# DCDmllm/AnyEdit

Hardware: AMD Instinct MI355X
Metric: edited-images/sec @512x512, 50 DDIM steps (higher is better)
Workload: dtype bf16; 1 GPU; configs[1]: AnySD (SD-1.5 UNet in=8 + task embedding/expert adapters) 512x512 bf16, 50 DDIM steps, batch=4/GPU, 3-branch CFG (UNet batch 12); images_per_gpu=4, ddim_steps=50, cfg_branches=3, hip_graph=True, parallelism=dp1 (image-sharded, no data-path collective)

## Files before the change

### anyedit_amd/_lib.py

```python
import ctypes
import os

import torch

_HERE = os.path.dirname(os.path.abspath(__file__))
LIB_PATH = os.environ.get("AE_LIB_PATH") or os.path.join(_HERE, "libanyedit_hip.so")

c_void_p, c_int, c_long, c_float = ctypes.c_void_p, ctypes.c_int, ctypes.c_long, ctypes.c_float

SIGNATURES = {
    "ae_version": [],
    "ae_last_error": [],
    "ae_device_arch": [ctypes.c_char_p, c_int],
    "ae_device_info": [ctypes.POINTER(c_int), ctypes.POINTER(c_long), ctypes.POINTER(c_int)],
    "ae_gemm_bf16": [c_void_p, c_long, c_void_p, c_long, c_int, c_void_p, c_long, c_void_p, c_long, c_int, c_int, c_int,
                     c_void_p, c_void_p, c_long, c_void_p, c_long, c_int, c_int, c_int, c_void_p, c_void_p],
    "ae_conv3x3_workspace_floats": [c_int, c_int, c_int, c_int, c_int, c_int, c_int],
    "ae_conv3x3_bf16": [c_void_p, c_void_p, c_void_p, c_void_p, c_long, c_void_p, c_void_p, c_int, c_int, c_int, c_int, c_int,
                        c_int, c_int, c_int, c_void_p, c_void_p, c_int, c_void_p],
    "ae_conv3x3_up2_bf16": [c_void_p, c_void_p, c_void_p, c_void_p, c_int, c_int, c_int, c_int, c_int, c_void_p, c_void_p],
    "ae_gemm_plan": [c_int] * 8 + [ctypes.POINTER(c_int)],
    "ae_conv3x3_plan": [c_int] * 11 + [ctypes.POINTER(c_int)],
    "ae_conv3x3_up2_plan": [c_int] * 6 + [ctypes.POINTER(c_int)],
    "ae_groupnorm_rows_per_chunk": [c_int, c_int],
    "ae_groupnorm_workspace_floats": [c_int, c_int, c_int, c_int],
    "ae_groupnorm_nhwc_bf16": [c_void_p, c_void_p, c_int, c_void_p, c_void_p, c_void_p, c_int, c_int, c_int, c_int, c_float,
                               c_int, c_void_p, c_void_p, c_void_p, c_void_p, c_void_p, c_void_p],
    "ae_layernorm_bf16": [c_void_p, c_void_p, c_void_p, c_void_p, c_int, c_int, c_float, c_void_p],
    "ae_attn_fwd_bf16": [c_void_p, c_void_p, c_void_p, c_void_p, c_int, c_int, c_int, c_int, c_int,
                         c_long, c_long, c_long, c_long, c_long, c_long, c_long, c_long, c_long, c_long, c_long, c_long,
                         c_float, c_void_p, c_void_p, c_int, c_int, c_void_p, c_void_p, c_int,
                         c_void_p, c_void_p, c_int, c_long, c_long, c_long, c_long, c_long, c_long, c_void_p, c_void_p, c_void_p,
                         c_void_p],
    "ae_attn_bwd_bf16": [c_void_p] * 10 + [c_int] * 5 + [c_long] * 21 + [c_float, c_void_p, c_int, c_void_p, c_void_p],
    "ae_attn_bwd_workspace_floats": [c_int] * 5,
    "ae_groupnorm_bwd_workspace_floats": [c_int, c_int, c_int, c_int],
    "ae_groupnorm_bwd_nhwc_bf16": [c_void_p, c_void_p, c_int, c_void_p, c_void_p, c_void_p, c_void_p, c_void_p, c_int, c_int, c_int,
                                   c_int, c_float, c_int, c_void_p, c_void_p, c_void_p, c_int, c_void_p],
    "ae_layernorm_bwd_bf16": [c_void_p, c_void_p, c_void_p, c_void_p, c_void_p, c_int, c_int, c_float, c_int, c_void_p],
    "ae_layernorm_param_grad_f32": [c_void_p, c_void_p, c_void_p, c_void_p, c_void_p, c_int, c_int, c_void_p],
    "ae_add_bf16": [c_void_p, c_void_p, c_void_p, c_long, c_void_p],
    "ae_axpy_bf16": [c_void_p, c_void_p, c_float, c_void_p, c_long, c_void_p],
    "ae_geglu_fwd_bf16": [c_void_p, c_void_p, c_long, c_int, c_void_p],
    "ae_geglu_bwd_bf16": [c_void_p, c_void_p, c_void_p, c_long, c_int, c_void_p],
    "ae_sumpool2x2_bf16": [c_void_p, c_void_p, c_int, c_int, c_int, c_int, c_void_p],
    "ae_colsum_bf16_f32": [c_void_p, c_void_p, c_int, c_int, c_long, c_void_p],
    "ae_mse_grad_f32": [c_void_p, c_void_p, c_void_p, c_long, c_float, c_void_p],
    "ae_adamw_f32": [c_void_p, c_void_p, c_void_p, c_void_p, c_long, c_float, c_float, c_float, c_float, c_float, c_int, c_float,
                     c_void_p],
    "ae_rowsum_f32": [c_void_p, c_void_p, c_int, c_long, c_void_p],
    "ae_scatter_add_rows_f32": [c_void_p, c_void_p, c_void_p, c_int, c_int, c_int, c_void_p],
    "ae_attn_fp8_workspace_bytes": [c_int, c_int, c_int, c_int, c_int],
    "ae_attn_fwd_fp8": [c_void_p, c_void_p, c_void_p, c_void_p, c_int, c_int, c_int, c_int, c_int] + [c_long] * 12 +
                       [c_float, c_void_p, c_void_p, c_int, c_int, c_void_p, c_long, c_void_p],
    "ae_ln_gemm_supported": [c_int, c_int, c_int, c_int],
    "ae_ln_gemm_bf16": [c_void_p, c_long, c_void_p, c_long, c_void_p, c_long, c_int, c_int, c_int, c_void_p, c_void_p, c_long, c_void_p, c_void_p,
                        c_float, c_int, c_void_p, c_void_p],
    "ae_gemm_ln_plan": [c_int, c_int, c_int, c_int, c_int],
    "ae_ff_fused_supported": [c_int, c_int, c_int],
    "ae_ff_fused_bf16": [c_void_p, c_long, c_void_p, c_void_p, c_float, c_void_p, c_long, c_void_p, c_void_p, c_void_p, c_void_p, c_long,
                         c_void_p, c_long, c_void_p, c_void_p, c_long, c_void_p, c_void_p, c_long, c_int, c_int, c_int, c_void_p],
    "ae_gemm_ln_bf16": [c_void_p, c_long, c_void_p, c_long, c_void_p, c_long, c_int, c_int, c_int, c_void_p, c_void_p, c_long, c_int, c_void_p,
                        c_void_p, c_int, c_void_p, c_float, c_void_p],
    "ae_task_gate_bwd": [c_void_p, c_void_p, c_void_p, c_void_p, c_int, c_int, c_int, c_void_p, c_void_p],
    "ae_task_gate_wgrad": [c_void_p, c_void_p, c_void_p, c_void_p, c_void_p, c_int, c_int, c_int, c_int, c_void_p, c_void_p, c_void_p],
    "ae_expert_kv_fwd": [c_void_p, c_void_p, c_void_p, c_void_p, c_int, c_int, c_int, c_int, c_int, c_void_p],
    "ae_expert_kv_dgrad_slices": [c_int],
    "ae_expert_kv_dgrad": [c_void_p, c_void_p, c_void_p, c_void_p, c_int, c_int, c_int, c_int, c_int, c_void_p, c_void_p],
    "ae_expert_kv_wgrad": [c_void_p, c_void_p, c_void_p, c_void_p, c_int, c_int, c_int, c_int, c_int, c_void_p],
    "ae_transpose_last2": [c_void_p, c_void_p, c_int, c_int, c_int, c_int, c_int, c_int, c_void_p],
    "ae_concat_channels_bf16": [c_void_p, c_int, c_void_p, c_int, c_void_p, c_long, c_void_p],
    "ae_im2col3x3_c8_bf16": [c_void_p, c_void_p, c_int, c_int, c_int, c_void_p],
    "ae_split_channels_bf16": [c_void_p, c_int, c_int, c_void_p, c_void_p, c_long, c_int, c_int, c_void_p],
    "ae_timestep_embedding": [c_void_p, c_void_p, c_void_p, c_void_p, c_int, c_int, c_float, c_void_p],
    "ae_ddim_step_f32": [c_void_p, c_void_p, c_void_p, c_void_p, c_void_p, c_void_p, c_long, c_int, c_float, c_float, c_float,
                         c_float, c_float, c_float, c_float, c_float, c_void_p],
    "ae_ddim_encode_step_f32": [c_void_p, c_void_p, c_void_p, c_long, c_int, c_float, c_float, c_float, c_void_p],
    "ae_plms_combine_f32": [c_void_p, c_void_p, c_void_p, c_void_p, c_void_p, c_long, c_int, c_void_p],
    "ae_mask_blend_f32": [c_void_p, c_void_p, c_void_p, c_void_p, c_void_p, c_int, c_int, c_int, c_float, c_float, c_int, c_void_p],
    "ae_q_sample_f32": [c_void_p, c_void_p, c_void_p, c_void_p, c_void_p, c_int, c_long, c_void_p],
    "ae_silu_to_bf16": [c_void_p, c_int, c_void_p, c_long, c_void_p],
    "ae_add_bcast_bf16": [c_void_p, c_void_p, c_void_p, c_long, c_long, c_void_p],
    "ae_resample2x_rows_bf16": [c_void_p, c_void_p, c_int, c_int, c_int, c_int, c_int, c_void_p],
    "ae_scale_shift_rows_bf16": [c_void_p, c_void_p, c_long, c_void_p, c_int, c_long, c_int, c_int, c_void_p],
    "ae_window_partition_bf16": [c_void_p, c_void_p, c_int, c_int, c_int, c_int, c_int, c_int, c_void_p],
    "ae_layernorm_window_supported": [c_int],
    "ae_layernorm_window_bf16": [c_void_p, c_void_p, c_void_p, c_void_p, c_void_p, c_void_p, c_int, c_int, c_int, c_int, c_int, c_int, c_float,
                                 c_void_p],
    "ae_sam_relpos_terms": [c_void_p, c_long, c_long, c_long, c_void_p, c_void_p, c_void_p, c_void_p, c_int, c_int, c_int, c_int,
                            c_int, c_int, c_int, c_void_p],
    "ae_softmax_rows_f32_bf16": [c_void_p, c_long, c_void_p, c_long, c_int, c_int, c_float, c_void_p],
    "ae_gaussian_moments_f32": [c_void_p, c_void_p, c_void_p, c_void_p, c_void_p, c_void_p, c_int, c_long, c_void_p],
    "ae_ms_deform_attn_fwd_f32": [c_void_p] * 6 + [c_int] * 7 + [c_void_p],
    "ae_ms_deform_attn_bwd_f32": [c_void_p] * 9 + [c_int] * 7 + [c_void_p],
    "ae_linear_f32": [c_void_p, c_long, c_void_p, c_long, c_void_p, c_void_p, c_long, c_int, c_int, c_int, c_void_p],
    "ae_dpm_multistep_f32": [c_void_p] * 5 + [c_long, c_int, c_float, c_int, c_int, c_float, c_float, c_int, c_float, c_float, c_float,
                             c_float, c_void_p],
    "ae_layernorm_act_bf16": [c_void_p, c_void_p, c_void_p, c_void_p, c_long, c_int, c_float, c_int, c_void_p],
    "ae_sam_pe_encode_f32": [c_void_p, c_void_p, c_void_p, c_void_p, c_void_p, c_int, c_int, c_float, c_float, c_float, c_void_p],
    "ae_sam_mask_downscale_bf16": [c_void_p] * 10 + [c_int, c_int, c_int, c_float, c_void_p],
    "ae_sam_mask_product_f32": [c_void_p, c_void_p, c_void_p, c_int, c_int, c_int, c_int, c_int, c_void_p],
    "ae_sam_postprocess_masks": [c_void_p, c_void_p, c_void_p] + [c_int] * 8 + [c_float, c_int, c_void_p],
    "ae_nms_sorted_f32": [c_void_p, c_void_p, c_int, c_float, c_void_p],
    "ae_sam_preprocess_f32": [c_void_p, c_int, c_void_p, c_int, c_int, c_int, c_int, c_int, c_void_p, c_void_p, c_void_p],
    "ae_patchify_f32_bf16": [c_void_p, c_void_p, c_int, c_int, c_int, c_int, c_int, c_void_p],
    "ae_mse_f32": [c_void_p, c_void_p, c_void_p, c_void_p, c_long, c_void_p],
    "ae_lincomb4_f32": [c_void_p, c_void_p, c_float, c_void_p, c_float, c_void_p, c_float, c_void_p, c_float, c_long, c_void_p],
    "ae_dpm_adaptive_err_f32": [c_void_p, c_void_p, c_void_p, c_float, c_float, c_int, c_long, c_void_p, c_void_p],
    "ae_task_gate": [c_void_p, c_void_p, c_void_p, c_void_p, c_int, c_int, c_int, c_int, c_void_p, c_void_p, c_void_p, c_void_p],
    "ae_attn_causal_short_bf16": [c_void_p, c_void_p, c_void_p, c_void_p, c_int, c_int, c_int, c_int] + [c_long] * 12 + [c_float, c_void_p],
    "ae_clip_embed_bf16": [c_void_p, c_int, c_void_p, c_void_p, c_void_p, c_int, c_int, c_int, c_int, c_int, c_void_p],
    "ae_bias_act_f32_bf16": [c_void_p, c_long, c_void_p, c_void_p, c_long, c_long, c_int, c_int, c_void_p],
    "ae_clip_pool_eos_bf16": [c_void_p, c_int, c_void_p, c_void_p, c_int, c_int, c_int, c_long, c_void_p],
    "ae_clip_patch_rows_bf16": [c_void_p, c_int, c_void_p, c_int, c_int, c_int, c_int, c_int, c_int, c_float, c_void_p, c_void_p, c_void_p],
    "ae_clip_vision_embed_ln_bf16": [c_void_p, c_long, c_void_p, c_void_p, c_void_p, c_void_p, c_void_p, c_int, c_int, c_int, c_float, c_void_p],
    "ae_clip_vision_pool_ln_bf16": [c_void_p, c_long, c_void_p, c_void_p, c_void_p, c_int, c_int, c_float, c_void_p],
    "ae_dino_embed_bf16": [c_void_p, c_long, c_void_p, c_void_p, c_void_p, c_void_p, c_int, c_int, c_int, c_void_p],
    "ae_swiglu_f32_bf16": [c_void_p, c_long, c_void_p, c_void_p, c_long, c_long, c_int, c_void_p],
    "ae_swin_window_attn_bf16": [c_void_p, c_long, c_void_p, c_void_p, c_void_p, c_long, c_int, c_int, c_int, c_int, c_int, c_int, c_int, c_float, c_void_p],
    "ae_swin_merge_ln_bf16": [c_void_p, c_void_p, c_void_p, c_void_p, c_int, c_int, c_int, c_int, c_float, c_void_p],
    "ae_scale_residual_f32_bf16": [c_void_p, c_long, c_void_p, c_void_p, c_void_p, c_long, c_void_p, c_long, c_long, c_int, c_void_p],
    "ae_biattn_split_rows": [c_int],
    "ae_biattn_workspace_bytes": [c_int, c_int, c_int, c_int, c_int],
    "ae_biattn_bf16": [c_void_p, c_long] * 4 + [c_void_p, c_void_p] + [c_void_p, c_long] * 2 + [c_int] * 5 + [c_float, c_void_p, c_long, c_void_p],
    "ae_attn_masked_short_bf16": [c_void_p] * 5 + [c_int] * 4 + [c_long] * 12 + [c_float, c_void_p],
    "ae_contrastive_bf16": [c_void_p, c_long, c_void_p, c_void_p, c_void_p, c_long, c_void_p] + [c_int] * 5 + [c_void_p],
    "ae_topk_rows_max_n": [],
    "ae_topk_rows_f32": [c_void_p, c_long, c_void_p, c_int, c_int, c_int, c_void_p],
    "ae_gdino_proposals_f32": [c_void_p, ctypes.POINTER(c_int), ctypes.POINTER(c_int), c_int, c_void_p, c_void_p, c_int, c_int, c_void_p],
    "ae_gdino_query_sine": [c_void_p, c_void_p, c_void_p, c_void_p, c_long, c_int, c_int, c_int, c_void_p],
    "ae_gdino_box_refine_f32": [c_void_p, c_long, c_void_p, c_void_p, c_void_p, c_void_p, c_void_p, c_long, c_int, c_void_p],
    "ae_gdino_text_spans": [c_void_p, c_int, c_int, c_int, c_int] + [c_long] * 8 + [c_void_p, c_void_p, c_void_p, c_void_p],
    "ae_bert_embed_ln_bf16": [c_void_p, c_void_p, c_void_p] + [c_void_p] * 6 + [c_int] * 6 + [c_float, c_void_p],
    "ae_attn_span_short_bf16": [c_void_p] * 5 + [c_int] * 4 + [c_long] * 12 + [c_float, c_void_p],
    "ae_gdino_level_geometry": [c_void_p, c_int, c_int, c_int, ctypes.POINTER(c_int), ctypes.POINTER(c_int), c_int, c_float, c_float, c_void_p, c_void_p, c_void_p,
                                c_void_p, c_int, c_void_p],
    "ae_gdino_neck_groupnorm_workspace_floats": [c_int, c_int],
    "ae_gdino_neck_groupnorm": [c_void_p, c_long, c_void_p, c_void_p, c_float, c_void_p, c_long, c_long, c_int, c_int, c_void_p, c_void_p],
    "ae_gdino_ground": [c_void_p, c_void_p, c_float, c_float, c_void_p, c_void_p, c_void_p, c_void_p, c_void_p, c_int, c_int, c_int, c_void_p],
    "ae_hed_stem_bf16": [c_void_p, c_int, c_long, c_long, c_long, c_long, c_void_p, c_void_p, c_void_p, c_void_p, c_int, c_int, c_int, c_int, c_void_p],
    "ae_relu_bf16": [c_void_p, c_long, c_void_p],
    "ae_hed_tail_bf16": [c_void_p, c_void_p, c_void_p, c_void_p, c_void_p, c_int, c_int, c_int, c_int, c_void_p],
    "ae_hed_fuse": [c_void_p] * 7 + [c_int] * 4 + [c_void_p],
}
_RESTYPES = {"ae_last_error": ctypes.c_char_p, "ae_groupnorm_workspace_floats": c_long, "ae_conv3x3_workspace_floats": c_long,
             "ae_groupnorm_bwd_workspace_floats": c_long, "ae_attn_fp8_workspace_bytes": c_long, "ae_attn_bwd_workspace_floats": c_long,
             "ae_biattn_workspace_bytes": c_long, "ae_gdino_neck_groupnorm_workspace_floats": c_long}


class AnyEditHipError(RuntimeError):
    pass


def _load():
    if not os.path.exists(LIB_PATH):
        raise ImportError(
            f"{LIB_PATH} is missing: the HIP extension is REQUIRED (no CPU/eager fallback exists). "
            "Build it with `python -c 'import __graft_entry__ as g; g.build()'` or `python anyedit_amd/build.py`.")
    lib = ctypes.CDLL(LIB_PATH)
    for name, argtypes in SIGNATURES.items():
        fn = getattr(lib, name)
        fn.argtypes = argtypes
        fn.restype = _RESTYPES.get(name, c_int)
    return lib


lib = _load()


def check(rc, what=""):
    if rc != 0:
        msg = lib.ae_last_error()
        raise AnyEditHipError(f"{what} failed (rc={rc}): {msg.decode() if msg else ''}")


def device_arch():
    buf = ctypes.create_string_buffer(128)
    check(lib.ae_device_arch(buf, 128), "ae_device_arch")
    return buf.value.decode()
```

### anyedit_amd/anysd/model.py

```python
import torch
import torch.nn as nn

from anyedit_amd import ops
from anyedit_amd.cldm.model import trusted_torch_load
from anyedit_amd.ldm.modules.attention import BasicTransformerBlock

BF16 = torch.bfloat16

EDIT_TYPES = ["add", "remove", "replace", "color_alter", "appearance_alter", "material_alter", "action_change",
              "textual_change", "background_change", "tone_transfer", "style_change", "movement", "outpaint", "rotation_change",
              "resize", "implicit_change", "relation_change", "counting", "visual_reference", "visual_bbox", "visual_depth",
              "visual_scribble", "visual_segment", "visual_sketch", "visual_material_transfer"]


class ImageProjModel(nn.Module):

    def __init__(self, clip_dim=1280, cross_dim=768, tokens=4):
        super().__init__()
        self.tokens, self.cross_dim = tokens, cross_dim
        self.proj = nn.Linear(clip_dim, tokens * cross_dim)
        self.norm = nn.LayerNorm(cross_dim)

    def rows(self, ref_embeds):
        B = ref_embeds.shape[0]
        cls = ref_embeds[:, 0].to(BF16).contiguous()
        y = ops.gemm(cls, ops.pack_linear(self.proj.weight), self.proj.bias.detach().float().contiguous())
        y = y.reshape(B * self.tokens, self.cross_dim)
        return ops.layernorm(y, self.norm.weight.detach().float().contiguous(), self.norm.bias.detach().float().contiguous(),
                             self.norm.eps)


class MoE(nn.Module):

    def __init__(self, unet, image_encoder=None, expert_num=11, ckpt_path=None, n_tasks=len(EDIT_TYPES), context_dim=768,
                 clip_dim=1280, ip_tokens=4):
        super().__init__()
        self.unet = unet
        enc_dim = getattr(image_encoder, "hidden_size", None)
        if enc_dim is not None and enc_dim != clip_dim:
            raise ValueError(f"MoE: the image encoder's hidden_size {enc_dim} does not match clip_dim {clip_dim} (image_proj_model reads hidden states of that width)")
        self.image_encoder = image_encoder
        self.expert_num = expert_num
        self.context_dim = context_dim
        self.image_proj_model = ImageProjModel(clip_dim, context_dim, ip_tokens)
        self.task_embs = nn.Parameter(torch.randn(n_tasks, context_dim) * 0.02)
        self.gate = nn.Linear(context_dim, expert_num)
        self._blocks = [m for m in unet.modules() if isinstance(m, BasicTransformerBlock)]
        self.adapter_modules = nn.ParameterList(
            [nn.Parameter(torch.randn(expert_num, 2 * b.attn2.heads * b.attn2.dim_head, context_dim) * context_dim ** -0.5)
             for b in self._blocks])
        if ckpt_path is not None:
            self.load_state_dict(trusted_torch_load(ckpt_path, "cpu"), strict=False)

    def save_pretrained(self, path):
        sd = {k: v for k, v in self.state_dict().items() if not k.startswith(("unet.", "image_encoder."))}
        torch.save(sd, path)

    @torch.no_grad()
    def route(self, edit_code):
        return ops.task_gate(self.task_embs.detach(), edit_code, self.gate.weight.detach(), self.gate.bias.detach())

    @torch.no_grad()
    def reference_embeds(self, pixel_values):
        if self.image_encoder is None:
            raise ValueError("MoE.reference_embeds: this MoE was built without an image_encoder (MoE(unet, image_encoder=CLIPVisionModelWithProjection(...)))")
        return self.image_encoder.encode_pixels(pixel_values, -2).clone()

    @torch.no_grad()
    def prepare_conditioning(self, encoder_hidden_states, ref_embeds, edit_code, ip_scale=None):
        if ref_embeds.dim() == 4:
            ref_embeds = self.reference_embeds(ref_embeds)
        B, L, Dc = encoder_hidden_states.shape
        dev = encoder_hidden_states.device
        te = self.task_embs.detach()[edit_code.long()]
        ctx = torch.cat([encoder_hidden_states.float(), te[:, None, :].float()], dim=1)
        context_rows = ctx.reshape(B * (L + 1), Dc).to(BF16).contiguous()
        probs, top1, top1p = self.route(edit_code)
        gate = top1p if ip_scale is None else top1p * ip_scale
        ip_rows = self.image_proj_model.rows(ref_embeds)
        T_ip = self.image_proj_model.tokens
        kv_cache = {}
        for blk, W in zip(self._blocks, self.adapter_modules):
            attn = blk.attn2
            kv_cache[id(attn)] = attn.project_kv(context_rows)
            Wm = W.detach()
            if Wm.dtype != torch.float32 or not Wm.is_contiguous():
                Wm = Wm.float().contiguous()
            kv_ip = ops.expert_kv(ip_rows, Wm, top1, T_ip)
            kv_cache[("adapter", id(attn))] = (kv_ip, gate.float().contiguous())
        return context_rows, kv_cache

    @torch.no_grad()
    def denoise(self, x, timesteps, context_rows, kv_cache, emb_pack=None):
        return self.unet.forward_rows(x, timesteps, context_rows, kv_cache=kv_cache, emb_pack=emb_pack)

    def forward(self, noisy_latents, timesteps, encoder_hidden_states, image_embeds, edit_code):
        context_rows, kv_cache = self.prepare_conditioning(encoder_hidden_states, image_embeds, edit_code)
        return self.denoise(noisy_latents, timesteps, context_rows, kv_cache)
```

### anyedit_amd/anysd/pipeline.py

```python
import numpy as np
import torch

from anyedit_amd import ops
from anyedit_amd.ldm.models.diffusion.ddim import DDIMSampler, _f32


class EditPipeline:
    def __init__(self, moe, schedule_model, use_graph=True, text_encoder=None):
        self.moe = moe
        self.text_encoder = text_encoder
        self._null_ehs, self._null_tok = None, None
        self.sampler = DDIMSampler(schedule_model)
        self.schedule_model = schedule_model
        self.use_graph = use_graph
        self._graph = None
        self._graph_key = None
        self._emb_pack = None
        self.randn = torch.randn

    def _denoise_static(self):
        if self._emb_pack is not None:
            return self.moe.denoise(self._x_in, self._t, self._ctx_rows, self._kv_cache, emb_pack=self._emb_pack)
        return self.moe.denoise(self._x_in, self._t, self._ctx_rows, self._kv_cache)

    def _hoist_time_embedding(self, steps_desc, nb, dev):
        import os
        unet = getattr(self.moe, "unet", None)
        if os.environ.get("AE_HOIST_TEMB", "1") == "0" or unet is None or not hasattr(unet, "time_embedding_rows") or getattr(unet, "num_classes", None) is not None:
            if self._emb_pack is not None:
                self._emb_pack, self._graph = None, None
            return None
        pack = unet.time_embedding_rows(torch.as_tensor(np.ascontiguousarray(steps_desc), dtype=torch.long, device=dev))
        if self._emb_pack is None or tuple(self._emb_pack.all.shape) != (nb, pack.all.shape[1]) or self._emb_pack.offsets != pack.offsets:
            from anyedit_amd.ldm.modules.diffusionmodules.openaimodel import EmbPack
            self._emb_pack = EmbPack(None, torch.empty(nb, pack.all.shape[1], dtype=torch.float32, device=dev), pack.offsets)
            self._graph = None
        return pack.all

    def set_step(self, t, temb_row=None):
        self._t.fill_(int(t))
        if self._emb_pack is not None:
            if temb_row is None:
                temb_row = self.moe.unet.time_embedding_rows(torch.full((1,), int(t), dtype=torch.long, device=self._t.device)).all[0]
            self._emb_pack.all.copy_(temb_row.unsqueeze(0).expand_as(self._emb_pack.all))

    def _ensure_graph(self, key):
        if self._graph is not None and self._graph_key == key:
            return
        cur = torch.cuda.current_stream()
        side = torch.cuda.Stream()
        side.wait_stream(cur)
        with torch.cuda.stream(side):
            for _ in range(2):
                self._denoise_static()
        cur.wait_stream(side)
        torch.cuda.synchronize()
        g = torch.cuda.CUDAGraph()
        with torch.cuda.graph(g):
            self._eps = self._denoise_static()
        self._graph, self._graph_key = g, key

    @torch.no_grad()
    def prepare(self, img_lat, ehs, null_ehs, ref_embeds, edit_code):
        B = img_lat.shape[0]
        if null_ehs.shape[0] == 1:
            null_ehs = null_ehs.expand(B, -1, -1)
        ehs3 = torch.cat([ehs, null_ehs, null_ehs], 0)
        ref3 = torch.cat([ref_embeds, ref_embeds, torch.zeros_like(ref_embeds)], 0)
        code3 = torch.cat([edit_code] * 3, 0)
        ctx_rows, kv_cache = self.moe.prepare_conditioning(ehs3, ref3, code3)
        img_cond3 = torch.cat([img_lat, img_lat, torch.zeros_like(img_lat)], 0).float()
        C = img_lat.shape[1]
        shape_in = (3 * B, 2 * C, *img_lat.shape[2:])
        if self._same_layout(ctx_rows, kv_cache, shape_in):
            self._ctx_rows.copy_(ctx_rows)
            for k, v in kv_cache.items():
                cur = self._kv_cache[k]
                if isinstance(v, tuple):
                    for c, n in zip(cur, v):
                        c.copy_(n)
                else:
                    cur.copy_(v)
        else:
            self._ctx_rows, self._kv_cache = ctx_rows, kv_cache
            self._x_in = torch.empty(shape_in, dtype=torch.float32, device=img_lat.device)
            self._t = torch.zeros(3 * B, dtype=torch.long, device=img_lat.device)
            self._graph = None
        self._x_in[:, C:] = img_cond3

    def _same_layout(self, ctx_rows, kv_cache, shape_in):
        if getattr(self, "_kv_cache", None) is None or getattr(self, "_x_in", None) is None:
            return False
        if tuple(self._x_in.shape) != tuple(shape_in) or self._ctx_rows.shape != ctx_rows.shape or self._kv_cache.keys() != kv_cache.keys():
            return False
        for k, v in kv_cache.items():
            cur = self._kv_cache[k]
            a, b = (cur, v) if isinstance(v, tuple) else ((cur,), (v,))
            if any(x.shape != y.shape or x.dtype != y.dtype for x, y in zip(a, b)):
                return False
        return True

    def _prompt_ids(self, prompts_or_ids):
        te = self.text_encoder
        if isinstance(prompts_or_ids, str) or (isinstance(prompts_or_ids, (list, tuple)) and prompts_or_ids and isinstance(prompts_or_ids[0], str)):
            tok = te._need_tokenizer()
            return tok(prompts_or_ids, truncation=True, max_length=te.max_length, return_length=True, return_overflowing_tokens=False,
                       padding="max_length", return_tensors="pt")["input_ids"]
        return prompts_or_ids

    def null_prompt_ehs(self):
        te = self.text_encoder
        tok = te.transformer.weights_token()
        if self._null_ehs is None or self._null_tok != tok:
            cfg = te.transformer.config
            n = min(te.max_length, cfg["max_position_embeddings"])
            ids = [[cfg["bos_token_id"], cfg["eos_token_id"]] + [cfg["pad_token_id"]] * (n - 2)]
            self._null_ehs, self._null_tok = te.encode_ids(ids).clone(), tok
        return self._null_ehs

    @torch.no_grad()
    def edit_text(self, x_T, img_lat, prompts_or_ids, ref_embeds, edit_code, reference_images=None, **edit_kwargs):
        if self.text_encoder is None:
            raise ValueError("edit_text: this pipeline was built without a text_encoder (EditPipeline(..., text_encoder=FrozenCLIPEmbedder(...)))")
        null_ehs = self.null_prompt_ehs()
        ehs = self.text_encoder.encode_ids(self._prompt_ids(prompts_or_ids))
        return self.edit(x_T, img_lat, ehs, null_ehs, ref_embeds, edit_code, reference_images=reference_images, **edit_kwargs)

    @torch.no_grad()
    def edit(self, x_T, img_lat, ehs, null_ehs, ref_embeds, edit_code, steps=50, s_txt=7.5, s_img=1.5, eta=0.0, mask=None,
             x0=None, prepared=False, step_callback=None, reference_images=None):
        B, C = x_T.shape[0], x_T.shape[1]
        dev = x_T.device
        if reference_images is not None:
            if ref_embeds is not None:
                raise ValueError("edit: pass ref_embeds or reference_images, not both")
            ref_embeds = self.moe.reference_embeds(reference_images)
        if not prepared:
            self.prepare(img_lat, ehs, null_ehs, ref_embeds, edit_code)
        s = self.sampler
        s.make_schedule(ddim_num_steps=steps, ddim_eta=eta, verbose=False)
        timesteps = s.ddim_timesteps
        total = timesteps.shape[0]
        img = x_T.float().contiguous()
        blend_noise = self.randn(x0.shape, device=dev) if mask is not None else None
        temb = self._hoist_time_embedding(np.flip(timesteps), 3 * B, dev)
        if temb is not None:
            self._emb_pack.all.copy_(temb[0].unsqueeze(0).expand_as(self._emb_pack.all))
        if self.use_graph:
            self._ensure_graph((tuple(x_T.shape), steps))
        x_view = self._x_in[:, :C].view(3, B, C, *x_T.shape[2:])
        for i, step in enumerate(np.flip(timesteps)):
            index = total - i - 1
            x_view.copy_(img.unsqueeze(0))
            self.set_step(step, temb[i] if temb is not None else None)
            if self.use_graph:
                self._graph.replay()
                eps = self._eps
            else:
                eps = self._denoise_static()
            noise = self.randn(img.shape, device=dev) if eta != 0.0 else None
            img, _ = ops.ddim_step(img, eps, s._coeffs(index, False), 3, s0=float(s_txt), s1=float(s_img), noise=noise,
                                   want_pred_x0=False)
            if mask is not None:
                sa = float(_f32(self.schedule_model.sqrt_alphas_cumprod[int(step)]))
                s1 = float(_f32(self.schedule_model.sqrt_one_minus_alphas_cumprod[int(step)]))
                img = ops.mask_blend(img, x0, blend_noise, mask, sa, s1, ip2p_order=True)
            if step_callback is not None:
                step_callback(i, img)
        return img
```

### anyedit_amd/csrc/c_api.hip

```cpp
#include "common.hpp"
#include <stdarg.h>
#include <stdio.h>
#include <string.h>

static thread_local char g_err[512] = "";

void ae_set_error(const char* fmt, ...) {
    va_list ap;
    va_start(ap, fmt);
    vsnprintf(g_err, sizeof(g_err), fmt, ap);
    va_end(ap);
}

int ae_check_launch(const char* what) {
    hipError_t e = hipGetLastError();
    if (e != hipSuccess) {
        ae_set_error("%s: launch failed: %s", what, hipGetErrorString(e));
        return AE_ERR_LAUNCH;
    }
    return AE_OK;
}

extern "C" int ae_version(void) { return 100; }

extern "C" const char* ae_last_error(void) { return g_err; }

extern "C" int ae_device_arch(char* buf, int n) {
    if (!buf || n <= 0) return AE_ERR_ARG;
    int dev = 0;
    hipDeviceProp_t prop;
    if (hipGetDevice(&dev) != hipSuccess || hipGetDeviceProperties(&prop, dev) != hipSuccess) {
        ae_set_error("ae_device_arch: no HIP device");
        buf[0] = 0;
        return AE_ERR_LAUNCH;
    }
    strncpy(buf, prop.gcnArchName, (size_t)n - 1);
    buf[n - 1] = 0;
    return AE_OK;
}

extern "C" int ae_device_info(int* cus, long* hbm_bytes, int* clock_khz) {
    int dev = 0;
    hipDeviceProp_t prop;
    if (hipGetDevice(&dev) != hipSuccess || hipGetDeviceProperties(&prop, dev) != hipSuccess) {
        ae_set_error("ae_device_info: no HIP device");
        return AE_ERR_LAUNCH;
    }
    if (cus) *cus = prop.multiProcessorCount;
    if (hbm_bytes) *hbm_bytes = (long)prop.totalGlobalMem;
    if (clock_khz) *clock_khz = prop.clockRate;
    return AE_OK;
}
```

### anyedit_amd/csrc/common.hpp

```cpp
#pragma once
#include <hip/hip_runtime.h>
#include <stdint.h>

typedef uint16_t bf16_t;
typedef __attribute__((ext_vector_type(8))) __bf16 bf16x8_t;
typedef __attribute__((ext_vector_type(4))) float f32x4;
typedef __attribute__((ext_vector_type(2))) float f32x2;
typedef __attribute__((ext_vector_type(4))) uint32_t u32x4;
typedef __attribute__((ext_vector_type(2))) uint32_t u32x2;

#define AE_OK 0
#define AE_ERR_ARG -1
#define AE_ERR_LAUNCH -2
#define AE_ERR_UNSUPPORTED -3

void ae_set_error(const char* fmt, ...);
int ae_check_launch(const char* what);
int ae_launch_colstats(const uint16_t* x, long ld, int M, int N, float* out, hipStream_t stream);

int ae_rowpanel_fold_covers(int M, int N, int K, int epilogue, int mode);
int ae_rowpanel_fold_launch(const void* A, long lda, const void* W, long ldw, void* C, long ldc, int M, int N, int K, const float* bias, const void* residual,
                            long ldr, int epilogue, float* rowstats_out, const float* ln_stats, int ln_parts, const float* ln_colsum, float ln_eps, void* stream);

#define AE_REQUIRE(cond, ...)                 \
    do {                                      \
        if (!(cond)) {                        \
            ae_set_error(__VA_ARGS__);        \
            return AE_ERR_ARG;                \
        }                                     \
    } while (0)

__device__ __forceinline__ float bf16_to_f32(bf16_t h) { return __uint_as_float(((uint32_t)h) << 16); }

typedef __attribute__((ext_vector_type(2))) __bf16 bf16x2_t;

__device__ __forceinline__ uint32_t pack_bf16x2(float lo, float hi) {
    union { bf16x2_t b; uint32_t u; } c;
    c.b = (bf16x2_t){(__bf16)lo, (__bf16)hi};
    return c.u;
}

__device__ __forceinline__ bf16_t f32_to_bf16(float f) { return (bf16_t)(pack_bf16x2(f, 0.f) & 0xffffu); }

__device__ __forceinline__ float bf16lo(uint32_t w) { return __uint_as_float(w << 16); }
__device__ __forceinline__ float bf16hi(uint32_t w) { return __uint_as_float(w & 0xffff0000u); }

__device__ __forceinline__ bf16x8_t as_bf16x8(u32x4 v) {
    union { u32x4 u; bf16x8_t b; } c;
    c.u = v;
    return c.b;
}

typedef __attribute__((ext_vector_type(4))) short s16x4_t;
__device__ __forceinline__ s16x4_t as_s16x4(u32x2 v) {
    union { u32x2 u; s16x4_t s; } c;
    c.u = v;
    return c.s;
}

__device__ __forceinline__ float silu_f(float x) {
    return x * __builtin_amdgcn_rcpf(1.0f + __builtin_amdgcn_exp2f(-1.4426950408889634f * x));
}
__device__ __forceinline__ float erf_as_f(float z) {
    const float az = __builtin_fabsf(z);
    const float t = __builtin_amdgcn_rcpf(__builtin_fmaf(0.3275911f, az, 1.0f));
    float poly = __builtin_fmaf(1.061405429f, t, -1.453152027f);
    poly = __builtin_fmaf(poly, t, 1.421413741f);
    poly = __builtin_fmaf(poly, t, -0.284496736f);
    poly = __builtin_fmaf(poly, t, 0.254829592f);
    poly *= t;
    const float e = __builtin_amdgcn_exp2f(-1.4426950408889634f * az * az);
    const float r = __builtin_fmaf(-poly, e, 1.0f);
    return __builtin_copysignf(r, z);
}
#ifndef AE_GELU_POLY
#define AE_GELU_POLY 0
#endif
__device__ __forceinline__ float gelu_w_poly_f(float x) {
    const float ax = __builtin_fminf(__builtin_fabsf(x), 4.25f);
    const float t = __builtin_fmaf(ax * ax, 0.11072664707899094f, -1.0f);
    float p = __builtin_fmaf(0.004925727378576994f, t, -0.012811211869120598f);
    p = __builtin_fmaf(p, t, 0.017165469005703926f);
    p = __builtin_fmaf(p, t, -0.02821926586329937f);
    p = __builtin_fmaf(p, t, 0.05118509382009506f);
    p = __builtin_fmaf(p, t, -0.07870230078697205f);
    p = __builtin_fmaf(p, t, 0.11140184104442596f);
    p = __builtin_fmaf(p, t, -0.1615230143070221f);
    p = __builtin_fmaf(p, t, 0.33187076449394226f);
    return ax * p;
}
__device__ __forceinline__ float gelu_w_f(float x) {
    if (AE_GELU_POLY) return gelu_w_poly_f(x);
    const float ax = __builtin_fabsf(x);
    const float t = __builtin_amdgcn_rcpf(__builtin_fmaf(0.3275911f * 0.70710678118654752440f, ax, 1.0f));
    float poly = __builtin_fmaf(1.061405429f, t, -1.453152027f);
    poly = __builtin_fmaf(poly, t, 1.421413741f);
    poly = __builtin_fmaf(poly, t, -0.284496736f);
    poly = __builtin_fmaf(poly, t, 0.254829592f);
    poly *= t;
    const float e = __builtin_amdgcn_exp2f((-0.5f * 1.4426950408889634f) * ax * ax);
    return __builtin_fmaf(-poly, e, 1.0f);
}
#ifndef AE_GELU_OLD
#define AE_GELU_OLD 0
#endif
__device__ __forceinline__ float gelu_erf_f(float x) {
    if (AE_GELU_OLD) return 0.5f * x * (1.0f + erf_as_f(x * 0.70710678118654752440f));
    return 0.5f * __builtin_fmaf(__builtin_fabsf(x), gelu_w_f(x), x);
}
__device__ __forceinline__ float geglu_half_f(float a_half, float g) {
    if (AE_GELU_OLD) return (a_half + a_half) * gelu_erf_f(g);
    return a_half * __builtin_fmaf(__builtin_fabsf(g), gelu_w_f(g), g);
}

__device__ __forceinline__ int xcd_remap(int bid, int nblocks) {
    const int NX = 8;
    int xcd = bid % NX, j = bid / NX;
    int q = nblocks / NX, r = nblocks % NX;
    int base = (xcd < r) ? xcd * (q + 1) : r * (q + 1) + (xcd - r) * q;
    return base + j;
}

__device__ __forceinline__ void ae_dma16(__amdgpu_buffer_rsrc_t rs, int lds_byte, int voffset, int soffset = 0) {
#if defined(__HIP_DEVICE_COMPILE__)
    asm volatile("s_mov_b32 m0, %2\n\ts_nop 0\n\tbuffer_load_dwordx4 %0, %1, %3 offen lds" ::"v"(voffset), "s"(rs), "s"(lds_byte), "s"(soffset)
                 : "memory", "m0");
#endif
}

__device__ __forceinline__ float wave_reduce_sum(float v) {
#pragma unroll
    for (int o = 32; o > 0; o >>= 1) v += __shfl_xor(v, o, 64);
    return v;
}
__device__ __forceinline__ float wave_reduce_max(float v) {
#pragma unroll
    for (int o = 32; o > 0; o >>= 1) v = fmaxf(v, __shfl_xor(v, o, 64));
    return v;
}
```

### anyedit_amd/csrc/elementwise.hip

```cpp
#include "common.hpp"

namespace {

constexpr int NT = 256;

__device__ __forceinline__ float ld_any(const void* p, long i, int is_bf16) {
    return is_bf16 ? bf16_to_f32(reinterpret_cast<const bf16_t*>(p)[i]) : reinterpret_cast<const float*>(p)[i];
}
__device__ __forceinline__ void st_any(void* p, long i, float v, int is_bf16) {
    if (is_bf16) reinterpret_cast<bf16_t*>(p)[i] = f32_to_bf16(v);
    else reinterpret_cast<float*>(p)[i] = v;
}

__global__ void transpose_kernel(const void* in, void* out, int X, int Y, int Xpad, int in_bf16, int out_bf16) {
    __shared__ float tile[32][33];
    const int b = blockIdx.z;
    const int x0 = blockIdx.x * 32, y0 = blockIdx.y * 32;
    const int tx = threadIdx.x & 31, ty = threadIdx.x >> 5;
    for (int j = ty; j < 32; j += 8) {
        const int x = x0 + j, y = y0 + tx;
        tile[j][tx] = (x < X && y < Y) ? ld_any(in, ((long)b * X + x) * Y + y, in_bf16) : 0.f;
    }
    __syncthreads();
    for (int j = ty; j < 32; j += 8) {
// ... 334 lines not shown
    }
}

struct RelposArgs {
    long q_sb, q_sh, q_sn;
    int BH, Hh, qH, qW, kH, kW;
    int items[2];
};

template <int D16>
__global__ __launch_bounds__(256) void relpos_mfma_kernel(const bf16_t* __restrict__ q, const float* __restrict__ Rh, const float* __restrict__ Rw,
                                                          float* __restrict__ rel_h, float* __restrict__ rel_w, const RelposArgs p) {
    constexpr int D = 16 * D16;
    const int lane = threadIdx.x & 63, l15 = lane & 15, g = lane >> 4;
    long item = (long)blockIdx.x * 4 + __builtin_amdgcn_readfirstlane(threadIdx.x >> 6);
    int part = 0;
    if (item >= p.items[0]) { item -= p.items[0]; part = 1; }
    if (item >= p.items[part]) return;
    const int Lq = part == 0 ? p.qW : p.qH, K = part == 0 ? p.kH : p.kW;
    const int nks = (K + 15) / 16;
    const long ntrip = (long)p.BH * Lq;
    const int ngrp = (int)((ntrip + 63) / 64);
    int r = (int)item;
    const int grp = r % ngrp; r /= ngrp;
    const int ks = r % nks; r /= nks;
    const int line = r;
    const int k0 = ks * 16;
    const int krow = k0 + l15 < K ? k0 + l15 : K - 1;
    const float* Rrow = (part == 0 ? Rh : Rw) + ((long)line * K + krow) * D + 4 * g;
    f32x4 av[D16];
#pragma unroll
    for (int u = 0; u < D16; ++u) av[u] = *reinterpret_cast<const f32x4*>(Rrow + 16 * u);
    float* outp = part == 0 ? rel_h : rel_w;
    const long N = (long)p.qH * p.qW;
#pragma unroll
    for (int t = 0; t < 4; ++t) {
        long trip = (long)grp * 64 + t * 16 + l15;
        const bool live = trip < ntrip;
        if (!live) trip = ntrip - 1;
        const int h = (int)(trip % p.Hh);
        const long rest = trip / p.Hh;
        const int qi = (int)(rest % Lq), b = (int)(rest / Lq);
        const long n = part == 0 ? (long)line * p.qW + qi : (long)qi * p.qW + line;
        const bf16_t* qr = q + (long)b * p.q_sb + (long)h * p.q_sh + n * p.q_sn + 4 * g;
        uint2 bv[D16];
#pragma unroll
        for (int u = 0; u < D16; ++u) bv[u] = *reinterpret_cast<const uint2*>(qr + 16 * u);
        f32x4 acc = {0.f, 0.f, 0.f, 0.f};
#pragma unroll
        for (int u = 0; u < D16; ++u) {
            acc = __builtin_amdgcn_mfma_f32_16x16x4f32(av[u][0], bf16lo(bv[u].x), acc, 0, 0, 0);
            acc = __builtin_amdgcn_mfma_f32_16x16x4f32(av[u][1], bf16hi(bv[u].x), acc, 0, 0, 0);
            acc = __builtin_amdgcn_mfma_f32_16x16x4f32(av[u][2], bf16lo(bv[u].y), acc, 0, 0, 0);
            acc = __builtin_amdgcn_mfma_f32_16x16x4f32(av[u][3], bf16hi(bv[u].y), acc, 0, 0, 0);
        }
        if (live) {
            float* o = outp + (((long)b * p.Hh + h) * N + n) * K;
            const int kk = k0 + 4 * g;
            if ((K & 3) == 0 && kk + 3 < K) *reinterpret_cast<f32x4*>(o + kk) = acc;
            else if ((K & 1) == 0) {
                if (kk + 1 < K) *reinterpret_cast<float2*>(o + kk) = make_float2(acc[0], acc[1]);
                if (kk + 3 < K) *reinterpret_cast<float2*>(o + kk + 2) = make_float2(acc[2], acc[3]);
            } else {
#pragma unroll
                for (int e = 0; e < 4; ++e)
                    if (kk + e < K) o[kk + e] = acc[e];
            }
        }
    }
}

__global__ __launch_bounds__(NT) void softmax_rows_kernel(const float* S, long lds, bf16_t* P, long ldp, int cols, float scale) {
    __shared__ float red[NT / 64];
    const float* src = S + (long)blockIdx.x * lds;
    bf16_t* dst = P + (long)blockIdx.x * ldp;
    const int lane = threadIdx.x & 63, wave = threadIdx.x >> 6;
    float mx = -INFINITY;
    for (int c = threadIdx.x; c < cols; c += NT) mx = fmaxf(mx, src[c]);
    mx = wave_reduce_max(mx);
    if (lane == 0) red[wave] = mx;
    __syncthreads();
    mx = fmaxf(fmaxf(red[0], red[1]), fmaxf(red[2], red[3]));
    __syncthreads();
    const float c2 = scale * 1.4426950408889634f;
    float sum = 0.f;
    for (int c = threadIdx.x; c < cols; c += NT) sum += __builtin_amdgcn_exp2f((src[c] - mx) * c2);
    sum = wave_reduce_sum(sum);
    if (lane == 0) red[wave] = sum;
    __syncthreads();
    const float inv = 1.0f / ((red[0] + red[1]) + (red[2] + red[3]));
    for (int c = threadIdx.x; c < cols; c += NT) dst[c] = f32_to_bf16(__builtin_amdgcn_exp2f((src[c] - mx) * c2) * inv);
}

__global__ __launch_bounds__(NT) void gaussian_kernel(const float* moments, const float* noise, float* z, float* mean_o, float* logvar_o,
                                                      float* std_o, long per_half, long n) {
    for (long i = (long)blockIdx.x * NT + threadIdx.x; i < n; i += (long)gridDim.x * NT) {
        const long b = i / per_half, r = i - b * per_half;
        const float mean = moments[b * 2 * per_half + r];
        const float logvar = fminf(fmaxf(moments[b * 2 * per_half + per_half + r], -30.0f), 20.0f);
        const float sd = expf(0.5f * logvar);
        z[i] = noise ? mean + sd * noise[i] : mean;
        if (mean_o) mean_o[i] = mean;
        if (logvar_o) logvar_o[i] = logvar;
        if (std_o) std_o[i] = sd;
    }
}

__global__ void patchify_kernel(const float* x, bf16_t* y, int B, int Cin, int H, int W, int P) {
    const int gh = H / P, gw = W / P, K = Cin * P * P;
    const long total = (long)B * gh * gw * K;
    for (long i = (long)blockIdx.x * NT + threadIdx.x; i < total; i += (long)gridDim.x * NT) {
        const int k = (int)(i % K);
        long r = i / K;
        const int px = (int)(r % gw); r /= gw;
        const int py = (int)(r % gh); r /= gh;
        const int b = (int)r;
        const int c = k / (P * P), kk = k % (P * P), ky = kk / P, kx = kk % P;
        y[i] = f32_to_bf16(x[(((long)b * Cin + c) * H + py * P + ky) * W + px * P + kx]);
    }
}

constexpr int MSE_MAX_BLOCKS = 1024;
__global__ __launch_bounds__(NT) void mse_partial_kernel(const float* a, const float* b, float* partial, long n) {
    __shared__ float red[NT / 64];
    float s = 0.f;
    for (long i = (long)blockIdx.x * NT + threadIdx.x; i < n; i += (long)gridDim.x * NT) {
        const float d = a[i] - b[i];
        s += d * d;
    }
    s = wave_reduce_sum(s);
    if ((threadIdx.x & 63) == 0) red[threadIdx.x >> 6] = s;
    __syncthreads();
    if (threadIdx.x == 0) partial[blockIdx.x] = (red[0] + red[1]) + (red[2] + red[3]);
}
__global__ __launch_bounds__(NT) void mse_final_kernel(const float* partial, int nb, float* out, float inv_n) {
    __shared__ float red[NT / 64];
    float s = 0.f;
    for (int i = threadIdx.x; i < nb; i += NT) s += partial[i];
    s = wave_reduce_sum(s);
    if ((threadIdx.x & 63) == 0) red[threadIdx.x >> 6] = s;
    __syncthreads();
    if (threadIdx.x == 0) out[0] = ((red[0] + red[1]) + (red[2] + red[3])) * inv_n;
}

inline unsigned grid_for(long n, int per_thread = 1) {
    long b = (n + (long)NT * per_thread - 1) / ((long)NT * per_thread);
    if (b > 4096) b = 4096;
    if (b < 1) b = 1;
    return (unsigned)b;
}

}

__global__ __launch_bounds__(256) void lincomb4_kernel(float* __restrict__ out, const float* x0, float c0, const float* x1, float c1,
                                                        const float* x2, float c2, const float* x3, float c3, long n) {
    const long i = ((long)blockIdx.x * 256 + threadIdx.x) * 4;
    if (i >= n) return;
    if (i + 4 <= n) {
        f32x4 a = *reinterpret_cast<const f32x4*>(x0 + i);
        f32x4 r = {a[0] * c0, a[1] * c0, a[2] * c0, a[3] * c0};
        if (x1) { const f32x4 b = *reinterpret_cast<const f32x4*>(x1 + i); for (int e = 0; e < 4; ++e) r[e] = fmaf(b[e], c1, r[e]); }
        if (x2) { const f32x4 b = *reinterpret_cast<const f32x4*>(x2 + i); for (int e = 0; e < 4; ++e) r[e] = fmaf(b[e], c2, r[e]); }
        if (x3) { const f32x4 b = *reinterpret_cast<const f32x4*>(x3 + i); for (int e = 0; e < 4; ++e) r[e] = fmaf(b[e], c3, r[e]); }
        *reinterpret_cast<f32x4*>(out + i) = r;
    } else {
        for (long j = i; j < n; ++j) {
            float r = x0[j] * c0;
            if (x1) r = fmaf(x1[j], c1, r);
            if (x2) r = fmaf(x2[j], c2, r);
            if (x3) r = fmaf(x3[j], c3, r);
            out[j] = r;
        }
    }
}

__global__ __launch_bounds__(1024) void dpm_adaptive_err_kernel(const float* __restrict__ xl, const float* __restrict__ xh,
                                                                const float* __restrict__ xp, float atol, float rtol, long n, float* out) {
    __shared__ float red[16];
    const long base = (long)blockIdx.x * n;
    float acc = 0.f;
    for (long i = threadIdx.x; i < n; i += 1024) {
        const float l = xl[base + i];
        const float delta = fmaxf(atol, rtol * fmaxf(fabsf(l), fabsf(xp[base + i])));
        const float v = (xh[base + i] - l) / delta;
        acc = fmaf(v, v, acc);
    }
    acc = wave_reduce_sum(acc);
    if ((threadIdx.x & 63) == 0) red[threadIdx.x >> 6] = acc;
    __syncthreads();
    if (threadIdx.x == 0) {
        float t = 0.f;
        for (int w = 0; w < 16; ++w) t += red[w];
        out[blockIdx.x] = sqrtf(t / (float)n);
    }
}

extern "C" int ae_transpose_last2(const void* in, void* out, int B, int X, int Y, int Xpad, int in_bf16, int out_bf16, void* stream) {
    AE_REQUIRE(in && out && B > 0 && X > 0 && Y > 0 && Xpad >= X, "ae_transpose_last2: bad arguments");
    AE_REQUIRE(B <= 65535, "ae_transpose_last2: batch %d too large", B);
    dim3 grid((Xpad + 31) / 32, (Y + 31) / 32, B);
    hipLaunchKernelGGL(transpose_kernel, grid, dim3(256), 0, (hipStream_t)stream, in, out, X, Y, Xpad, in_bf16, out_bf16);
    return ae_check_launch("ae_transpose_last2");
}

extern "C" int ae_concat_channels_bf16(const void* a, int Ca, const void* b, int Cb, void* y, long rows, void* stream) {
    AE_REQUIRE(a && b && y && rows > 0 && Ca > 0 && Cb > 0 && Ca % 8 == 0 && Cb % 8 == 0, "ae_concat_channels_bf16: bad arguments");
    hipLaunchKernelGGL(concat_kernel, dim3(grid_for(rows * ((Ca + Cb) / 8))), dim3(NT), 0, (hipStream_t)stream,
                       (const bf16_t*)a, Ca, (const bf16_t*)b, Cb, (bf16_t*)y, rows);
    return ae_check_launch("ae_concat_channels_bf16");
}

extern "C" int ae_im2col3x3_c8_bf16(const void* x, void* y, int B, int H, int W, void* stream) {
    AE_REQUIRE(x && y && B > 0 && H > 0 && W > 0, "ae_im2col3x3_c8_bf16: bad arguments");
    AE_REQUIRE(((uintptr_t)x & 15) == 0 && ((uintptr_t)y & 15) == 0, "ae_im2col3x3_c8_bf16: 16-byte alignment");
    hipLaunchKernelGGL(im2col3x3_c8_kernel, dim3(grid_for((long)B * H * W * 16)), dim3(NT), 0, (hipStream_t)stream, (const bf16_t*)x, (bf16_t*)y, B, H, W);
    return ae_check_launch("ae_im2col3x3_c8_bf16");
}

extern "C" int ae_split_channels_bf16(const void* y, int Ca, int Cb, void* a, void* b, long rows, int accumulate_a, int accumulate_b, void* stream) {
    AE_REQUIRE(y && (a || b) && rows > 0 && Ca > 0 && Cb > 0 && Ca % 8 == 0 && Cb % 8 == 0, "ae_split_channels_bf16: bad arguments");
    hipLaunchKernelGGL(split_kernel, dim3(grid_for(rows * ((Ca + Cb) / 8))), dim3(NT), 0, (hipStream_t)stream, (const bf16_t*)y, Ca, Cb, (bf16_t*)a,
                       (bf16_t*)b, rows, accumulate_a, accumulate_b);
    return ae_check_launch("ae_split_channels_bf16");
}

extern "C" int ae_timestep_embedding(const long* t_i64, const float* t_f32, void* out_bf16, float* out_f32, int B, int dim,
                                     float max_period, void* stream) {
    AE_REQUIRE((t_i64 != nullptr) != (t_f32 != nullptr), "ae_timestep_embedding: pass exactly one of t_i64 / t_f32");
    AE_REQUIRE((out_bf16 || out_f32) && B > 0 && dim > 1, "ae_timestep_embedding: bad arguments");
    hipLaunchKernelGGL(timestep_embedding_kernel, dim3((B * dim + NT - 1) / NT), dim3(NT), 0, (hipStream_t)stream, t_i64, t_f32,
                       (bf16_t*)out_bf16, out_f32, B, dim, max_period);
    return ae_check_launch("ae_timestep_embedding");
}

extern "C" int ae_ddim_step_f32(const float* x, const float* eps, const float* noise, float* x_prev, float* pred_x0, float* e_out,
                                long n, int branches, float s0, float s1, float sqrt_one_minus_at, float sqrt_at,
                                float sqrt_a_prev, float dir_coef, float sigma_t, float temperature, void* stream) {
    AE_REQUIRE(x && eps && x_prev && n > 0, "ae_ddim_step_f32: null pointer / bad n");
    AE_REQUIRE(branches >= 1 && branches <= 3, "ae_ddim_step_f32: branches must be 1, 2 or 3 (got %d)", branches);
    DdimArgs a{x, eps, noise, x_prev, pred_x0, e_out, n, branches, s0, s1, sqrt_one_minus_at, sqrt_at, sqrt_a_prev, dir_coef, sigma_t, temperature};
    hipLaunchKernelGGL(ddim_step_kernel, dim3(grid_for(n)), dim3(NT), 0, (hipStream_t)stream, a);
    return ae_check_launch("ae_ddim_step_f32");
}

extern "C" int ae_ddim_encode_step_f32(const float* x, const float* eps, float* x_next, long n, int branches, float scale, float cx,
                                       float ce, void* stream) {
    AE_REQUIRE(x && eps && x_next && n > 0, "ae_ddim_encode_step_f32: null pointer / bad n");
    AE_REQUIRE(branches == 1 || branches == 2, "ae_ddim_encode_step_f32: branches must be 1 or 2 (got %d)", branches);
    hipLaunchKernelGGL(ddim_encode_step_kernel, dim3(grid_for(n)), dim3(NT), 0, (hipStream_t)stream, x, eps, x_next, n, branches, scale, cx, ce);
    return ae_check_launch("ae_ddim_encode_step_f32");
}

extern "C" int ae_plms_combine_f32(const float* e_t, const float* old1, const float* old2, const float* old3, float* out, long n, int order,
                                   void* stream) {
    AE_REQUIRE(e_t && out && n > 0 && order >= 0 && order <= 3, "ae_plms_combine_f32: bad arguments (order must be 0..3)");
    AE_REQUIRE(old1 && (order < 2 || old2) && (order < 3 || old3), "ae_plms_combine_f32: order %d needs that many previous predictions", order);
    hipLaunchKernelGGL(plms_combine_kernel, dim3(grid_for(n)), dim3(NT), 0, (hipStream_t)stream, e_t, old1, old2, old3, out, n, order);
    return ae_check_launch("ae_plms_combine_f32");
}

extern "C" int ae_mask_blend_f32(const float* img, const float* x0, const float* noise, const float* mask, float* out, int B,
                                 int C, int HW, float sqrt_ac, float sqrt_one_minus_ac, int ip2p_order, void* stream) {
    AE_REQUIRE(img && x0 && noise && mask && out && B > 0 && C > 0 && HW > 0, "ae_mask_blend_f32: bad arguments");
    const long n = (long)B * C * HW;
    hipLaunchKernelGGL(mask_blend_kernel, dim3(grid_for(n)), dim3(NT), 0, (hipStream_t)stream, img, x0, noise, mask, out, n, C, HW,
                       sqrt_ac, sqrt_one_minus_ac, ip2p_order);
    return ae_check_launch("ae_mask_blend_f32");
}

extern "C" int ae_q_sample_f32(const float* x0, const float* noise, const float* sqrt_ac, const float* sqrt_one_minus_ac, float* out,
                               int B, long per_sample, void* stream) {
    AE_REQUIRE(x0 && noise && sqrt_ac && sqrt_one_minus_ac && out && B > 0 && per_sample > 0, "ae_q_sample_f32: bad arguments");
    const long n = (long)B * per_sample;
    hipLaunchKernelGGL(q_sample_kernel, dim3(grid_for(n)), dim3(NT), 0, (hipStream_t)stream, x0, noise, sqrt_ac, sqrt_one_minus_ac, out,
                       per_sample, n);
    return ae_check_launch("ae_q_sample_f32");
}

extern "C" int ae_silu_to_bf16(const void* x, int in_bf16, void* y, long n, void* stream) {
    AE_REQUIRE(x && y && n > 0, "ae_silu_to_bf16: bad arguments");
    hipLaunchKernelGGL(silu_kernel, dim3(grid_for(n)), dim3(NT), 0, (hipStream_t)stream, x, in_bf16, (bf16_t*)y, n);
    return ae_check_launch("ae_silu_to_bf16");
}

extern "C" int ae_add_bcast_bf16(const void* x, const void* p, void* y, long n, long period, void* stream) {
    AE_REQUIRE(x && p && y && n > 0 && period > 0 && n % 8 == 0 && period % 8 == 0 && n % period == 0, "ae_add_bcast_bf16: bad arguments");
    hipLaunchKernelGGL(add_bcast_kernel, dim3(grid_for(n, 8)), dim3(NT), 0, (hipStream_t)stream, (const bf16_t*)x, (const bf16_t*)p,
                       (bf16_t*)y, n, period);
    return ae_check_launch("ae_add_bcast_bf16");
}

extern "C" int ae_resample2x_rows_bf16(const void* x, void* y, int B, int H, int W, int C, int mode, void* stream) {
    AE_REQUIRE(x && y && B > 0 && H > 0 && W > 0 && C > 0 && C % 8 == 0 && (mode == 0 || mode == 1), "ae_resample2x_rows_bf16: bad arguments (C %% 8 == 0, mode 0 = nearest x2, 1 = 2x2 mean)");
    AE_REQUIRE(mode == 0 || (H >= 2 && W >= 2), "ae_resample2x_rows_bf16: a 2x2 mean needs H, W >= 2");
    AE_REQUIRE(((uintptr_t)x & 15) == 0 && ((uintptr_t)y & 15) == 0, "ae_resample2x_rows_bf16: 16-byte alignment");
    const long n = (long)B * (mode ? H / 2 : 2 * H) * (mode ? W / 2 : 2 * W) * (C / 8);
    hipLaunchKernelGGL(resample2x_rows_kernel, dim3(grid_for(n)), dim3(NT), 0, (hipStream_t)stream, (const bf16_t*)x, (bf16_t*)y, B, H, W, C, mode);
    return ae_check_launch("ae_resample2x_rows_bf16");
}

extern "C" int ae_scale_shift_rows_bf16(const void* x, const float* emb, long ld_emb, void* y, int B, long HW, int C, int silu, void* stream) {
    AE_REQUIRE(x && emb && y && B > 0 && HW > 0 && C > 0 && C % 8 == 0 && ld_emb >= 2L * C, "ae_scale_shift_rows_bf16: bad arguments (C %% 8 == 0, emb rows hold scale | shift = 2 C floats)");
    AE_REQUIRE(((uintptr_t)x & 15) == 0 && ((uintptr_t)y & 15) == 0 && ((uintptr_t)emb & 3) == 0, "ae_scale_shift_rows_bf16: alignment");
    const long n = (long)B * HW * (C / 8);
    hipLaunchKernelGGL(scale_shift_rows_kernel, dim3(grid_for(n)), dim3(NT), 0, (hipStream_t)stream, (const bf16_t*)x, emb, ld_emb, (bf16_t*)y, HW, C, n, silu);
    return ae_check_launch("ae_scale_shift_rows_bf16");
// ... 122 lines not shown
```

### anyedit_amd/csrc/gemm_conv.hip

```cpp
#include "common.hpp"
#include <stdlib.h>
#include <string.h>
#include <type_traits>

namespace {

#ifndef AE_CONV_SPEC
#define AE_CONV_SPEC 1
#endif
#ifndef AE_XE_OCC
#define AE_XE_OCC 4
#endif
#ifndef AE_PP_LAB
#define AE_PP_LAB 0
#endif
#ifndef AE_PP_PRIO
#define AE_PP_PRIO 1
#endif
#ifndef AE_PP_DMA_FIRST
#define AE_PP_DMA_FIRST 0
#endif
constexpr int BK = 64;

enum { A_DENSE = 0, A_CONV3 = 1 };
// ... 1170 lines not shown
    }
}

int pick_tile(int M, int N) {
    const int cand[3][2] = {{128, 128}, {128, 64}, {64, 64}};
    if (N % 160 == 0 && N % 128 != 0 && (long)((M + 127) / 128) * (N / 160) >= 256) return 3;
    for (int c = 0; c < 3; ++c) {
        const long tm = (M + cand[c][0] - 1) / cand[c][0], tn = (N + cand[c][1] - 1) / cand[c][1];
        const double waste = (double)(tn * cand[c][1]) / (double)N;
        if (tm * tn >= 256 && waste <= 1.10) return c;
    }
    return 2;
}

struct Plan { int tile, splitk; };
Plan make_plan(int M, int N, int K, bool can_split) {
    const int t = pick_tile(M, N);
    const int kt = (K + BK - 1) / BK;
    static const int force_s = getenv("AE_GEMM_SPLITK") ? atoi(getenv("AE_GEMM_SPLITK")) : 0;
    static const int t320_split = getenv("AE_CONV_T320_SPLITK") ? atoi(getenv("AE_CONV_T320_SPLITK")) : 3;
    if (t320_split && can_split && N % 320 == 0 && M % 192 == 0 && force_s <= 0) {
        const long t192 = (long)(M / 192) * (N / 320);
        if (t192 >= 32 && t192 <= (t320_split == 2 ? 64 : (t320_split == 3 && kt < 180 ? 64 : 128))) {
            int s = (int)(256 / t192);
            if (s > 8) s = 8;
            while (s > 1 && kt / s < 16) --s;
            if (s >= 2) return {4, s};
        }
    }
    if (!can_split || kt < 32 || t == 0 || t == 3) return {t, 1};
    const long t128 = (long)((M + 127) / 128) * ((N + 127) / 128);
    const double waste128 = (double)(((N + 127) / 128) * 128) / (double)N;
    if (waste128 <= 1.10 && t128 < 256) {
        int s = force_s > 0 ? force_s : (int)((480 + t128 - 1) / t128);
        static const int smax = getenv("AE_CONV_SPLIT_MAX") ? atoi(getenv("AE_CONV_SPLIT_MAX")) : 8;
        if (s > smax) s = smax;
        if (s > kt / 8) s = kt / 8;
        if (s >= 2) return {0, s};
    }
    return {t, 1};
}

template <typename Kern>
int launch_kernel(Kern kern, unsigned grid, int threads, size_t lds, hipStream_t stream, const GemmArgs& a, const char* what) {
    if (lds > 64 * 1024) {
        static const void* done[32];
        static int ndone = 0;
        const void* fn = reinterpret_cast<const void*>(kern);
        bool seen = false;
        for (int i = 0; i < ndone; ++i) seen |= done[i] == fn;
        if (!seen) {
            if (hipFuncSetAttribute(fn, hipFuncAttributeMaxDynamicSharedMemorySize, (int)lds) != hipSuccess) {
                ae_set_error("hipFuncSetAttribute(MaxDynamicSharedMemorySize=%zu) failed", lds);
                return AE_ERR_LAUNCH;
            }
            if (ndone < 32) done[ndone++] = fn;
        }
    }
    hipLaunchKernelGGL(kern, dim3(grid), dim3(threads), lds, stream, a);
    return ae_check_launch(what);
}

struct PlanReport {
    int BM, BN, AMODE, WAVES_M, WAVES_N, GLDS, WAVES_K, STAGES, CS, LAB, WA, XE;
    int grid, threads, lds, splitk;
    int reduce, colstats;
    int rowpanel;
};
#define AE_PLAN_INTS 19
static_assert(sizeof(PlanReport) == AE_PLAN_INTS * sizeof(int), "PlanReport is the int array of anyedit_hip.h");

void* const kQueryPtr = reinterpret_cast<void*>(uintptr_t(256));
float* const kQueryF32 = reinterpret_cast<float*>(uintptr_t(256));
int plan_out(int rc, const PlanReport& r, int* plan) {
    if (!rc) memcpy(plan, &r, sizeof r);
    return rc;
}

struct LaunchCtx { const GemmArgs& a; hipStream_t stream; const char* what; PlanReport* report; };

template <int BM, int BN, int AMODE, int WAVES_M = 2, int WAVES_N = 2, bool GLDS = false, int WAVES_K = 1, int STAGES = 2, bool CS = false, int LAB = 0, int WA = 0, int XE = 0>
int run_tile(const LaunchCtx& c, long grid, size_t lds) {
    constexpr int threads = 64 * WAVES_M * WAVES_N * WAVES_K;
    if (c.report) {
        *c.report = PlanReport{BM, BN, AMODE, WAVES_M, WAVES_N, GLDS, WAVES_K, STAGES, CS, LAB, WA, XE, (int)grid, threads, (int)lds, c.a.splitk, 0, 0, 0};
        return 0;
    }
    return launch_kernel(gemm_kernel<BM, BN, AMODE, WAVES_M, WAVES_N, GLDS, WAVES_K, STAGES, CS, LAB, WA, XE>, (unsigned)grid, threads, lds, c.stream, c.a, c.what);
}

template <int BM, int BN, int AMODE, int WAVES_M, int WAVES_N>
int run_plain(const LaunchCtx& c, bool glds, long grid) {
    const size_t lds = (size_t)2 * (BM + BN) * BK * sizeof(bf16_t);
    return glds ? run_tile<BM, BN, AMODE, WAVES_M, WAVES_N, true>(c, grid, lds) : run_tile<BM, BN, AMODE, WAVES_M, WAVES_N, false>(c, grid, lds);
}

template <int AMODE>
int launch(const GemmArgs& a_in, hipStream_t stream, PlanReport* report = nullptr, int split_tile = 0) {
    GemmArgs a = a_in;
    static const int mfast_env = getenv("AE_GEMM_MFAST") ? atoi(getenv("AE_GEMM_MFAST")) : -1;
    a.m_fast = mfast_env >= 0 ? mfast_env : (AMODE == A_CONV3 ? (9L * a.N >= 8L * a.M) : ((long)a.N >= 3L * a.M)) ? 1 : 0;
    const int cand[4][2] = {{128, 128}, {128, 64}, {64, 64}, {128, 160}};
    static const int t160 = getenv("AE_GEMM_T160") ? atoi(getenv("AE_GEMM_T160")) : 1;
    int pick = a.splitk > 1 ? 0 : pick_tile(a.M, a.N);
    static const int force_tile = getenv("AE_GEMM_TILE") ? atoi(getenv("AE_GEMM_TILE")) : -1;
    if (force_tile >= 0 && force_tile <= 2 && a.splitk <= 1) pick = force_tile;
    if (pick == 3 && (!t160 || AMODE == A_DENSE || a.epi == EPI_GEGLU || a.splitk > 1)) pick = 1;
    const int kt_block = ((a.K + BK - 1) / BK + a.splitk - 1) / a.splitk;
    const bool conv = AMODE == A_CONV3;
    const char* what = conv ? "ae_conv3x3_bf16" : "ae_gemm_bf16";
    const LaunchCtx lc{a, stream, what, report};
    static const int glds_env = getenv("AE_GEMM_GLDS") ? atoi(getenv("AE_GEMM_GLDS")) : 1;
    const bool glds = glds_env && (conv ? (a.Cin == a.CinPad) : (a.K % BK == 0 && (!a.A2 || a.Ksplit % BK == 0)));
    if (conv && a.kmajor && !glds) { ae_set_error("%s: the chunk-major K order exists only in the LDS-DMA loader (AE_GEMM_GLDS=0 is set)", what); return AE_ERR_UNSUPPORTED; }
    auto lds_of = [](int bm, int bn, int st) { return (size_t)st * (bm + bn) * BK * sizeof(bf16_t); };
    auto lds_wa = [](int bm, int bn) { return (size_t)(2 * bm + 3 * bn) * BK * sizeof(bf16_t); };
#ifdef AE_GEMM_TRACE
    auto lds_aa = [](int bm, int bn) { return (size_t)(3 * bm + 2 * bn) * BK * sizeof(bf16_t) + 8192; };
#else
    auto lds_aa = [](int bm, int bn) { return (size_t)(3 * bm + 2 * bn) * BK * sizeof(bf16_t); };
#endif
    int rc = 0;

    static const int t320 = getenv("AE_GEMM_T320") ? atoi(getenv("AE_GEMM_T320")) : 11;
    bool done = false;
    bool xe_done = false;
    const bool cs_epi_ok = a.colstats && a.epi != EPI_GEGLU && !a.out_f32 && a.splitk <= 1 && a.N % 8 == 0 && a.ldc % 8 == 0 &&
                           (!a.res || (a.ldr % 8 == 0 && (reinterpret_cast<uintptr_t>(a.res) & 15) == 0));
    bool cs_done = false;
#ifdef AE_GEMM_ABLATE
    static const int lab_abl = getenv("AE_GEMM_ABL") ? atoi(getenv("AE_GEMM_ABL")) : 0;
#endif
    const bool slab_ok = conv && a.kmajor && a.stride == 1 && !a.ups && a.Cin == a.CinPad && a.H == a.Ho && a.Wd == a.Wo && a.Wd % 16 == 0 && 192 % a.Wd == 0 &&
                         192 / a.Wd <= a.H + 1 &&
                         (a.splitk <= 1 || kt_block % 9 == 0);
    const size_t lds_slab = (size_t)2 * ((192 + 192 / 16 + 1 + 7) / 8) * 1024 + (size_t)2 * 320 * BK * sizeof(bf16_t);
    if (conv && a.splitk > 1 && glds && split_tile == 4) {
        const long t = (long)(a.M / 192) * (a.N / 320) * a.splitk;
        if constexpr (AMODE == A_CONV3) {
            if (slab_ok) rc = run_tile<192, 320, A_CONV3, 2, 4, true, 1, 2, false, 0, 4>(lc, t, lds_slab);
            else if (!a.ups) rc = run_tile<192, 320, A_CONV3, 2, 4, true, 1, 2, false, 0, 3>(lc, t, lds_aa(192, 320));
            else rc = run_tile<192, 320, A_CONV3, 2, 4, true>(lc, t, lds_of(192, 320, 2));
        }
        done = true;
    }
    if (!done && t320 && glds && a.splitk <= 1 && a.N % 320 == 0 && ((conv && (t320 & 1)) || (!conv && a.epi == EPI_GEGLU && a.K >= 640 && (t320 & 2)) || (!conv && a.epi == EPI_GEGLU && a.K < 640 && a.K >= 320 && (t320 & 4)) ||
                                                                     (!conv && a.epi != EPI_GEGLU && a.K >= 640 && (t320 & 8)))) {
        const long t = (long)((a.M + 191) / 192) * (a.N / 320);
        const double fill = (double)t / (double)(((t + 255) / 256) * 256) * ((double)a.M / (double)(((a.M + 191) / 192) * 192));
        static const int t320_xe = getenv("AE_GEMM_T320_XE") ? atoi(getenv("AE_GEMM_T320_XE")) : 1;
        const long t128x = (long)((a.M + 127) / 128) * ((a.N + 127) / 128);
        const bool xe_tail = t320_xe && !conv && a.xe == 2 && a.epi != EPI_GEGLU && fill >= 0.74 && fill < 0.85 &&
                             (double)t128x / (double)(((t128x + 511) / 512) * 512) <= 0.72;
        if (fill >= 0.85 || xe_tail) {
            if constexpr (AMODE == A_DENSE) {
                if (xe_tail || (a.epi == EPI_GEGLU && a.xe == 2)) { rc = run_tile<192, 320, A_DENSE, 4, 2, true, 1, 2, false, 0, 3, 2>(lc, t, lds_aa(192, 320) + 2 * 320 * sizeof(float)); xe_done = true; }
                else if (a.epi == EPI_GEGLU) rc = run_tile<192, 320, A_DENSE, 4, 2, true, 1, 2, false, 0, 3>(lc, t, lds_aa(192, 320));
                else rc = run_tile<192, 320, A_DENSE, 2, 4, true, 1, 2, false, 0, 3>(lc, t, lds_aa(192, 320));
            } else {
#ifdef AE_GEMM_ABLATE
                if (lab_abl == 1) rc = run_tile<192, 320, A_CONV3, 2, 4, true, 1, 2, false, 1>(lc, t, lds_of(192, 320, 2));
                else if (lab_abl == 2) rc = run_tile<192, 320, A_CONV3, 2, 4, true, 1, 2, false, 2>(lc, t, lds_of(192, 320, 2));
                else if (lab_abl == 3) rc = run_tile<192, 320, A_CONV3, 2, 4, true, 1, 2, false, 3>(lc, t, lds_of(192, 320, 2));
                else if (lab_abl == 4) rc = run_tile<192, 320, A_CONV3, 2, 4, true, 1, 2, false, 4>(lc, t, lds_of(192, 320, 2));
                else if (lab_abl == 20) rc = run_tile<192, 320, A_CONV3, 2, 4, false>(lc, t, lds_of(192, 320, 2));
                else
#endif
                if (!a.ups) {
                    if (slab_ok && cs_epi_ok) { rc = run_tile<192, 320, A_CONV3, 2, 4, true, 1, 2, true, 0, 4>(lc, t, lds_slab); cs_done = true; }
                    else if (slab_ok) rc = run_tile<192, 320, A_CONV3, 2, 4, true, 1, 2, false, 0, 4>(lc, t, lds_slab);
                    else if (cs_epi_ok) { rc = run_tile<192, 320, A_CONV3, 2, 4, true, 1, 2, true, 0, 3>(lc, t, lds_aa(192, 320)); cs_done = true; }
                    else rc = run_tile<192, 320, A_CONV3, 2, 4, true, 1, 2, false, 0, 3>(lc, t, lds_aa(192, 320));
                } else if (cs_epi_ok) {
                    rc = run_tile<192, 320, A_CONV3, 2, 4, true, 1, 2, true>(lc, t, lds_of(192, 320, 2));
                    cs_done = true;
                }
                else rc = run_tile<192, 320, A_CONV3, 2, 4, true>(lc, t, lds_of(192, 320, 2));
            }
            done = true;
        }
    }
    static const int deep_pref = getenv("AE_GEMM_DEEP") ? atoi(getenv("AE_GEMM_DEEP")) : 1;
    if constexpr (AMODE == A_DENSE) {
        if (!done && deep_pref && glds && a.splitk <= 1 && a.epi != EPI_GEGLU && a.N % 128 == 0 && a.K >= 1280) {
            const long t128 = (long)((a.M + 127) / 128) * (a.N / 128);
            const long t192 = (long)((a.M + 191) / 192) * (a.N / 128);
            if (t128 >= 128 && t128 <= 256) {
                if (a.xe == 1) rc = run_tile<128, 128, A_DENSE, 4, 2, true, 1, 3, false, 0, 0, 1>(lc, t128, lds_of(128, 128, 3));
                else if (a.xe) rc = run_tile<128, 128, A_DENSE, 4, 2, true, 1, 3, false, 0, 0, 2>(lc, t128, lds_of(128, 128, 3));
                else rc = run_tile<128, 128, A_DENSE, 4, 2, true, 1, 3>(lc, t128, lds_of(128, 128, 3));
                xe_done = a.xe != 0;
                done = true;
            } else if (t128 > 256 && t192 >= 128 && t192 <= 256 && a.K >= 2560) {
                rc = run_tile<192, 128, A_DENSE, 4, 2, true, 1, 3>(lc, t192, lds_of(192, 128, 3));
                done = true;
            }
        }
    }
    if (!done) {
        const int BM = cand[pick][0], BN = cand[pick][1];
        const unsigned grid = (unsigned)((long)((a.M + BM - 1) / BM) * ((a.N + BN - 1) / BN) * a.splitk);
        static const int deep64_max = getenv("AE_GEMM_DEEP64_MAX") ? atoi(getenv("AE_GEMM_DEEP64_MAX")) : 768;
        if (pick == 3) {
            if constexpr (AMODE == A_CONV3) rc = run_plain<128, 160, AMODE, 2, 2>(lc, glds, grid);
        }
#ifdef AE_GEMM_ABLATE
        else if (pick == 0 && glds && lab_abl == 1) rc = run_tile<128, 128, AMODE, 4, 2, true, 1, 2, false, 1>(lc, grid, lds_of(128, 128, 2));
        else if (pick == 0 && glds && lab_abl == 2) rc = run_tile<128, 128, AMODE, 4, 2, true, 1, 2, false, 2>(lc, grid, lds_of(128, 128, 2));
        else if (pick == 0 && glds && lab_abl == 3) rc = run_tile<128, 128, AMODE, 4, 2, true, 1, 2, false, 3>(lc, grid, lds_of(128, 128, 2));
        else if (pick == 0 && glds && lab_abl == 4) rc = run_tile<128, 128, AMODE, 4, 2, true, 1, 2, false, 4>(lc, grid, lds_of(128, 128, 2));
#endif
        else if (pick == 0 && cs_epi_ok && glds) {
            rc = run_tile<128, 128, AMODE, 4, 2, true, 1, 2, true, 0, 1>(lc, grid, lds_wa(128, 128));
            cs_done = true;
        } else if (pick == 0 && glds && (conv || kt_block >= 3)) {
            if constexpr (AMODE == A_DENSE) {
                if (a.xe == 1) rc = run_tile<128, 128, A_DENSE, 4, 2, true, 1, 2, false, 0, 1, 1>(lc, grid, lds_wa(128, 128));
                else if (a.xe) rc = run_tile<128, 128, A_DENSE, 4, 2, true, 1, 2, false, 0, 1, 2>(lc, grid, lds_wa(128, 128));
                xe_done = a.xe != 0;
            }
            if (!a.xe) rc = run_tile<128, 128, AMODE, 4, 2, true, 1, 2, false, 0, 1>(lc, grid, lds_wa(128, 128));
        }
        else if (pick == 0) {
            if constexpr (AMODE == A_DENSE) rc = run_plain<128, 128, AMODE, 4, 2>(lc, glds, grid);
            else rc = run_tile<128, 128, A_CONV3, 4, 2, false>(lc, grid, lds_of(128, 128, 2));
        } else if (pick == 1) {
            if constexpr (AMODE == A_DENSE) rc = run_plain<128, 64, AMODE, 4, 2>(lc, glds, grid);
            else rc = run_plain<128, 64, AMODE, 2, 2>(lc, glds, grid);
        } else if (deep_pref && glds && !conv && a.splitk <= 1 && grid <= (unsigned)deep64_max && a.K >= 1280) {
            if constexpr (AMODE == A_DENSE) rc = run_tile<64, 64, A_DENSE, 2, 2, true, 1, 3>(lc, grid, lds_of(64, 64, 3));
        } else rc = run_plain<64, 64, AMODE, 2, 2>(lc, glds, grid);
    }
    if (rc) return rc;
    if (a.xe && !xe_done) {
        ae_set_error("%s: no %s instantiation for M=%d N=%d K=%d epilogue %d (ae_gemm_ln_plan says which shapes are covered)", what,
                     a.xe == 1 ? "row-statistics" : "LayerNorm-fold", a.M, a.N, a.K, a.epi);
        return AE_ERR_UNSUPPORTED;
    }
    if (report) {
        report->reduce = a.splitk > 1;
        report->colstats = a.colstats && !cs_done;
        return 0;
    }
    if (a.splitk > 1) {
        long nb = ((long)a.M * a.N / 4 + 255) / 256;
        if (nb > 2048) nb = 2048;
        hipLaunchKernelGGL(splitk_reduce_kernel, dim3((unsigned)nb), dim3(256), 0, stream, a);
        rc = ae_check_launch("ae_conv3x3_bf16(split-K reduce)");
        if (rc) return rc;
    }
    if (a.colstats && !cs_done) return ae_launch_colstats(reinterpret_cast<const bf16_t*>(a.C), a.ldc, a.M, a.epi == EPI_GEGLU ? a.N / 2 : a.N, a.colstats, stream);
    return rc;
}

bool aligned16(const void* p) { return (reinterpret_cast<uintptr_t>(p) & 15) == 0; }

}

int ae_launch_colstats(const bf16_t* x, long ld, int M, int N, float* out, hipStream_t stream) {
    hipLaunchKernelGGL(colstats_kernel, dim3((unsigned)((M + 31) / 32), (unsigned)((N + 255) / 256)), dim3(256), 0, stream, x, ld, M, N, out);
    return ae_check_launch("column statistics");
}

namespace {
struct LnExtras {
    float* rowstats_out = nullptr;
    const float* ln_stats = nullptr;
    const float* ln_colsum = nullptr;
    int ln_parts = 0;
    float ln_eps = 0.f;
};
int gemm_args(GemmArgs& a, const void* A, long lda, const void* A2, long lda2, int Ksplit, const void* W, long ldw,
              void* C, long ldc, int M, int N, int K, const float* bias, const void* residual, long ldr,
              const float* addvec, long addvec_ld, int rows_per_batch, int epilogue, int out_f32, float* colstats, const LnExtras& x) {
    AE_REQUIRE(A && W && C, "ae_gemm_bf16: null pointer");
    if (colstats) AE_REQUIRE(!out_f32 && N % 8 == 0 && ldc % 8 == 0 && (reinterpret_cast<uintptr_t>(colstats) & 15) == 0, "ae_gemm_bf16: column statistics need a bf16 output with N %% 8 == 0 and 16-byte rows");
    AE_REQUIRE(M > 0 && N > 0 && K > 0, "ae_gemm_bf16: M,N,K must be positive (got %d,%d,%d)", M, N, K);
    AE_REQUIRE(K % 8 == 0, "ae_gemm_bf16: K=%d must be a multiple of 8", K);
    AE_REQUIRE(N % 4 == 0, "ae_gemm_bf16: N=%d must be a multiple of 4", N);
    AE_REQUIRE(lda % 8 == 0 && ldw % 8 == 0 && aligned16(A) && aligned16(W), "ae_gemm_bf16: A/W rows must be 16-byte aligned");
    AE_REQUIRE(ldc % 4 == 0 && (reinterpret_cast<uintptr_t>(C) & 15) == 0, "ae_gemm_bf16: C must be 16-byte aligned, ldc %% 4 == 0");
    AE_REQUIRE(epilogue >= EPI_NONE && epilogue <= EPI_RELU, "ae_gemm_bf16: bad epilogue %d", epilogue);
    if (A2) {
        AE_REQUIRE(Ksplit > 0 && Ksplit < K && Ksplit % 8 == 0 && lda2 % 8 == 0 && aligned16(A2),
                   "ae_gemm_bf16: bad two-source split (Ksplit=%d, K=%d)", Ksplit, K);
    }
    if (epilogue == EPI_GEGLU) {
        AE_REQUIRE(N % 32 == 0 && !residual && !addvec && !out_f32, "ae_gemm_bf16: GEGLU needs N %% 32 == 0, bf16 out, no residual");
    }
    if (residual) AE_REQUIRE(ldr % 4 == 0 && (reinterpret_cast<uintptr_t>(residual) & 7) == 0, "ae_gemm_bf16: residual alignment");
    if (addvec) AE_REQUIRE(rows_per_batch > 0, "ae_gemm_bf16: rows_per_batch must be > 0 with addvec");
    a = GemmArgs{};
    a.A = (const bf16_t*)A; a.A2 = (const bf16_t*)A2; a.W = (const bf16_t*)W; a.C = C;
    a.bias = bias; a.res = (const bf16_t*)residual; a.addvec = addvec;
    a.M = M; a.N = N; a.K = K; a.Ksplit = A2 ? Ksplit : K;
    a.lda = lda; a.lda2 = lda2; a.ldw = ldw; a.ldc = ldc; a.ldr = ldr; a.ldav = addvec_ld > 0 ? addvec_ld : N;
    a.epi = epilogue; a.out_f32 = out_f32; a.rows_per_batch = rows_per_batch > 0 ? rows_per_batch : 1;
    a.splitk = 1; a.partial = nullptr; a.colstats = colstats;
    a.a_bytes = (unsigned)((((long)M - 1) * lda + (A2 ? Ksplit : K)) * 2);
    a.a2_bytes = A2 ? (unsigned)((((long)M - 1) * lda2 + (K - Ksplit)) * 2) : 0u;
    a.w_bytes = (unsigned)((((long)N - 1) * ldw + K) * 2);
    AE_REQUIRE(((long)M * lda * 2) < (1L << 31) && ((long)N * ldw * 2) < (1L << 31) && (!A2 || ((long)M * lda2 * 2) < (1L << 31)),
               "ae_gemm_bf16: operands must be smaller than 2 GiB");
    if (x.rowstats_out || x.ln_stats) {
        const int n_out = epilogue == EPI_GEGLU ? N / 2 : N;
        AE_REQUIRE(N % 64 == 0 && n_out % 8 == 0 && ldc % 8 == 0 && (!residual || (ldr % 8 == 0 && aligned16(residual))),
                   "ae_gemm_ln_bf16: N %% 64 == 0 and 16-byte aligned output / residual rows");
// ... 192 lines not shown
```

### anyedit_amd/ldm/modules/attention.py

```python
import os

import torch
import torch.nn as nn

from anyedit_amd import ops
from anyedit_amd.ldm.util import default, exists
from anyedit_amd.ldm.modules.diffusionmodules.util import Linear, Conv2d, LayerNorm, checkpoint

BF16 = torch.bfloat16
_FF_TAIL = os.environ.get("AE_FF_TAIL", "1") != "0"
_SEG2_160 = os.environ.get("AE_ATTN_SEG2_160", "1") != "0"


def zero_module(module):
    for p in module.parameters():
        p.detach().zero_()
    return module


class _GN6(nn.GroupNorm):

    def _affine(self):
        if ops.cache_stale(self, "_pk", self.weight, self.bias):
            self._pk = (self.weight.detach().float().contiguous(), self.bias.detach().float().contiguous())
        return self._pk

    def repack(self):
        self._pk = None

    def rows(self, x, B, HW, colstats=None):
        g, b = self._affine()
        return ops.groupnorm(x, g, b, B, HW, self.eps, silu=False, groups=self.num_groups, colstats=colstats)

    def forward(self, x):
        B, C, H, W = x.shape
        return ops.rows_to_nchw(self.rows(ops.nchw_to_rows(x), B, H * W), B, H, W, out_dtype=x.dtype)


def Normalize(in_channels):
    return _GN6(num_groups=32, num_channels=in_channels, eps=1e-6, affine=True)


class GEGLU(nn.Module):

    def __init__(self, dim_in, dim_out):
        super().__init__()
        self.proj = Linear(dim_in, dim_out * 2)
        self._pk = None

    def repack(self):
        self._pk = None
        self._pkln = None

    def _packed_ln(self, norm):
        if ops.cache_stale(self, "_pkln", self.proj.weight, self.proj.bias, norm.weight, norm.bias):
            self._pkln = ops.pack_ln_fold(self.proj.weight, self.proj.bias, norm.weight, norm.bias, geglu=True)
        return self._pkln

    def rows(self, x, norm=None, rowstats=None):
        if ops._TAPE is not None and ops._TAPE.active:
            if norm is not None:
                x = norm.rows(x)
            if ops.cache_stale(self, "_pk_plain", self.proj.weight, self.proj.bias):
                self._pk_plain = (ops.pack_linear(self.proj.weight), self.proj.bias.detach().float().contiguous())
            w, b = self._pk_plain
            return ops.geglu(ops.gemm(x, w, b))
        if ops.cache_stale(self, "_pk", self.proj.weight, self.proj.bias):
            self._pk = ops.pack_geglu(self.proj.weight, self.proj.bias)
        w, b = self._pk
        if norm is not None and rowstats is not None and ops.ln_fold_plan(x.shape[0], w.shape[0], x.shape[1], ops.EPI_GEGLU, 2):
            wq, s, c = self._packed_ln(norm)
            return ops.gemm_ln(x, rowstats, wq, s, c, norm.eps, epilogue=ops.EPI_GEGLU)
        if norm is not None:
            g, be = norm._affine()
            return ops.ln_gemm(x, g, be, norm.eps, w, b, epilogue=ops.EPI_GEGLU)
        return ops.gemm(x, w, b, epilogue=ops.EPI_GEGLU)

    def forward(self, x):
        shp = x.shape
        return self.rows(x.reshape(-1, shp[-1]).to(BF16).contiguous()).reshape(*shp[:-1], -1).to(x.dtype)


class FeedForward(nn.Module):

    def __init__(self, dim, dim_out=None, mult=4, glu=False, dropout=0.):
        super().__init__()
        inner_dim = int(dim * mult)
        dim_out = default(dim_out, dim)
        self.glu = glu
        project_in = GEGLU(dim, inner_dim) if glu else nn.Sequential(Linear(dim, inner_dim), nn.GELU())
        self.net = nn.Sequential(project_in, nn.Dropout(dropout), Linear(inner_dim, dim_out))

    def repack(self):
        self._pkf = None

    def fused_ok(self, M, C):
        return self.glu and ops.ff_fused_ok(M, C, self.net[2].weight.shape[1])

    def rows(self, x, residual=None, norm=None, rowstats=None, tail=None):
        if norm is not None and self.fused_ok(x.shape[0], x.shape[1]):
            proj, ff2 = self.net[0].proj, self.net[2]
            if ops.cache_stale(self, "_pkf", proj.weight, proj.bias, ff2.weight, ff2.bias):
                w1, b1 = ops.pack_geglu(proj.weight, proj.bias)
                self._pkf = (w1, b1, ops.pack_ff2_fused(ff2.weight), None if ff2.bias is None else ff2.bias.detach().float().contiguous())
            w1, b1, w2img, b2 = self._pkf
            g, be = norm._affine()
            if tail is not None:
                w3, b3, res3, cs = tail
                return ops.ff_fused(x, g, be, norm.eps, w1, b1, w2img, b2, residual=residual, w3=w3, b3=b3, residual3=res3, colstats=cs)
            return ops.ff_fused(x, g, be, norm.eps, w1, b1, w2img, b2, residual=residual)
        assert tail is None, "FeedForward.rows: the projection tail goes with the fused launch only"
        if not self.glu:
            if norm is not None:
                x = norm.rows(x)
            return self.net[2].rows(self.net[0][0].rows(x, epilogue=ops.EPI_GELU), residual=residual)
        return self.net[2].rows(self.net[0].rows(x, norm=norm, rowstats=rowstats), residual=residual)

    def forward(self, x):
        shp = x.shape
        return self.rows(x.reshape(-1, shp[-1]).to(BF16).contiguous()).reshape(shp).to(x.dtype)


class CrossAttention(nn.Module):

    def __init__(self, query_dim, context_dim=None, heads=8, dim_head=64, dropout=0.):
        super().__init__()
        inner_dim = dim_head * heads
        self.is_self = context_dim is None
        context_dim = default(context_dim, query_dim)
        self.scale = dim_head ** -0.5
        self.heads = heads
        self.dim_head = dim_head
        self.to_q = Linear(query_dim, inner_dim, bias=False)
        self.to_k = Linear(context_dim, inner_dim, bias=False)
        self.to_v = Linear(context_dim, inner_dim, bias=False)
        self.to_out = nn.Sequential(Linear(inner_dim, query_dim), nn.Dropout(dropout))
        self._pk = None

    def repack(self):
        self._pk = None
        self._pkx = None
        self._pkln_q = self._pkln_qkv = None

    def _packed_ln(self, wname, norm):
        attr = "_pkln_" + wname
        mods = (self.to_q, self.to_k, self.to_v) if wname == "qkv" else (self.to_q,)
        if ops.cache_stale(self, attr, *(m.weight for m in mods), norm.weight, norm.bias):
            w = torch.cat([m.weight.detach().float() for m in mods], 0)
            setattr(self, attr, ops.pack_ln_fold(w, None, norm.weight, norm.bias))
        return getattr(self, attr)

    def _packed(self):
        if ops.cache_stale(self, "_pk", self.to_q.weight, self.to_k.weight, self.to_v.weight):
            wq, wk, wv = (ops.pack_linear(m.weight) for m in (self.to_q, self.to_k, self.to_v))
            pk = {"dev": self.to_q.weight.device, "q": wq, "kv": torch.cat([wk, wv], 0).contiguous()}
            if wq.shape[1] == wk.shape[1]:
                pk["qkv"] = torch.cat([wq, wk, wv], 0).contiguous()
            self._pk = pk
        return self._pk

    def project_kv(self, ctx_rows):
        return ops.gemm(ctx_rows, self._packed()["kv"])

    def rows(self, x, B, N, context_rows=None, Nk=None, kv=None, key_mask=None, residual=None, adapter=None, norm=None, rowstats=None,
             out_rowstats=None):
        h, d = self.heads, self.dim_head
        inner = h * d
        pk = self._packed()

        def proj(wname):
            if norm is None:
                return ops.gemm(x, pk[wname])
            if rowstats is not None and ops.ln_fold_plan(x.shape[0], pk[wname].shape[0], x.shape[1], ops.EPI_NONE, 2):
                wq, s, c = self._packed_ln(wname, norm)
                return ops.gemm_ln(x, rowstats, wq, s, c, norm.eps)
            g, be = norm._affine()
            return ops.ln_gemm(x, g, be, norm.eps, pk[wname])

        if context_rows is None and kv is None:
            qkv = proj("qkv")
            s = (N * 3 * inner, d, 3 * inner)
            o = ops.attention(qkv, qkv[:, inner:], qkv[:, 2 * inner:], B, h, N, N, d, self.scale, s, s, s, key_mask=key_mask)
        else:
            q = proj("q")
            if kv is None:
                kv = self.project_kv(context_rows)
            Nk = kv.shape[0] // B
            qs = (N * inner, d, inner)
            ks = (Nk * 2 * inner, d, 2 * inner)
            if adapter is not None and (d <= 96 or (d == 160 and _SEG2_160)) and key_mask is None:
                kv_ip, gate = adapter
                T_ip = kv_ip.shape[0] // B
                ks_ip = (T_ip * 2 * inner, d, 2 * inner)
                seg2 = (kv_ip, kv_ip[:, inner:], T_ip, ks_ip, ks_ip, gate)
                o = ops.attention(q, kv, kv[:, inner:], B, h, N, Nk, d, self.scale, qs, ks, ks, seg2=seg2)
            else:
                o = ops.attention(q, kv, kv[:, inner:], B, h, N, Nk, d, self.scale, qs, ks, ks, key_mask=key_mask)
                if adapter is not None:
                    kv_ip, gate = adapter
                    T_ip = kv_ip.shape[0] // B
                    ks_ip = (T_ip * 2 * inner, d, 2 * inner)
                    ops.attention(q, kv_ip, kv_ip[:, inner:], B, h, N, T_ip, d, self.scale, qs, ks_ip, ks_ip, out=o,
                                  out_scale=gate, accumulate=True)
        return self.to_out[0].rows(o.reshape(B * N, inner), residual=residual, rowstats=out_rowstats)

    def forward(self, x, context=None, mask=None):
        B, N, C = x.shape
        xr = x.reshape(B * N, C).to(BF16).contiguous()
        ctx = None
        if context is not None:
            ctx = context.reshape(-1, context.shape[-1]).to(BF16).contiguous()
        km = None
        if exists(mask):
            km = mask.reshape(B, -1).to(torch.uint8).contiguous()
        if ctx is None and not self.is_self:
            raise ValueError("CrossAttention built with context_dim needs a context of that width")
        if ctx is not None and self.is_self:
            y = self.rows(xr, B, N, context_rows=ctx, key_mask=km)
        else:
            y = self.rows(xr, B, N, context_rows=ctx, key_mask=km)
        return y.reshape(B, N, -1).to(x.dtype)


class MemoryEfficientCrossAttention(CrossAttention):
    """attention.py:197-243 — same operator; the xformers call site (:233) is `ops.attention_bhnd`."""


class BasicTransformerBlock(nn.Module):
    ATTENTION_MODES = {"softmax": CrossAttention, "softmax-xformers": MemoryEfficientCrossAttention,
                       "softmax-hip": CrossAttention}

    def __init__(self, dim, n_heads, d_head, dropout=0., context_dim=None, gated_ff=True, checkpoint=True,
                 disable_self_attn=False):
        super().__init__()
        attn_cls = self.ATTENTION_MODES["softmax-hip"]
        self.disable_self_attn = disable_self_attn
        self.attn1 = attn_cls(query_dim=dim, heads=n_heads, dim_head=d_head, dropout=dropout,
                              context_dim=context_dim if self.disable_self_attn else None)
        self.ff = FeedForward(dim, dropout=dropout, glu=gated_ff)
        self.attn2 = attn_cls(query_dim=dim, context_dim=context_dim, heads=n_heads, dim_head=d_head, dropout=dropout)
        self.norm1 = LayerNorm(dim)
        self.norm2 = LayerNorm(dim)
        self.norm3 = LayerNorm(dim)
        self.checkpoint = checkpoint

    def rows(self, x, B, N, context_rows=None, kv_cache=None, rowstats=None, tail=None):
        tape = ops._TAPE
        if self.checkpoint and tape is not None and tape.active:
            return tape.checkpoint(lambda: self._rows(x, B, N, context_rows, kv_cache))
        return self._rows(x, B, N, context_rows, kv_cache, rowstats, tail)

    def takes_tail(self, M, C):
        return _FF_TAIL and self.ff.fused_ok(M, C)

    def _fold_plan(self, M, C):
        key = (M, C, ops._LN_FOLD, ops._TAPE is not None and ops._TAPE.active)
        if getattr(self, "_fold_key", None) != key:
            inner1 = self.attn1.heads * self.attn1.dim_head
            inner2 = self.attn2.heads * self.attn2.dim_head
            n1 = inner1 if (self.disable_self_attn and not self.attn1.is_self) else 3 * inner1
            f1 = ops.ln_fold_plan(M, n1, C, ops.EPI_NONE, 2)
            f2 = ops.ln_fold_plan(M, inner2, C, ops.EPI_NONE, 2) and ops.ln_fold_plan(M, C, inner1, ops.EPI_NONE, 1)
            f3 = self.ff.glu and not self.ff.fused_ok(M, C) and ops.ln_fold_plan(M, self.ff.net[0].proj.weight.shape[0], C, ops.EPI_GEGLU, 2) \
                and ops.ln_fold_plan(M, C, inner2, ops.EPI_NONE, 1)
            self._fold_key, self._fold = key, (f1, f2, f3)
        return self._fold

    def wants_rowstats(self, M, C):
        return self._fold_plan(M, C)[0]

    def _rows(self, x, B, N, context_rows=None, kv_cache=None, rowstats=None, tail=None):
        c1 = context_rows if self.disable_self_attn else None
        M, C = x.shape
        f1, f2, f3 = self._fold_plan(M, C)
        kv2, adapter = None, None
        st2 = ops.rowstats_buffer(M, C, x.device) if f2 else None
        st3 = ops.rowstats_buffer(M, C, x.device) if f3 else None
        x = self.attn1.rows(x, B, N, context_rows=c1, residual=x, norm=self.norm1, rowstats=rowstats if f1 else None, out_rowstats=st2)
        if kv_cache is not None and context_rows is not None:
            key = id(self.attn2)
            kv2 = kv_cache.get(key)
            if kv2 is None:
                kv2 = self.attn2.project_kv(context_rows)
                if not (ops._TAPE is not None and ops._TAPE.active):
                    kv_cache[key] = kv2
            adapter = kv_cache.get(("adapter", key))
            if callable(adapter):
                adapter = adapter()
        x = self.attn2.rows(x, B, N, context_rows=context_rows, kv=kv2, residual=x, adapter=adapter, norm=self.norm2, rowstats=st2, out_rowstats=st3)
        x = self.ff.rows(x, residual=x, norm=self.norm3, rowstats=st3, tail=tail)
        return x

    def forward(self, x, context=None):
        B, N, C = x.shape
        ctx = None if context is None else context.reshape(-1, context.shape[-1]).to(BF16).contiguous()
        y = self.rows(x.reshape(B * N, C).to(BF16).contiguous(), B, N, context_rows=ctx)
        return y.reshape(B, N, C).to(x.dtype)

    _forward = forward


class SpatialTransformer(nn.Module):

    def __init__(self, in_channels, n_heads, d_head, depth=1, dropout=0., context_dim=None, disable_self_attn=False,
                 use_linear=False, use_checkpoint=True):
        super().__init__()
        if exists(context_dim) and not isinstance(context_dim, list):
            context_dim = [context_dim] * depth
        if context_dim is None:
            context_dim = [None] * depth
        self.in_channels = in_channels
        inner_dim = n_heads * d_head
        self.norm = Normalize(in_channels)
        if not use_linear:
            self.proj_in = Conv2d(in_channels, inner_dim, kernel_size=1, stride=1, padding=0)
        else:
            self.proj_in = Linear(in_channels, inner_dim)
        self.transformer_blocks = nn.ModuleList(
            [BasicTransformerBlock(inner_dim, n_heads, d_head, dropout=dropout, context_dim=context_dim[d],
                                   disable_self_attn=disable_self_attn, checkpoint=use_checkpoint) for d in range(depth)])
        if not use_linear:
            self.proj_out = zero_module(Conv2d(inner_dim, in_channels, kernel_size=1, stride=1, padding=0))
        else:
            self.proj_out = zero_module(Linear(in_channels, inner_dim))
        self.use_linear = use_linear

    def rows(self, x, B, H, W, context_rows=None, kv_cache=None, colstats=None, out_colstats=None):
        if isinstance(context_rows, (list, tuple)):
            ctxs = list(context_rows)
        else:
            ctxs = [context_rows] * len(self.transformer_blocks)
        N = H * W
        h = self.norm.rows(x, B, N, colstats=colstats)
        pin = self.proj_in._packed()
        M, Ci = h.shape[0], pin["w"].shape[0]
        st = None
        if self.transformer_blocks[0].wants_rowstats(M, Ci) and ops.ln_fold_plan(M, Ci, h.shape[1], ops.EPI_NONE, 1):
            st = ops.rowstats_buffer(M, Ci, h.device)
        h = ops.gemm(h, pin["w"], pin["b"], rowstats=st)
        pout = self.proj_out._packed()
        last = len(self.transformer_blocks) - 1
        tail_ok = self.transformer_blocks[last].takes_tail(M, Ci) and pout["w"].shape == (Ci, Ci) and x.shape[1] == Ci
        for i, blk in enumerate(self.transformer_blocks):
            tail = (pout["w"], pout["b"], x, out_colstats) if (tail_ok and i == last) else None
            h = blk.rows(h, B, N, context_rows=ctxs[i], kv_cache=kv_cache, rowstats=st if i == 0 else None, tail=tail)
        if tail_ok:
            return h
        return ops.gemm(h, pout["w"], pout["b"], residual=x, colstats=out_colstats)

    def forward(self, x, context=None):
        B, C, H, W = x.shape
        if isinstance(context, list):
            ctx = [None if c is None else c.reshape(-1, c.shape[-1]).to(BF16).contiguous() for c in context]
        else:
            ctx = None if context is None else context.reshape(-1, context.shape[-1]).to(BF16).contiguous()
        y = self.rows(ops.nchw_to_rows(x), B, H, W, context_rows=ctx)
        return ops.rows_to_nchw(y, B, H, W, out_dtype=x.dtype)
```

### anyedit_amd/ldm/modules/diffusionmodules/openaimodel.py

```python
from abc import abstractmethod
import math

import torch
import torch.nn as nn

from anyedit_amd import ops
from anyedit_amd.ldm.util import exists
from anyedit_amd.ldm.modules.attention import SpatialTransformer
from anyedit_amd.ldm.modules.diffusionmodules.util import avg_pool_nd, conv_nd, linear, normalization, zero_module

BF16 = torch.bfloat16


class TimestepBlock(nn.Module):

    @abstractmethod
    def forward(self, x, emb):
        """Apply the module to `x` given `emb` timestep embeddings."""


class Feat:
    __slots__ = ("t", "B", "H", "W", "t2", "st", "st2")

    def __init__(self, t, B, H, W, t2=None, st=None, st2=None):
        self.t, self.B, self.H, self.W, self.t2, self.st, self.st2 = t, B, H, W, t2, st, st2

    def materialize(self):
        if self.t2 is not None:
            self.t = ops.concat_channels(self.t, self.t2)
            self.t2 = None
            self.st = self.st2 = None
        return self.t


def _stats_for(B, H, W, C, device):
    return ops.colstats_buffer(B * H * W, C, device) if ops.want_colstats(H * W) else None


class EmbPack:
    __slots__ = ("silu", "all", "offsets")

    def __init__(self, silu, all_out=None, offsets=None):
        self.silu, self.all, self.offsets = silu, all_out, offsets or {}


class TimestepEmbedSequential(nn.Sequential, TimestepBlock):

    def rows(self, f, emb_silu, context_rows=None, kv_cache=None):
        for layer in self:
            if isinstance(layer, TimestepBlock):
                f = layer.rows(f, emb_silu)
            elif isinstance(layer, SpatialTransformer):
                x_st = f.st if f.t2 is None else None
                x = f.materialize()
                st = _stats_for(f.B, f.H, f.W, x.shape[1], x.device)
                f = Feat(layer.rows(x, f.B, f.H, f.W, context_rows=context_rows, kv_cache=kv_cache, colstats=x_st, out_colstats=st),
                         f.B, f.H, f.W, st=st)
            elif isinstance(layer, AttentionBlock):
                x_st = f.st if f.t2 is None else None
                f = Feat(layer.rows(f.materialize(), f.B, f.H * f.W, colstats=x_st), f.B, f.H, f.W)
            else:
                f = layer.rows(f)
        return f

    def forward(self, x, emb, context=None):
        for layer in self:
            if isinstance(layer, TimestepBlock):
                x = layer(x, emb)
            elif isinstance(layer, SpatialTransformer):
                x = layer(x, context)
            else:
                x = layer(x)
        return x


class Upsample(nn.Module):

    def __init__(self, channels, use_conv, dims=2, out_channels=None, padding=1):
        super().__init__()
        self.channels = channels
        self.out_channels = out_channels or channels
        self.use_conv = use_conv
        self.dims = dims
        if dims != 2:
            raise NotImplementedError("Upsample: only dims=2 (the 1-D / 3-D forms of openaimodel.py:108-112 have no caller in AnyEdit)")
        if use_conv:
            self.conv = conv_nd(dims, self.channels, self.out_channels, 3, padding=padding)

    def rows(self, f):
        if not self.use_conv:
            y, Ho, Wo = ops.resample2x_rows(f.materialize(), f.B, f.H, f.W)
            return Feat(y, f.B, Ho, Wo)
        Ho, Wo = self.conv.out_hw(f.H, f.W, upsample2x=True)
        st = _stats_for(f.B, Ho, Wo, self.out_channels, f.t.device)
        y, Ho, Wo = self.conv.rows(f.materialize(), f.B, f.H, f.W, upsample2x=True, colstats=st)
        return Feat(y, f.B, Ho, Wo, st=st)

    def forward(self, x):
        assert x.shape[1] == self.channels
        B, C, H, W = x.shape
        f = self.rows(Feat(ops.nchw_to_rows(x), B, H, W))
        return ops.rows_to_nchw(f.t, B, f.H, f.W, out_dtype=x.dtype)


class Downsample(nn.Module):

    def __init__(self, channels, use_conv, dims=2, out_channels=None, padding=1):
        super().__init__()
        self.channels = channels
        self.out_channels = out_channels or channels
        self.use_conv = use_conv
        self.dims = dims
        if dims != 2:
            raise NotImplementedError("Downsample: only dims=2 (the 1-D / 3-D forms of openaimodel.py:146 have no caller in AnyEdit)")
        if use_conv:
            self.op = conv_nd(dims, self.channels, self.out_channels, 3, stride=2, padding=padding)
        else:
            assert self.channels == self.out_channels
            self.op = avg_pool_nd(dims, kernel_size=2, stride=2)

    def rows(self, f):
        if not self.use_conv:
            y, Ho, Wo = self.op.rows(f.materialize(), f.B, f.H, f.W)
            return Feat(y, f.B, Ho, Wo)
        Ho, Wo = self.op.out_hw(f.H, f.W)
        st = _stats_for(f.B, Ho, Wo, self.out_channels, f.t.device)
        y, Ho, Wo = self.op.rows(f.materialize(), f.B, f.H, f.W, colstats=st)
        return Feat(y, f.B, Ho, Wo, st=st)

    def forward(self, x):
        assert x.shape[1] == self.channels
        B, C, H, W = x.shape
        f = self.rows(Feat(ops.nchw_to_rows(x), B, H, W))
        return ops.rows_to_nchw(f.t, B, f.H, f.W, out_dtype=x.dtype)


class ResBlock(TimestepBlock):

    def __init__(self, channels, emb_channels, dropout, out_channels=None, use_conv=False, use_scale_shift_norm=False,
                 dims=2, use_checkpoint=False, up=False, down=False):
        super().__init__()
        self.channels = channels
        self.emb_channels = emb_channels
        self.dropout = dropout
        self.out_channels = out_channels or channels
        self.use_conv = use_conv
        self.use_checkpoint = use_checkpoint
        self.use_scale_shift_norm = use_scale_shift_norm
        self.in_layers = nn.Sequential(normalization(channels), nn.SiLU(), conv_nd(dims, channels, self.out_channels, 3, padding=1))
        self.updown = up or down
        self.up, self.down = bool(up), bool(down) and not up
        if up:
            self.h_upd, self.x_upd = Upsample(channels, False, dims), Upsample(channels, False, dims)
        elif down:
            self.h_upd, self.x_upd = Downsample(channels, False, dims), Downsample(channels, False, dims)
        else:
            self.h_upd = self.x_upd = nn.Identity()
        self.emb_layers = nn.Sequential(nn.SiLU(), linear(emb_channels, 2 * self.out_channels if use_scale_shift_norm else self.out_channels))
        self.out_layers = nn.Sequential(normalization(self.out_channels), nn.SiLU(), nn.Dropout(p=dropout),
                                        zero_module(conv_nd(dims, self.out_channels, self.out_channels, 3, padding=1)))
        if self.out_channels == channels:
            self.skip_connection = nn.Identity()
        elif use_conv:
            self.skip_connection = conv_nd(dims, channels, self.out_channels, 3, padding=1)
        else:
            self.skip_connection = conv_nd(dims, channels, self.out_channels, 1)

    def rows(self, f, emb_silu):
        tape = ops._TAPE
        if self.use_checkpoint and tape is not None and tape.active:
            return Feat(tape.checkpoint(lambda: self._rows(f, emb_silu).t), f.B, f.H, f.W)
        return self._rows(f, emb_silu)

    def _rows(self, f, emb_silu):
        B, H, W = f.B, f.H, f.W
        if isinstance(emb_silu, EmbPack) and id(self) in emb_silu.offsets:
            off = emb_silu.offsets[id(self)]
            emb_out = emb_silu.all[:, off:off + self.emb_layers[1].out_features]
        else:
            silu = emb_silu.silu if isinstance(emb_silu, EmbPack) else emb_silu
            emb_out = self.emb_layers[1].rows(silu, out_f32=True)
        dev = f.t.device
        ssn = self.use_scale_shift_norm
        h = self.in_layers[0].rows(f.t, B, H * W, silu=True, x2=f.t2, colstats=f.st, colstats2=f.st2)
        whole = (lambda: f.t if f.t2 is None else ops.concat_channels(f.t, f.t2))
        Ho, Wo, xs = H, W, None
        if self.up:
            Ho, Wo = 2 * H, 2 * W
            xs, _, _ = ops.resample2x_rows(whole(), B, H, W)
        elif self.down:
            h, Ho, Wo = ops.resample2x_rows(h, B, H, W, down=True)
            xs, _, _ = ops.resample2x_rows(whole(), B, H, W, down=True)
        conv1, norm2 = self.in_layers[2], self.out_layers[0]
        st1 = _stats_for(B, Ho, Wo, self.out_channels, dev)
        if self.up:
            h, _, _ = conv1.rows(h, B, H, W, addvec=None if ssn else emb_out, upsample2x=True, colstats=st1)
        else:
            h, _, _ = conv1.rows(h, B, Ho, Wo, addvec=None if ssn else emb_out, colstats=st1)
        if ssn:
            h = ops.scale_shift_rows(norm2.rows(h, B, Ho * Wo, silu=False, colstats=st1), emb_out, B, Ho * Wo, silu=True)
        else:
            h = norm2.rows(h, B, Ho * Wo, silu=True, colstats=st1)
        if isinstance(self.skip_connection, nn.Identity):
            res = whole() if xs is None else xs
        elif self.skip_connection.kernel_size[0] == 1 and xs is None:
            res, _, _ = self.skip_connection.rows(f.t, B, H, W, a2=f.t2)
        else:
            res, _, _ = self.skip_connection.rows(whole() if xs is None else xs, B, Ho, Wo)
        st = _stats_for(B, Ho, Wo, self.out_channels, dev)
        y, _, _ = self.out_layers[3].rows(h, B, Ho, Wo, residual=res, colstats=st)
        return Feat(y, B, Ho, Wo, st=st)

    def forward(self, x, emb):
        B, C, H, W = x.shape
        f = self.rows(Feat(ops.nchw_to_rows(x), B, H, W), ops.silu_to_bf16(emb))
        return ops.rows_to_nchw(f.t, B, f.H, f.W, out_dtype=x.dtype)

    _forward = forward


class _QKVAttentionBase(nn.Module):

    def __init__(self, n_heads):
        super().__init__()
        self.n_heads = n_heads

    def _offsets(self, ch):
        raise NotImplementedError

    def rows(self, qkv, B, T):
        width = qkv.shape[1]
        assert width % (3 * self.n_heads) == 0
        ch = width // (3 * self.n_heads)
        (oq, ok, ov), hs = self._offsets(ch)
        st = (T * width, hs, width)
        return ops.attention(qkv[:, oq:], qkv[:, ok:], qkv[:, ov:], B, self.n_heads, T, T, ch, 1.0 / math.sqrt(ch), st, st, st).reshape(B * T, self.n_heads * ch)

    def forward(self, qkv):
        bs, width, length = qkv.shape
        y = self.rows(ops.nchw_to_rows(qkv.reshape(bs, width, length, 1)), bs, length)
        return ops.rows_to_nchw(y, bs, length, 1, out_dtype=qkv.dtype).reshape(bs, -1, length)


class QKVAttentionLegacy(_QKVAttentionBase):

    def _offsets(self, ch):
        return (0, ch, 2 * ch), 3 * ch


class QKVAttention(_QKVAttentionBase):

    def _offsets(self, ch):
        return (0, self.n_heads * ch, 2 * self.n_heads * ch), ch


class AttentionBlock(nn.Module):

    def __init__(self, channels, num_heads=1, num_head_channels=-1, use_checkpoint=False, use_new_attention_order=False):
        super().__init__()
        self.channels = channels
        if num_head_channels == -1:
            self.num_heads = num_heads
        else:
            assert channels % num_head_channels == 0, f"q,k,v channels {channels} is not divisible by num_head_channels {num_head_channels}"
            self.num_heads = channels // num_head_channels
        self.use_checkpoint = use_checkpoint
        self.norm = normalization(channels)
        self.qkv = conv_nd(1, channels, channels * 3, 1)
        self.attention = QKVAttention(self.num_heads) if use_new_attention_order else QKVAttentionLegacy(self.num_heads)
        self.proj_out = zero_module(conv_nd(1, channels, channels, 1))

    def rows(self, x, B, T, colstats=None):
        h = self.norm.rows(x, B, T, silu=False, colstats=colstats)
        return self.proj_out.rows(self.attention.rows(self.qkv.rows(h), B, T), residual=x)

    def forward(self, x):
        b, c = x.shape[:2]
        T = int(x.numel() // (b * c))
        y = self.rows(ops.nchw_to_rows(x.reshape(b, c, T, 1)), b, T)
        return ops.rows_to_nchw(y, b, T, 1, out_dtype=x.dtype).reshape(x.shape)

    _forward = forward


class UNetModel(nn.Module):

    def __init__(self, image_size, in_channels, model_channels, out_channels, num_res_blocks, attention_resolutions,
                 dropout=0, channel_mult=(1, 2, 4, 8), conv_resample=True, dims=2, num_classes=None, use_checkpoint=False,
                 use_fp16=False, num_heads=-1, num_head_channels=-1, num_heads_upsample=-1, use_scale_shift_norm=False,
                 resblock_updown=False, use_new_attention_order=False, use_spatial_transformer=False, transformer_depth=1,
                 context_dim=None, n_embed=None, legacy=True, disable_self_attentions=None, num_attention_blocks=None,
                 disable_middle_self_attn=False, use_linear_in_transformer=False):
        super().__init__()
        if use_spatial_transformer:
            assert context_dim is not None, "use_spatial_transformer needs context_dim (openaimodel.py:474-475)"
        if context_dim is not None:
            assert use_spatial_transformer, "a cross-attention context_dim needs use_spatial_transformer (openaimodel.py:477-478)"
            if not isinstance(context_dim, int):
                context_dim = list(context_dim)
        if dims != 2:
            raise NotImplementedError("dims != 2: the 1-D / 3-D UNets of openaimodel.py have no caller in AnyEdit")
        if num_classes is not None and not isinstance(num_classes, int) and num_classes != "continuous":
            raise ValueError(f"num_classes must be None, an int or 'continuous' (openaimodel.py:533-540), got {num_classes!r}")
        if num_heads_upsample == -1:
            num_heads_upsample = num_heads
        if num_heads == -1:
            assert num_head_channels != -1, "Either num_heads or num_head_channels has to be set"
        if num_head_channels == -1:
            assert num_heads != -1, "Either num_heads or num_head_channels has to be set"
        self.image_size = image_size
        self.in_channels = in_channels
        self.model_channels = model_channels
        self.out_channels = out_channels
        if isinstance(num_res_blocks, int):
            self.num_res_blocks = len(channel_mult) * [num_res_blocks]
        else:
            if len(num_res_blocks) != len(channel_mult):
                raise ValueError("provide num_res_blocks either as an int or as a per-level list")
            self.num_res_blocks = list(num_res_blocks)
        if disable_self_attentions is not None:
            assert len(disable_self_attentions) == len(channel_mult)
        if num_attention_blocks is not None:
            assert len(num_attention_blocks) == len(self.num_res_blocks)
        self.attention_resolutions = attention_resolutions
        self.dropout = dropout
        self.channel_mult = channel_mult
        self.conv_resample = conv_resample
        self.num_classes = num_classes
        self.use_checkpoint = use_checkpoint
        self.dtype = torch.float32
        self.num_heads = num_heads
        self.num_head_channels = num_head_channels
        self.num_heads_upsample = num_heads_upsample
        self.predict_codebook_ids = n_embed is not None

        def heads_for(ch, nh):
            if num_head_channels == -1:
                return nh, ch // nh
            return ch // num_head_channels, num_head_channels

        def make_st(ch, nh, level, is_middle=False):
            if not use_spatial_transformer:
                d_h = num_head_channels if (num_head_channels != -1 or legacy) else ch // num_heads
                return AttentionBlock(ch, use_checkpoint=use_checkpoint, num_heads=nh, num_head_channels=d_h, use_new_attention_order=use_new_attention_order)
            n_h, d_h = heads_for(ch, nh)
            if legacy:
                d_h = ch // n_h
            dsa = disable_middle_self_attn if is_middle else (disable_self_attentions[level] if exists(disable_self_attentions) else False)
            return SpatialTransformer(ch, n_h, d_h, depth=transformer_depth, context_dim=context_dim, disable_self_attn=dsa,
                                      use_linear=use_linear_in_transformer, use_checkpoint=use_checkpoint)

        time_embed_dim = model_channels * 4
        self.time_embed = nn.Sequential(linear(model_channels, time_embed_dim), nn.SiLU(), linear(time_embed_dim, time_embed_dim))
        if num_classes is not None:
            self.label_emb = nn.Embedding(num_classes, time_embed_dim) if isinstance(num_classes, int) else nn.Linear(1, time_embed_dim)
        self.input_blocks = nn.ModuleList([TimestepEmbedSequential(conv_nd(dims, in_channels, model_channels, 3, padding=1))])
        self._feature_size = model_channels
        input_block_chans = [model_channels]
        ch = model_channels
        ds = 1
        for level, mult in enumerate(channel_mult):
            for nr in range(self.num_res_blocks[level]):
                layers = [ResBlock(ch, time_embed_dim, dropout, out_channels=mult * model_channels, dims=dims,
                                   use_checkpoint=use_checkpoint, use_scale_shift_norm=use_scale_shift_norm)]
                ch = mult * model_channels
                if ds in attention_resolutions:
                    if not exists(num_attention_blocks) or nr < num_attention_blocks[level]:
                        layers.append(make_st(ch, num_heads, level))
                self.input_blocks.append(TimestepEmbedSequential(*layers))
                self._feature_size += ch
                input_block_chans.append(ch)
            if level != len(channel_mult) - 1:
                out_ch = ch
                self.input_blocks.append(TimestepEmbedSequential(
                    ResBlock(ch, time_embed_dim, dropout, out_channels=out_ch, dims=dims, use_checkpoint=use_checkpoint,
                             use_scale_shift_norm=use_scale_shift_norm, down=True)
                    if resblock_updown else Downsample(ch, conv_resample, dims=dims, out_channels=out_ch)))
                ch = out_ch
                input_block_chans.append(ch)
                ds *= 2
                self._feature_size += ch
        self.middle_block = TimestepEmbedSequential(
            ResBlock(ch, time_embed_dim, dropout, dims=dims, use_checkpoint=use_checkpoint, use_scale_shift_norm=use_scale_shift_norm),
            make_st(ch, num_heads, 0, is_middle=True),
            ResBlock(ch, time_embed_dim, dropout, dims=dims, use_checkpoint=use_checkpoint, use_scale_shift_norm=use_scale_shift_norm))
        self._feature_size += ch
        self.output_blocks = nn.ModuleList([])
        for level, mult in list(enumerate(channel_mult))[::-1]:
            for i in range(self.num_res_blocks[level] + 1):
                ich = input_block_chans.pop()
                layers = [ResBlock(ch + ich, time_embed_dim, dropout, out_channels=model_channels * mult, dims=dims,
                                   use_checkpoint=use_checkpoint, use_scale_shift_norm=use_scale_shift_norm)]
                ch = model_channels * mult
                if ds in attention_resolutions:
                    if not exists(num_attention_blocks) or i < num_attention_blocks[level]:
                        layers.append(make_st(ch, num_heads_upsample, level))
                if level and i == self.num_res_blocks[level]:
                    out_ch = ch
                    layers.append(ResBlock(ch, time_embed_dim, dropout, out_channels=out_ch, dims=dims, use_checkpoint=use_checkpoint,
                                           use_scale_shift_norm=use_scale_shift_norm, up=True)
                                  if resblock_updown else Upsample(ch, conv_resample, dims=dims, out_channels=out_ch))
                    ds //= 2
                self.output_blocks.append(TimestepEmbedSequential(*layers))
                self._feature_size += ch
        self.out = nn.Sequential(normalization(ch), nn.SiLU(), zero_module(conv_nd(dims, model_channels, out_channels, 3, padding=1)))
        if self.predict_codebook_ids:
            self.id_predictor = nn.Sequential(normalization(ch), conv_nd(dims, model_channels, n_embed, 1))

    def repack(self):
        self._emb_pk = None
        for m in self.modules():
            if m is not self and hasattr(m, "repack"):
                m.repack()

    def _emb_pack(self, emb_silu):
        blocks = self.__dict__.get("_emb_blocks")
        if blocks is None:
            blocks = self.__dict__["_emb_blocks"] = [m for m in self.modules() if isinstance(m, ResBlock)]
        pk = getattr(self, "_emb_pk", None)
        if ops.cache_stale(self, "_emb_pk", *[p for b in blocks for p in (b.emb_layers[1].weight, b.emb_layers[1].bias)]):
            w = torch.cat([ops.pack_linear(b.emb_layers[1].weight) for b in blocks], 0).contiguous()
            bias = torch.cat([b.emb_layers[1].bias.detach().float() for b in blocks], 0).contiguous()
            offsets, off = {}, 0
            for b in blocks:
                offsets[id(b)] = off
                off += b.emb_layers[1].out_features
            pk = (w, bias, offsets)
            self._emb_pk = pk
        w, bias, offsets = pk
        return EmbPack(emb_silu, ops.gemm(emb_silu, w, bias, out_f32=True), offsets)

    def load_state_dict(self, *a, **k):
        r = super().load_state_dict(*a, **k)
        self.repack()
        return r

    def context_rows(self, context):
        if isinstance(context, (list, tuple)):
            return [self.context_rows(c) for c in context]
        return context.reshape(-1, context.shape[-1]).to(BF16).contiguous()

    def _label_rows(self, y, device):
        if isinstance(self.num_classes, int):
            return self.label_emb.weight.detach().float()[y.reshape(-1).long().to(device)].contiguous()
        w, b = self.label_emb.weight.detach().float(), self.label_emb.bias.detach().float().contiguous()
        yp = torch.zeros(y.shape[0], 16, dtype=torch.float32, device=device)
        yp[:, 0] = y.reshape(-1).to(device=device, dtype=torch.float32)
        wp = torch.zeros(w.shape[0], 16, dtype=torch.float32, device=device)
        wp[:, 0] = w[:, 0]
        return ops.linear_f32(yp, wp, b)

    def time_embedding_rows(self, timesteps):
        assert self.num_classes is None, "class-conditional models add label_emb(y) per sample: use forward_rows(y=...)"
        t_emb = ops.timestep_embedding(timesteps, self.model_channels)
        emb = self.time_embed[0].rows(t_emb, epilogue=ops.EPI_SILU)
        return self._emb_pack(self.time_embed[2].rows(emb, epilogue=ops.EPI_SILU))

    def forward_rows(self, x, timesteps, context_rows, kv_cache=None, y=None, emb_pack=None):
        B, C, H, W = x.shape
        assert (y is not None) == (self.num_classes is not None), "must specify y if and only if the model is class-conditional"
        if emb_pack is not None:
            assert y is None and emb_pack.all is not None and emb_pack.all.shape[0] == B and emb_pack.all.is_contiguous()
            emb_silu = emb_pack
        else:
            t_emb = ops.timestep_embedding(timesteps, self.model_channels)
            emb = self.time_embed[0].rows(t_emb, epilogue=ops.EPI_SILU)
            if y is None:
                emb_silu = self.time_embed[2].rows(emb, epilogue=ops.EPI_SILU)
            else:
                assert y.shape[0] == B
                e32 = self.time_embed[2].rows(emb, out_f32=True)
                lab = self._label_rows(y, e32.device)
                emb_silu = ops.silu_to_bf16(ops.lincomb([(e32, 1.0), (lab, 1.0)]))
            emb_silu = self._emb_pack(emb_silu)
        f = Feat(ops.nchw_to_rows(x, (C + 7) // 8 * 8), B, H, W)
        hs = []
        for module in self.input_blocks:
            if isinstance(module[0], TimestepBlock) or isinstance(module[0], (Downsample, Upsample)) or len(module) > 1:
                f = module.rows(f, emb_silu, context_rows, kv_cache)
            else:
                st = _stats_for(B, H, W, module[0].out_channels, f.t.device)
                stem, _, _ = module[0].rows(f.t, B, H, W, colstats=st)
                f = Feat(stem, B, H, W, st=st)
            hs.append(f)
        f = self.middle_block.rows(f, emb_silu, context_rows, kv_cache)
        for module in self.output_blocks:
            skip = hs.pop()
            st_a = f.st if f.t2 is None else None
            st_b = skip.st if skip.t2 is None else None
            f = Feat(f.materialize(), f.B, f.H, f.W, t2=skip.materialize(), st=st_a, st2=st_b)
            f = module.rows(f, emb_silu, context_rows, kv_cache)
        if self.predict_codebook_ids:
            h = self.id_predictor[0].rows(f.materialize(), f.B, f.H * f.W, silu=False, colstats=f.st if f.t2 is None else None)
            logits, _, _ = self.id_predictor[1].rows(h, f.B, f.H, f.W, out_f32=True)
            return ops.rows_to_nchw(logits, f.B, f.H, f.W, out_dtype=torch.float32)
        h = self.out[0].rows(f.materialize(), f.B, f.H * f.W, silu=True, colstats=f.st if f.t2 is None else None)
        eps, _, _ = self.out[2].rows(h, f.B, f.H, f.W, out_f32=True)
        return ops.rows_to_nchw(eps, f.B, f.H, f.W, out_dtype=torch.float32)

    def forward(self, x, timesteps=None, context=None, y=None, **kwargs):
        assert (y is not None) == (self.num_classes is not None), "must specify y if and only if the model is class-conditional"
        out = self.forward_rows(x, timesteps, self.context_rows(context) if context is not None else None, y=y)
        return out.to(x.dtype) if x.dtype != torch.float32 else out
```

### anyedit_amd/ldm/modules/diffusionmodules/util.py

```python

import numpy as np
import torch
import torch.nn as nn

from anyedit_amd import ops


def make_beta_schedule(schedule, n_timestep, linear_start=1e-4, linear_end=2e-2, cosine_s=8e-3):
    if schedule == "linear":
        betas = torch.linspace(linear_start ** 0.5, linear_end ** 0.5, n_timestep, dtype=torch.float64) ** 2
    elif schedule == "cosine":
        timesteps = torch.arange(n_timestep + 1, dtype=torch.float64) / n_timestep + cosine_s
        alphas = timesteps / (1 + cosine_s) * np.pi / 2
        alphas = torch.cos(alphas).pow(2)
        alphas = alphas / alphas[0]
        betas = 1 - alphas[1:] / alphas[:-1]
        betas = torch.clamp(betas, min=0, max=0.999)
    elif schedule == "sqrt_linear":
        betas = torch.linspace(linear_start, linear_end, n_timestep, dtype=torch.float64)
    elif schedule == "sqrt":
        betas = torch.linspace(linear_start, linear_end, n_timestep, dtype=torch.float64) ** 0.5
    else:
        raise ValueError(f"schedule '{schedule}' unknown.")
    return betas.numpy()


def make_ddim_timesteps(ddim_discr_method, num_ddim_timesteps, num_ddpm_timesteps, verbose=True):
    if ddim_discr_method == "uniform":
        c = num_ddpm_timesteps // num_ddim_timesteps
        ddim_timesteps = np.asarray(list(range(0, num_ddpm_timesteps, c)))
    elif ddim_discr_method == "quad":
        ddim_timesteps = ((np.linspace(0, np.sqrt(num_ddpm_timesteps * .8), num_ddim_timesteps)) ** 2).astype(int)
    else:
        raise NotImplementedError(f'There is no ddim discretization method called "{ddim_discr_method}"')
    steps_out = ddim_timesteps + 1
    if verbose:
        print(f"Selected timesteps for ddim sampler: {steps_out}")
    return steps_out


def make_ddim_sampling_parameters(alphacums, ddim_timesteps, eta, verbose=True):
    alphas = alphacums[ddim_timesteps]
    alphas_prev = np.asarray([alphacums[0]] + alphacums[ddim_timesteps[:-1]].tolist())
    sigmas = eta * np.sqrt((1 - alphas_prev) / (1 - alphas) * (1 - alphas / alphas_prev))
    if verbose:
        print(f"Selected alphas for ddim sampler: a_t: {alphas}; a_(t-1): {alphas_prev}")
        print(f"For the chosen value of eta, which is {eta}, this results in the following sigma_t schedule for ddim sampler {sigmas}")
    return sigmas, alphas, alphas_prev


def extract_into_tensor(a, t, x_shape):
    b, *_ = t.shape
    out = a.gather(-1, t)
    return out.reshape(b, *((1,) * (len(x_shape) - 1)))


def checkpoint(func, inputs, params, flag):
    return func(*inputs)


def timestep_embedding(timesteps, dim, max_period=10000, repeat_only=False):
    if repeat_only:
        return timesteps[:, None].repeat(1, dim)
    return ops.timestep_embedding(timesteps, dim, max_period, out_f32=True)


def zero_module(module):
    for p in module.parameters():
        p.detach().zero_()
    return module


def noise_like(shape, device, repeat=False):
    if repeat:
        return torch.randn((1, *shape[1:]), device=device).repeat(shape[0], *((1,) * (len(shape) - 1)))
    return torch.randn(shape, device=device)


class _Packed:

    def repack(self):
        self._pk = None

    def _packed(self):
        if ops.cache_stale(self, "_pk", self.weight, getattr(self, "bias", None)):
            pk = self._pack()
            pk["device"] = self.weight.device
            self._pk = pk
        return self._pk


class Linear(nn.Linear, _Packed):

    def _pack(self):
        return {"w": ops.pack_linear(self.weight), "b": None if self.bias is None else self.bias.detach().float().contiguous()}

    def rows(self, x, residual=None, epilogue=ops.EPI_NONE, out_f32=False, a2=None, rowstats=None):
        pk = self._packed()
        if rowstats is not None:
            return ops.gemm(x, pk["w"], pk["b"], residual=residual, epilogue=epilogue, out_f32=out_f32, a2=a2, rowstats=rowstats)
        return ops.gemm(x, pk["w"], pk["b"], residual=residual, epilogue=epilogue, out_f32=out_f32, a2=a2)

    def forward(self, x):
        shp = x.shape
        y = self.rows(x.reshape(-1, shp[-1]).to(torch.bfloat16).contiguous())
        return y.reshape(*shp[:-1], -1).to(x.dtype)


class Conv2d(nn.Conv2d, _Packed):

    def _pack(self):
        k = self.kernel_size[0]
        b = None if self.bias is None else self.bias.detach().float().contiguous()
        if k == 1:
            return {"w": ops.pack_linear(self.weight), "b": b}
        if k == 3 and self.padding[0] == 1 and self.stride[0] in (1, 2) and self.groups == 1 and self.dilation[0] == 1:
            return {"w": ops.pack_conv3x3(self.weight), "b": b}
        raise NotImplementedError(f"anyedit_amd Conv2d: unsupported configuration k={k} stride={self.stride} padding={self.padding}")

    def rows(self, x, B, H, W, addvec=None, residual=None, upsample2x=False, out_f32=False, a2=None, colstats=None):
        pk = self._packed()
        if self.kernel_size[0] == 1:
            return ops.gemm(x, pk["w"], pk["b"], residual=residual, out_f32=out_f32, a2=a2, colstats=colstats), H, W
        if addvec is None and residual is None and not out_f32 and a2 is None and ops.stem_im2col_ok(self.in_channels, self.stride[0], upsample2x):
            if "w_taps" not in pk:
                pk["w_taps"] = ops.pack_conv3x3_taps8(self.weight)
            return ops.gemm(ops.im2col3x3_c8(x, B, H, W), pk["w_taps"], pk["b"], colstats=colstats), H, W
        if upsample2x and addvec is None and residual is None and not out_f32 and a2 is None and \
                ops.up2_subpixel_ok(self.in_channels, self.out_channels, H, W, colstats is not None) and self.stride[0] == 1:
            if "w_up2" not in pk:
                pk["w_up2"] = ops.pack_conv3x3_up2(self.weight)
            return ops.conv3x3_up2(x, pk["w_up2"], pk["b"], B, H, W, colstats=colstats)
        Ho, Wo = self.out_hw(H, W, upsample2x)
        ko = ops.conv_k_order(B * Ho * Wo, self.in_channels, self.out_channels, self.stride[0], upsample2x)
        w = pk["w"]
        if ko:
            if "w_kmajor" not in pk:
                pk["w_kmajor"] = ops.pack_conv3x3(self.weight, k_order=1)
            w = pk["w_kmajor"]
        return ops.conv3x3(x, w, pk["b"], B, H, W, addvec=addvec, residual=residual, stride=self.stride[0],
                           upsample2x=upsample2x, out_f32=out_f32, colstats=colstats, k_order=ko)

    def out_hw(self, H, W, upsample2x=False):
        if self.kernel_size[0] == 1:
            return H, W
        Hv, Wv = (2 * H, 2 * W) if upsample2x else (H, W)
        return (Hv - 1) // self.stride[0] + 1, (Wv - 1) // self.stride[0] + 1

    def forward(self, x):
        B, C, H, W = x.shape
        cpad = (C + 7) // 8 * 8
        if cpad != C and self.kernel_size[0] == 1:
            raise NotImplementedError("1x1 conv with channels not a multiple of 8")
        y, Ho, Wo = self.rows(ops.nchw_to_rows(x, cpad), B, H, W)
        return ops.rows_to_nchw(y, B, Ho, Wo, out_dtype=x.dtype)


class GroupNorm32(nn.GroupNorm):

    def _affine(self):
        if ops.cache_stale(self, "_pk", self.weight, self.bias):
            self._pk = (self.weight.detach().float().contiguous(), self.bias.detach().float().contiguous())
        return self._pk

    def repack(self):
        self._pk = None

    def rows(self, x, B, HW, silu=False, x2=None, colstats=None, colstats2=None):
        g, b = self._affine()
        return ops.groupnorm(x, g, b, B, HW, self.eps, silu=silu, groups=self.num_groups, x2=x2, colstats=colstats, colstats2=colstats2)

    def forward(self, x):
        B, C, H, W = x.shape
        y = self.rows(ops.nchw_to_rows(x), B, H * W)
        return ops.rows_to_nchw(y, B, H, W, out_dtype=x.dtype)


class LayerNorm(nn.LayerNorm):
    def _affine(self):
        if ops.cache_stale(self, "_pk", self.weight, self.bias):
            self._pk = (self.weight.detach().float().contiguous(), self.bias.detach().float().contiguous())
        return self._pk

    def repack(self):
        self._pk = None

    def rows(self, x):
        g, b = self._affine()
        return ops.layernorm(x, g, b, self.eps)

    def forward(self, x):
        shp = x.shape
        return self.rows(x.reshape(-1, shp[-1]).to(torch.bfloat16).contiguous()).reshape(shp).to(x.dtype)


class Conv1d(nn.Conv1d, _Packed):

    def _pack(self):
        if self.kernel_size[0] != 1 or self.stride[0] != 1 or self.padding[0] != 0 or self.groups != 1:
            raise NotImplementedError(f"anyedit_amd Conv1d: only the 1-wide pointwise form (k={self.kernel_size} stride={self.stride} padding={self.padding})")
        return {"w": ops.pack_linear(self.weight), "b": None if self.bias is None else self.bias.detach().float().contiguous()}

    def rows(self, x, residual=None):
        pk = self._packed()
        return ops.gemm(x, pk["w"], pk["b"], residual=residual)

    def forward(self, x):
        B, C, T = x.shape
        y = self.rows(ops.nchw_to_rows(x.reshape(B, C, T, 1)))
        return ops.rows_to_nchw(y, B, T, 1, out_dtype=x.dtype).reshape(B, -1, T)


def conv_nd(dims, *args, **kwargs):
    if dims == 1:
        return Conv1d(*args, **kwargs)
    if dims == 2:
        return Conv2d(*args, **kwargs)
    raise ValueError(f"unsupported dimensions: {dims} (the AnyEdit hot path is 2-D)")


def linear(*args, **kwargs):
    return Linear(*args, **kwargs)


def normalization(channels):
    return GroupNorm32(32, channels)


class AvgPool2d(nn.AvgPool2d):

    def __init__(self, kernel_size=2, stride=None, **kw):
        super().__init__(kernel_size, stride, **kw)
        ks = self.kernel_size if isinstance(self.kernel_size, int) else self.kernel_size[0]
        st = self.stride if isinstance(self.stride, int) else self.stride[0]
        if ks != 2 or st != 2 or kw:
            raise NotImplementedError("AvgPool2d: only the 2x2 / stride-2 mean of openaimodel.py:146-155")

    def rows(self, x, B, H, W):
        return ops.resample2x_rows(x, B, H, W, down=True)

    def forward(self, x):
        B, C, H, W = x.shape
        y, Ho, Wo = self.rows(ops.nchw_to_rows(x), B, H, W)
        return ops.rows_to_nchw(y, B, Ho, Wo, out_dtype=x.dtype)


def avg_pool_nd(dims, *args, **kwargs):
    if dims == 2:
        return AvgPool2d(*args, **kwargs)
    raise ValueError(f"unsupported dimensions: {dims} (the AnyEdit hot path is 2-D)")
```

### anyedit_amd/ops.py

```python
import torch

import collections
import ctypes
import os
import threading

from ._lib import lib, check as _check

BF16 = torch.bfloat16
EPI_NONE, EPI_GELU, EPI_GEGLU, EPI_SILU, EPI_RELU = 0, 1, 2, 3, 4


def _s():
    return torch.cuda.current_stream().cuda_stream


def _p(t):
    return None if t is None else t.data_ptr()


_live = threading.local()


def _tmp(t):
# ... 1239 lines not shown
                         f"got {tuple(pred_logits.shape)}")
    if tuple(pred_boxes.shape) != (B, nq, 4) or not pred_boxes.is_contiguous():
        raise ValueError(f"gdino_ground: pred_boxes must be contiguous [{B}, {nq}, 4], got {tuple(pred_boxes.shape)}")
    dev = pred_logits.device
    shapes = ((B,), (B, nq), (B, nq), (B, nq, 4), (B, nq, T // 32))
    dts = (torch.int32, torch.int32, torch.float32, torch.float32, torch.int32)
    if out is None:
        out = tuple(torch.empty(s, dtype=d, device=dev) for s, d in zip(shapes, dts))
    for t, s, d in zip(out, shapes, dts):
        _chk(t, d, "gdino_ground.out")
        if tuple(t.shape) != s or not t.is_contiguous():
            raise ValueError(f"gdino_ground: an output must be contiguous {list(s)}, got {tuple(t.shape)}")
    count, idx, scores, boxes, bits = out
    check(lib.ae_gdino_ground(_p(pred_logits), _p(pred_boxes), float(box_threshold), float(text_threshold), _p(count), _p(idx), _p(scores), _p(boxes), _p(bits),
                              B, nq, T, _s()), "ae_gdino_ground")
    return out


HED_STEM_CMAX = 512
HED_LEVELS = 5
HED_MIN_SIDE = 1 << (HED_LEVELS - 1)
HED_MAX_SIDE = 16384


def _out_buf(out, dtype, shape, name, device):
    if out is None:
        return torch.empty(shape, dtype=dtype, device=device)
    return _target(out, dtype, shape, name)


def hed_stem(x, norm, w, bias, out=None):
    if not x.is_cuda:
        raise ValueError("hed_stem.x: expected a GPU tensor (anyedit_amd has no CPU path)")
    if x.dim() != 4:
        raise ValueError(f"hed_stem: x must be uint8 [B, H, W, 3] or fp32 [B, 3, H, W], got shape {tuple(x.shape)}")
    if x.dtype == torch.uint8:
        B, H, W, C = x.shape
        sb, sh, sw, sc = x.stride()
    elif x.dtype == torch.float32:
        B, C, H, W = x.shape
        sb, sc, sh, sw = x.stride()
    else:
        raise TypeError(f"hed_stem.x: expected torch.uint8 [B, H, W, 3] or torch.float32 [B, 3, H, W], got {x.dtype}")
    if C != 3 or B < 1 or H < 1 or W < 1:
        raise ValueError(f"hed_stem: x must be uint8 [B, H, W, 3] or fp32 [B, 3, H, W], got shape {tuple(x.shape)}")
    norm = _dense(norm, torch.float32, "hed_stem.norm")
    w = _dense(w, torch.float32, "hed_stem.w", 4)
    bias = _dense(bias, torch.float32, "hed_stem.bias", 1)
    C1 = w.shape[0]
    if tuple(w.shape) != (C1, 3, 3, 3) or norm.numel() != 3 or bias.numel() != C1:
        raise ValueError(f"hed_stem: need w [C1, 3, 3, 3], norm of 3 values and bias [C1], got {tuple(w.shape)}, {tuple(norm.shape)}, {tuple(bias.shape)}")
    out = _out_buf(out, BF16, (B * H * W, C1), "hed_stem.out", x.device)
    check(lib.ae_hed_stem_bf16(_p(x), 1 if x.dtype == torch.float32 else 0, sb, sc, sh, sw, _p(norm), _p(w), _p(bias), _p(out), B, H, W, C1, _s()),
          "ae_hed_stem_bf16")
    return out, B, H, W


def relu_(x):
    _chk(x, BF16, "relu_.x")
    if not x.is_contiguous() or x.numel() == 0:
        raise ValueError("relu_: x must be a contiguous, non-empty tensor (the kernel writes it in place)")
    check(lib.ae_relu_bf16(_p(x), x.numel(), _s()), "ae_relu_bf16")
    return x


def hed_tail(y, wp, bp, B, H, W, pool=True, proj=None, pooled=None):
    _chk(y, BF16, "hed_tail.y", 2)
    C = y.shape[1]
    if y.shape[0] != B * H * W or not y.is_contiguous() or B < 1 or H < 1 or W < 1:
        raise ValueError(f"hed_tail: y must be contiguous [B*H*W, C] = [{B * H * W}, C], got {tuple(y.shape)}")
    wp = _dense(wp, torch.float32, "hed_tail.wp").reshape(-1)
    bp = _dense(bp, torch.float32, "hed_tail.bp").reshape(-1)
    if wp.numel() != C or bp.numel() != 1:
        raise ValueError(f"hed_tail: need {C} projection weights and one bias, got {wp.numel()} and {bp.numel()}")
    proj = _out_buf(proj, torch.float32, (B, H, W), "hed_tail.proj", y.device)
    if pool:
        if H < 2 or W < 2:
            raise ValueError(f"hed_tail: a {H} x {W} map has no 2x2 window to pool")
        pooled = _out_buf(pooled, BF16, (B * (H // 2) * (W // 2), C), "hed_tail.pooled", y.device)
    elif pooled is not None:
        raise ValueError("hed_tail: a pooled buffer was given with pool=False")
    check(lib.ae_hed_tail_bf16(_p(y), _p(wp), _p(bp), _p(proj), _p(pooled), B, H, W, C, _s()), "ae_hed_tail_bf16")
    return proj, pooled


def hed_fuse(sides, invert=True, out=None, logits=None, want_logits=False):
    if len(sides) != HED_LEVELS:
        raise ValueError(f"hed_fuse: expected {HED_LEVELS} side maps, got {len(sides)}")
    s0 = sides[0]
    _chk(s0, torch.float32, "hed_fuse.sides[0]")
    if s0.dim() == 4 and s0.shape[1] == 1:
        sides = [s.squeeze(1) if s.dim() == 4 else s for s in sides]
        s0 = sides[0]
    if s0.dim() != 3:
        raise ValueError(f"hed_fuse: side maps must be [B, h, w] or [B, 1, h, w], got {tuple(s0.shape)}")
    B, H, W = s0.shape
    if not (HED_MIN_SIDE <= H <= HED_MAX_SIDE and HED_MIN_SIDE <= W <= HED_MAX_SIDE):
        raise ValueError(f"hed_fuse: sides of {HED_MIN_SIDE} .. {HED_MAX_SIDE} pixels are covered, got {H} x {W}")
    dense = []
    for k, s in enumerate(sides):
        _chk(s, torch.float32, f"hed_fuse.sides[{k}]", 3)
        if tuple(s.shape) != (B, H >> k, W >> k):
            raise ValueError(f"hed_fuse: side map {k} must be [{B}, {H >> k}, {W >> k}], got {tuple(s.shape)}")
        dense.append(_tmp(s.contiguous()))
    out = _out_buf(out, torch.uint8, (B, H, W), "hed_fuse.out", s0.device)
    if want_logits or logits is not None:
        logits = _out_buf(logits, torch.float32, (B, H, W), "hed_fuse.logits", s0.device)
    check(lib.ae_hed_fuse(*[_p(s) for s in dense], _p(out), _p(logits), B, H, W, 1 if invert else 0, _s()), "ae_hed_fuse")
    return out if logits is None else (out, logits)


def rows_to_nchw_out(x, out):
    _chk(x, BF16, "rows_to_nchw_out.x", 2)
    if not out.is_cuda or out.dtype not in (torch.float32, BF16) or out.dim() != 4 or not out.is_contiguous():
        raise ValueError("rows_to_nchw_out: out must be a contiguous fp32 / bf16 [B, C, H, W] GPU tensor")
    B, C, H, W = out.shape
    if tuple(x.shape) != (B * H * W, C) or not x.is_contiguous():
        raise ValueError(f"rows_to_nchw_out: x must be a contiguous [{B * H * W}, {C}] buffer, got {tuple(x.shape)}")
    check(lib.ae_transpose_last2(_p(x), _p(out), B, H * W, C, H * W, 1, 1 if out.dtype == BF16 else 0, _s()), "ae_transpose_last2")
    return out


def nchw_to_rows(x, c_pad=None):
    B, C, H, W = x.shape
    x = x.contiguous()
    c_pad = c_pad or C
    out = torch.empty(B * H * W, c_pad, dtype=BF16, device=x.device)
    check(lib.ae_transpose_last2(_p(x), _p(out), B, C, H * W, c_pad, 1 if x.dtype == BF16 else 0, 1, _s()), "ae_transpose_last2")
    return out


def rows_to_nchw(x, B, H, W, out_dtype=torch.float32):
    if _TAPE is not None and _TAPE.active:
        return _TAPE.rows_to_nchw(x, B, H, W, out_dtype=out_dtype)
    C = x.shape[1]
    x = x.contiguous()
    out = torch.empty(B, C, H, W, dtype=out_dtype, device=x.device)
    check(lib.ae_transpose_last2(_p(x), _p(out), B, H * W, C, H * W, 1 if x.dtype == BF16 else 0,
                                 1 if out_dtype == BF16 else 0, _s()), "ae_transpose_last2")
    return out


def concat_channels(a, b):
    if _TAPE is not None and _TAPE.active:
        return _TAPE.concat_channels(a, b)
    a, b = _dense(a, BF16, "concat_channels.a", 2), _dense(b, BF16, "concat_channels.b", 2)
    if a.shape[0] != b.shape[0]:
        raise ValueError(f"concat_channels: {a.shape[0]} rows against {b.shape[0]}")
    out = torch.empty(a.shape[0], a.shape[1] + b.shape[1], dtype=BF16, device=a.device)
    check(lib.ae_concat_channels_bf16(_p(a), a.shape[1], _p(b), b.shape[1], _p(out), a.shape[0], _s()), "ae_concat_channels_bf16")
    return out


def split_channels(dy, ca, a=None, b=None, want_a=True, want_b=True):
    dy = _dense(dy, BF16, "split_channels.dy", 2)
    rows, C = dy.shape
    cb = C - ca
    if a is not None:
        _target(a, BF16, (rows, ca), "split_channels.a")
    if b is not None:
        _target(b, BF16, (rows, cb), "split_channels.b")
    da = a if a is not None else (torch.empty(rows, ca, dtype=BF16, device=dy.device) if want_a else None)
    db = b if b is not None else (torch.empty(rows, cb, dtype=BF16, device=dy.device) if want_b else None)
    check(lib.ae_split_channels_bf16(_p(dy), ca, cb, _p(da), _p(db), rows, int(a is not None), int(b is not None), _s()), "ae_split_channels_bf16")
    return da, db


def timestep_embedding(t, dim, max_period=10000.0, out_f32=False):
    B = t.shape[0]
    out = torch.empty(B, dim, dtype=torch.float32 if out_f32 else BF16, device=t.device)
    t_i64 = t if t.dtype == torch.int64 else None
    t_f32 = None if t_i64 is not None else t.float().contiguous()
    check(lib.ae_timestep_embedding(_p(t_i64), _p(t_f32), None if out_f32 else _p(out), _p(out) if out_f32 else None, B, dim,
                                    float(max_period), _s()), "ae_timestep_embedding")
    return out


def ddim_step(x, eps, coeffs, branches, s0=1.0, s1=0.0, noise=None, temperature=1.0, want_pred_x0=True, want_e=False):
    _chk(x, torch.float32, "ddim_step.x")
    _chk(eps, torch.float32, "ddim_step.eps")
    x = x.contiguous()
    eps = eps.contiguous()
    n = x.numel()
    if eps.numel() != branches * n:
        raise ValueError(f"ddim_step: eps has {eps.numel()} elements, expected {branches}*{n}")
    if noise is not None:
        noise = _dense(noise, torch.float32, "ddim_step.noise")
        if noise.numel() != n:
            raise ValueError(f"ddim_step: noise has {noise.numel()} elements, expected {n}")
    x_prev = torch.empty_like(x)
    pred_x0 = torch.empty_like(x) if want_pred_x0 else None
    s1m, sat, sap, dirc, sig = coeffs
    e_out = torch.empty_like(x) if want_e else None
    check(lib.ae_ddim_step_f32(_p(x), _p(eps), _p(noise), _p(x_prev), _p(pred_x0), _p(e_out), n, branches, s0, s1, s1m, sat, sap,
                               dirc, sig, temperature, _s()), "ae_ddim_step_f32")
    if want_e:
        return x_prev, pred_x0, e_out
    return x_prev, pred_x0


def ddim_encode_step(x, eps, cx, ce, branches=1, scale=1.0):
    _chk(x, torch.float32, "ddim_encode_step.x")
    _chk(eps, torch.float32, "ddim_encode_step.eps")
    x, eps = x.contiguous(), eps.contiguous()
    out = torch.empty_like(x)
    check(lib.ae_ddim_encode_step_f32(_p(x), _p(eps), _p(out), x.numel(), branches, float(scale), float(cx), float(ce), _s()),
          "ae_ddim_encode_step_f32")
    return out


def dpm_multistep(x, model_out, branches, scale, sigma_s, alpha_s, predict_x0=True, v_param=False, m_prev=None, update=None,
                  want_m=True):
    _chk(x, torch.float32, "dpm_multistep.x")
    _chk(model_out, torch.float32, "dpm_multistep.model_out")
    n = x.numel()
    if model_out.numel() != branches * n or not x.is_contiguous() or not model_out.is_contiguous():
        raise ValueError("dpm_multistep: model_out must hold `branches` contiguous copies of x's shape")
    m = torch.empty_like(x) if want_m else None
    xn = torch.empty_like(x) if update is not None else None
    a, b, c, inv_r0 = update if update is not None else (0.0, 0.0, 0.0, 0.0)
    check(lib.ae_dpm_multistep_f32(_p(x), _p(model_out), _p(m_prev), _p(m), _p(xn), n, branches, float(scale), 1 if v_param else 0,
                                   1 if predict_x0 else 0, float(sigma_s), float(alpha_s), 1 if update is not None else 0, float(a),
                                   float(b), float(c), float(inv_r0), _s()), "ae_dpm_multistep_f32")
    return m, xn


def plms_combine(e_t, old_eps):
    order = min(len(old_eps), 3)
    e_t = e_t.contiguous()
    olds = [t.contiguous() for t in old_eps[::-1][:3]] + [None, None, None]
    out = torch.empty_like(e_t)
    check(lib.ae_plms_combine_f32(_p(e_t), _p(olds[0]), _p(olds[1]), _p(olds[2]), _p(out), e_t.numel(), order, _s()), "ae_plms_combine_f32")
    return out


def plms_combine_first(e_t, e_t_next):
    out = torch.empty(e_t.shape, dtype=e_t.dtype, device=e_t.device)
    check(lib.ae_plms_combine_f32(_p(_tmp(e_t.contiguous())), _p(_tmp(e_t_next.contiguous())), None, None, _p(out), e_t.numel(), 0, _s()),
          "ae_plms_combine_f32")
    return out


def mask_blend_shape(mask, B, C, H, W):
    while mask.dim() < 4:
        mask = mask.unsqueeze(0)
    if mask.shape[1] == 1:
        return mask.expand(B, 1, H, W), B, C
    if mask.shape[1] == C:
        return mask.expand(B, C, H, W).reshape(B * C, 1, H, W), B * C, 1
    raise ValueError(f"mask_blend: mask of shape {tuple(mask.shape)} does not broadcast against [{B}, {C}, {H}, {W}]")


def mask_blend(img, x0, noise, mask, sqrt_ac, sqrt_one_minus_ac, ip2p_order=False):
    B, C, H, W = img.shape
    out = torch.empty(img.shape, dtype=img.dtype, device=img.device)
    m, Bk, Ck = mask_blend_shape(mask, B, C, H, W)
    check(lib.ae_mask_blend_f32(_p(_tmp(img.contiguous())), _p(_tmp(x0.contiguous())), _p(_tmp(noise.contiguous())), _p(_tmp(m.contiguous().float())),
                                _p(out), Bk, Ck, H * W, sqrt_ac, sqrt_one_minus_ac, 1 if ip2p_order else 0, _s()), "ae_mask_blend_f32")
    return out


def q_sample(x0, noise, sqrt_ac_t, sqrt_one_minus_ac_t):
    out = torch.empty(x0.shape, dtype=x0.dtype, device=x0.device)
    B = x0.shape[0]
    check(lib.ae_q_sample_f32(_p(_tmp(x0.contiguous())), _p(_tmp(noise.contiguous())), _p(_tmp(sqrt_ac_t.contiguous())),
                              _p(_tmp(sqrt_one_minus_ac_t.contiguous())), _p(out), B, x0.numel() // B, _s()), "ae_q_sample_f32")
    return out


def silu_to_bf16(x):
    x = x.contiguous()
    out = torch.empty(x.shape, dtype=BF16, device=x.device)
    check(lib.ae_silu_to_bf16(_p(x), 1 if x.dtype == BF16 else 0, _p(out), x.numel(), _s()), "ae_silu_to_bf16")
    return out


def add_bcast(x, p):
    x, p = _dense(x, BF16, "add_bcast.x"), _dense(p, BF16, "add_bcast.p")
    out = torch.empty_like(x)
    check(lib.ae_add_bcast_bf16(_p(x), _p(p), _p(out), x.numel(), p.numel(), _s()), "ae_add_bcast_bf16")
    return out


def _no_tape(what):
    if _TAPE is not None and _TAPE.active:
        raise NotImplementedError(f"{what}: forward only (no backward closure on the tape; the AnyEdit training step never builds it)")


def resample2x_rows(x, B, H, W, down=False):
    _no_tape("resample2x_rows")
    C = x.shape[1]
    if x.dtype != BF16 or not x.is_contiguous() or x.shape[0] != B * H * W or C % 8:
        raise ValueError(f"resample2x_rows: bf16 contiguous rows [B*H*W, C % 8 == 0] expected, got {tuple(x.shape)} {x.dtype}")
    Ho, Wo = (H // 2, W // 2) if down else (2 * H, 2 * W)
    out = torch.empty(B * Ho * Wo, C, dtype=BF16, device=x.device)
    check(lib.ae_resample2x_rows_bf16(_p(x), _p(out), B, H, W, C, 1 if down else 0, _s()), "ae_resample2x_rows_bf16")
    return out, Ho, Wo


def scale_shift_rows(x, emb, B, HW, silu=True):
    _no_tape("scale_shift_rows")
    C = x.shape[1]
    if (x.dtype != BF16 or not x.is_contiguous() or x.shape[0] != B * HW or C % 8 or emb.dtype != torch.float32 or tuple(emb.shape) != (B, 2 * C)
            or emb.stride(1) != 1):
        raise ValueError(f"scale_shift_rows: x bf16 rows [B*HW, C % 8 == 0], emb fp32 [B, 2C] expected, got {tuple(x.shape)} {x.dtype} / {tuple(emb.shape)} {emb.dtype}")
    out = torch.empty_like(x)
# ... 467 lines not shown

def expert_kv_wgrad(dy, x, experts, tokens, n_experts, out=None):
    B = dy.shape[0] // tokens
    N, Dc = dy.shape[1], x.shape[1]
    assert dy.dtype == BF16 and x.dtype == BF16 and dy.is_contiguous() and x.is_contiguous()
    if out is None:
        out = torch.empty(n_experts, N, Dc, dtype=torch.float32, device=dy.device)
    assert out.dtype == torch.float32 and out.is_contiguous() and out.numel() == n_experts * N * Dc
    ex = _tmp(_experts_i32(experts))
    check(lib.ae_expert_kv_wgrad(_p(dy), _p(x), _p(ex), _p(out), B, tokens, N, Dc, n_experts, _s()), "ae_expert_kv_wgrad")
    return out


class OpProfiler:

    def __init__(self):
        self.records = []

    def __enter__(self):
        global _PROF
        _PROF = self
        return self

    def __exit__(self, *a):
        global _PROF
        _PROF = None
        torch.cuda.synchronize()

    def summary(self, by_shape=False):
        agg = {}
        for label, flops, nbytes, e0, e1, nlaunch in self.records:
            if not by_shape:
                label = label.split("|")[0]
            ms = e0.elapsed_time(e1)
            a = agg.setdefault(label, {"calls": 0, "launches": 0, "ms": 0.0, "flops": 0.0, "bytes": 0.0})
            a["calls"] += 1
            a["launches"] += nlaunch
            a["ms"] += ms
            a["flops"] += flops
            a["bytes"] += nbytes
        for a in agg.values():
            a["avg_us"] = 1e3 * a["ms"] / a["calls"]
            a["tflops"] = a["flops"] / (a["ms"] * 1e-3) / 1e12 if a["ms"] > 0 else 0.0
            a["gbps"] = a["bytes"] / (a["ms"] * 1e-3) / 1e9 if a["ms"] > 0 else 0.0
        return agg


_PROF = None


def _wrap_profiled(fn, label_fn):
    def wrapped(*args, **kwargs):
        if _PROF is None:
            return fn(*args, **kwargs)
        e0, e1 = torch.cuda.Event(enable_timing=True), torch.cuda.Event(enable_timing=True)
        e0.record()
        out = fn(*args, **kwargs)
        e1.record()
        lab = label_fn(out, *args, **kwargs)
        if lab is not None:
            _PROF.records.append((lab[0], lab[1], lab[2], e0, e1, lab[3] if len(lab) > 3 else 1))
        return out
    wrapped.__doc__ = fn.__doc__
    return wrapped


def _gemm_label(_r, a, w, bias=None, residual=None, addvec=None, rows_per_batch=0, epilogue=EPI_NONE, out_f32=False, a2=None, **_):
    if _.get("rowstats") is not None:
        return None
    M, (N, K) = a.shape[0], w.shape
    nb = 2 * (M * K + N * K) + _r.numel() * _r.element_size() + (2 * M * N if residual is not None else 0)
    if a2 is None and addvec is None and not out_f32 and _rowpanel_ok(a, w, _r, residual, M, N, K, epilogue):
        return f"gemm_rowpanel_kernel<K=320{',geglu' if epilogue == EPI_GEGLU else ''}>|M={M} N={N}", 2.0 * M * N * K, nb
    p = gemm_plan(M, N, K, epilogue, a.shape[1] if a2 is not None else 0, out_f32, _.get("colstats") is not None)
    return f"gemm_kernel<{plan_label(p)},dense>|M={M} N={N} K={K}", 2.0 * M * N * K, float(nb), 1 + p.colstats


def _conv_label(_r, x, w, bias, B, H, W, addvec=None, residual=None, stride=1, upsample2x=False, out_f32=False, **_):
    y = _r[0]
    M, Cout, Cin = y.shape[0], w.shape[0], x.shape[1]
    nb = 2 * (x.numel() + 9 * Cin * Cout) + y.numel() * y.element_size() + (2 * y.numel() if residual is not None else 0)
    p = conv_plan(B, H, W, Cin, Cout, stride, upsample2x, out_f32, _.get("colstats") is not None, _.get("k_order", 0))
    return f"gemm_kernel<{plan_label(p)},conv3x3>|M={M} Cin={Cin} Cout={Cout} s{stride}{'u' if upsample2x else ''}", 2.0 * M * Cout * 9 * Cin, float(nb), 1 + p.reduce + p.colstats


def _attn_label(_r, q, k, v, B, H, Nq, Nk, D, *a, **kw):
    fast = D in (40, 80, 160) and kw.get("key_mask") is None and os.environ.get("AE_ATTN_FAST", "1") != "0" and \
        (D != 160 or os.environ.get("AE_ATTN_FAST160", "1") != "0") and \
        (kw.get("rel_h") is None or (D == 80 and ((kw.get("kW") == 64 and Nk % 64 == 0) or (kw.get("kH", 99) <= 16 and kw.get("kW", 99) <= 16))))
    seg2 = kw.get("seg2")
    skv = fast and kw.get("rel_h") is None and Nk <= 128 and (seg2 is None or seg2[2] <= 64) and os.environ.get("AE_ATTN_SKV", "1") != "0"
    name = ("attn_fast_kernel" if fast else "attn_kernel")
    return f"{name}<D={D}{',shortKV' if skv else ''}>|Nq={Nq} Nk={Nk}", 4.0 * B * H * Nq * Nk * D, 2.0 * B * H * D * (2 * Nq + 2 * Nk)


def _attn8_label(_r, q, k, v, B, H, Nq, Nk, D, *a, **kw):
    return f"fp8_attn_kernel<D={D}>+prepare|Nq={Nq} Nk={Nk}", 4.0 * B * H * Nq * Nk * D, 2.0 * B * H * D * (2 * Nq + 2 * Nk)


def _gn_label(_r, x, gamma, beta, B, HW, eps, silu=False, groups=32, x2=None, **_):
    nl = 2 if _.get("colstats") is not None and ((x2 is None) == (_.get("colstats2") is None)) else (1 if HW <= 256 and os.environ.get("AE_GN_SLAB", "1") != "0" else (2 if _GN_TAIL else 3))
    return f"groupnorm(stats+apply)|rows={_r.shape[0]} C={_r.shape[1]}", 0.0, 2.0 * _r.numel() * 2, nl


def _ln_label(_r, x, *a, **_):
    return f"layernorm_kernel|M={_r.shape[0]} C={_r.shape[1]}", 0.0, 2.0 * _r.numel() * 2


def _ln_gemm_label(_r, x, w, bias, residual, gamma, beta, eps, epilogue, o, M, N, K, colstats=None):
    nb = 2 * (M * K + N * K) + _r.numel() * 2 + (2 * M * N if residual is not None else 0)
    return f"gemm_rowpanel_kernel<K=320,LN{',geglu' if epilogue == EPI_GEGLU else ''}>|M={M} N={N}", 2.0 * M * N * K, nb


def _gemm_ln_label(_r, a, w, bias, residual, epilogue, out, M, N, K, rowstats_out, ln_stats, nparts, ln_colsum, eps):
    nb = 2 * (M * K + N * K) + _r.numel() * 2 + (2 * M * N if residual is not None else 0)
    tag = "rowstats" if rowstats_out is not None else "LNfold"
    p = gemm_plan(M, N, K, epilogue, ln_mode=1 if rowstats_out is not None else 2)
    if p.rowpanel:
        return f"gemm_rowpanel_kernel<K=320,{tag}{',geglu' if epilogue == EPI_GEGLU else ''}>|M={M} N={N}", 2.0 * M * N * K, nb
    return f"gemm_kernel<{plan_label(p)},dense,{tag}>|M={M} N={N} K={K}", 2.0 * M * N * K, float(nb)


def _up2_label(_r, x, w4, bias, B, H, W, **_):
    y = _r[0]
    Cout, Cin = w4.shape[1], x.shape[1]
    tl = plan_label(up2_plan(B, H, W, Cin, Cout, _.get("colstats") is not None))
    nb = 2 * (x.numel() + 16 * Cin * Cout) + 2 * y.numel()
    return f"gemm_kernel<{tl},conv3x3,up2x2>|M={y.shape[0]} Cin={Cin} Cout={Cout}", 2.0 * y.shape[0] * Cout * 4 * Cin, float(nb)


conv3x3_up2 = _wrap_profiled(conv3x3_up2, _up2_label)
ff_fused = _wrap_profiled(ff_fused, lambda _r, x, gamma, beta, eps, w1, b1, w2img, b2, residual=None, out=None, w3=None, b3=None, residual3=None, colstats=None: (
    f"ff_fused_kernel<C=320{',proj_out' if w3 is not None else ''}>|M={x.shape[0]} H={w1.shape[0] // 2}",
    2.0 * x.shape[0] * x.shape[1] * (3 * (w1.shape[0] // 2) + (x.shape[1] if w3 is not None else 0)),
    float(2 * (x.numel() * (2 + (residual is not None and residual is not x) + (residual3 is not None)) + w1.numel() + w2img.numel() + (w3.numel() if w3 is not None else 0))),
    2 if colstats is not None else 1))
_ln_gemm_fused = _wrap_profiled(_ln_gemm_launch, _ln_gemm_label)
_gemm_ln_launch = _wrap_profiled(_gemm_ln_launch, _gemm_ln_label)
gemm = _wrap_profiled(gemm, _gemm_label)
attention_fp8 = _wrap_profiled(attention_fp8, _attn8_label)
conv3x3 = _wrap_profiled(conv3x3, _conv_label)
attention = _wrap_profiled(attention, _attn_label)
groupnorm = _wrap_profiled(groupnorm, _gn_label)
layernorm = _wrap_profiled(layernorm, _ln_label)
expert_kv = _wrap_profiled(expert_kv, lambda _r, x, W, experts, tokens: (
    f"expert_kv_fwd_kernel|rows={x.shape[0]} N={W.shape[1]} Dc={W.shape[2]}", 2.0 * x.shape[0] * W.shape[1] * W.shape[2], 4.0 * (x.shape[0] // tokens) * W.shape[1] * W.shape[2]))
expert_kv_dgrad = _wrap_profiled(expert_kv_dgrad, lambda _r, dy, W, experts, tokens: (
    f"expert_kv_dgrad_kernel|rows={dy.shape[0]} N={W.shape[1]} Dc={W.shape[2]}", 2.0 * dy.shape[0] * W.shape[1] * W.shape[2], 4.0 * (dy.shape[0] // tokens) * W.shape[1] * W.shape[2]))
expert_kv_wgrad = _wrap_profiled(expert_kv_wgrad, lambda _r, dy, x, experts, tokens, n_experts, out=None: (
    f"expert_kv_wgrad_kernel|rows={dy.shape[0]} N={dy.shape[1]} Dc={x.shape[1]} E={n_experts}", 2.0 * dy.shape[0] * dy.shape[1] * x.shape[1], 4.0 * n_experts * dy.shape[1] * x.shape[1]))
hed_stem = _wrap_profiled(hed_stem, lambda _r, x, norm, w, bias, out=None: (
    f"hed_stem_kernel<{'u8' if x.dtype == torch.uint8 else 'f32'}>|M={_r[0].shape[0]} C1={_r[0].shape[1]}", 2.0 * 27 * _r[0].numel(),
    float(x.numel() * x.element_size() + 2 * _r[0].numel())))
relu_ = _wrap_profiled(relu_, lambda _r, x: (f"relu_bf16_kernel|n={x.numel()}", 0.0, 4.0 * x.numel()))
hed_tail = _wrap_profiled(hed_tail, lambda _r, y, wp, bp, B, H, W, pool=True, proj=None, pooled=None: (
    f"hed_tail_kernel<{'pool' if pool else 'last'}>|M={y.shape[0]} C={y.shape[1]}", 2.0 * y.numel(),
    float(2 * y.numel() + 4 * _r[0].numel() + (2 * _r[1].numel() if pool else 0))))
hed_fuse = _wrap_profiled(hed_fuse, lambda _r, sides, invert=True, out=None, logits=None, want_logits=False: (
    f"hed_fuse_kernel|B={sides[0].shape[0]} {sides[0].shape[-2]}x{sides[0].shape[-1]}", 0.0,
    float(4 * sum(s.numel() for s in sides) + sides[0].numel() * (1 + 4 * (want_logits or logits is not None)))))
```

### include/anyedit_hip.h

```cpp
#ifndef ANYEDIT_HIP_H
#define ANYEDIT_HIP_H

#ifdef __cplusplus
extern "C" {
#endif

#define AE_OK 0
#define AE_ERR_ARG (-1)
#define AE_ERR_LAUNCH (-2)
#define AE_ERR_UNSUPPORTED (-3)

#define AE_EPI_NONE 0
#define AE_EPI_GELU 1
#define AE_EPI_GEGLU 2
#define AE_EPI_SILU 3
#define AE_EPI_RELU 4

int ae_version(void);
const char* ae_last_error(void);
int ae_device_arch(char* buf, int n);
int ae_device_info(int* cus, long* hbm_bytes, int* clock_khz);

int ae_gemm_bf16(const void* A, long lda, const void* A2, long lda2, int Ksplit, const void* W, long ldw, void* C, long ldc,
                 int M, int N, int K, const float* bias, const void* residual, long ldr, const float* addvec, long addvec_ld,
                 int rows_per_batch, int epilogue, int out_f32, float* colstats, void* stream);

int ae_ln_gemm_supported(int M, int N, int K, int epilogue);
int ae_ln_gemm_bf16(const void* A, long lda, const void* W, long ldw, void* C, long ldc, int M, int N, int K, const float* bias,
                    const void* residual, long ldr, const float* ln_gamma, const float* ln_beta, float ln_eps, int epilogue,
                    float* colstats , void* stream);

int ae_gemm_ln_plan(int M, int N, int K, int epilogue, int mode);
int ae_gemm_ln_bf16(const void* A, long lda, const void* W, long ldw, void* C, long ldc, int M, int N, int K, const float* bias,
                    const void* residual, long ldr, int epilogue, float* rowstats_out, const float* ln_stats, int ln_parts,
                    const float* ln_colsum, float ln_eps, void* stream);

int ae_ff_fused_supported(int M, int C, int H);
int ae_ff_fused_bf16(const void* X, long ldx, const float* ln_gamma, const float* ln_beta, float ln_eps, const void* W1, long ldw1, const float* b1,
                     const void* W2img, const float* b2, const void* residual, long ldr, const void* W3, long ldw3, const float* b3,
                     const void* residual3, long ldr3, float* colstats, void* Y, long ldy, int M, int C, int H, void* stream);

long ae_conv3x3_workspace_floats(int B, int H, int W, int Cin, int Cout, int stride, int upsample2x);
int ae_conv3x3_bf16(const void* x, const void* w, const float* bias, const float* addvec, long addvec_ld, const void* residual,
                    void* y, int B, int H, int W, int Cin, int Cout, int stride, int upsample2x, int out_f32, float* workspace,
                    float* colstats , int k_order, void* stream);

int ae_conv3x3_up2_bf16(const void* x, const void* w4, const float* bias, void* y, int B, int H, int W, int Cin, int Cout,
                        float* colstats, void* stream);

#define AE_PLAN_INTS 19
int ae_gemm_plan(int M, int N, int K, int epilogue, int Ksplit, int out_f32, int colstats, int ln_mode, int* plan);
int ae_conv3x3_plan(int B, int H, int W, int Cin, int Cout, int stride, int upsample2x, int out_f32, int workspace, int colstats, int k_order,
                    int* plan);
int ae_conv3x3_up2_plan(int B, int H, int W, int Cin, int Cout, int colstats, int* plan);

int ae_groupnorm_rows_per_chunk(int HW, int C);
long ae_groupnorm_workspace_floats(int B, int HW, int C, int groups);
int ae_groupnorm_nhwc_bf16(const void* x, const void* x2, int C1, const float* gamma, const float* beta, void* y, int B, int HW,
                           int C, int groups, float eps, int act, float* workspace, int* counters, float* stat_out,
                           const float* colstats, const float* colstats2, void* stream);

int ae_layernorm_bf16(const void* x, const float* gamma, const float* beta, void* y, int M, int C, float eps, void* stream);

int ae_attn_fwd_bf16(const void* q, const void* k, const void* v, void* out, int B, int H, int Nq, int Nk, int D,
                     long q_sb, long q_sh, long q_sn, long k_sb, long k_sh, long k_sn, long v_sb, long v_sh, long v_sn,
                     long o_sb, long o_sh, long o_sn, float scale, const float* rel_h, const float* rel_w, int kH, int kW,
                     const unsigned char* key_mask, const float* out_scale, int accumulate, const void* k2, const void* v2,
                     int Nk2, long k2_sb, long k2_sh, long k2_sn, long v2_sb, long v2_sh, long v2_sn, const float* scale2,
                     float* lse, float* lse2, void* stream);
long ae_attn_fp8_workspace_bytes(int B, int H, int Nq, int Nk, int D);
int ae_attn_fwd_fp8(const void* q, const void* k, const void* v, void* out, int B, int H, int Nq, int Nk, int D, long q_sb, long q_sh,
                    long q_sn, long k_sb, long k_sh, long k_sn, long v_sb, long v_sh, long v_sn, long o_sb, long o_sh, long o_sn,
                    float scale, const float* rel_h, const float* rel_w, int kH, int kW, void* workspace, long workspace_bytes,
                    void* stream);
long ae_attn_bwd_workspace_floats(int B, int H, int Nq, int Nk, int D);
int ae_attn_bwd_bf16(const void* q, const void* k, const void* v, const void* dout, const void* out, const float* lse, float* delta, void* dq,
                     void* dk, void* dv, int B, int H, int Nq, int Nk, int D, long q_sb, long q_sh, long q_sn, long k_sb,
                     long k_sh, long k_sn, long v_sb, long v_sh, long v_sn, long o_sb, long o_sh, long o_sn, long dq_sb,
                     long dq_sh, long dq_sn, long dk_sb, long dk_sh, long dk_sn, long dv_sb, long dv_sh, long dv_sn,
                     float scale, const float* out_scale, int accumulate_dq, float* workspace, void* stream);
long ae_groupnorm_bwd_workspace_floats(int B, int HW, int C, int groups);
int ae_groupnorm_bwd_nhwc_bf16(const void* x, const void* x2, int C1, const float* gamma, const float* beta, const void* dy,
                               void* dx, void* dx2, int B, int HW, int C, int groups, float eps, int act, float* workspace,
                               int* counters, const float* stat_in, int accumulate, void* stream);
int ae_layernorm_bwd_bf16(const void* x, const float* gamma, const void* dy, void* dx, float* row_stat, int M, int C, float eps,
                          int accumulate, void* stream);
int ae_layernorm_param_grad_f32(const void* x, const void* dy, const float* row_stat, float* dgamma, float* dbeta, int M, int C,
                                void* stream);
int ae_add_bf16(const void* a, const void* b, void* y, long n, void* stream);
int ae_axpy_bf16(const void* a, const void* b, float alpha, void* y, long n, void* stream);
int ae_geglu_fwd_bf16(const void* h, void* y, long M, int F, void* stream);
int ae_geglu_bwd_bf16(const void* h, const void* dy, void* dh, long M, int F, void* stream);
int ae_sumpool2x2_bf16(const void* x, void* y, int B, int H, int W, int C, void* stream);
int ae_colsum_bf16_f32(const void* x, float* out, int M, int N, long ld, void* stream);
int ae_mse_grad_f32(const float* pred, const float* target, float* out, long n, float loss_scale, void* stream);
int ae_adamw_f32(float* param, const float* grad, float* exp_avg, float* exp_avg_sq, long n, float lr, float beta1, float beta2,
                 float eps, float weight_decay, int step, float grad_scale, void* stream);
int ae_rowsum_f32(const float* x, float* out, int rows, long n, void* stream);
int ae_scatter_add_rows_f32(const float* src, const int* code, float* dst, int B, int D, int n_rows, void* stream);
int ae_task_gate_bwd(const float* probs, const int* top1, const float* dgate, const float* Wg, int B, int Dt, int E, float* dte,
                     void* stream);
int ae_task_gate_wgrad(const float* probs, const int* top1, const float* dgate, const float* task_emb, const long* edit_code, int B,
                       int n_tasks, int Dt, int E, float* dWg, float* dbg, void* stream);

int ae_expert_kv_fwd(const void* x, const float* W, const int* experts, void* y, int B, int T, int N, int Dc, int E, void* stream);
int ae_expert_kv_dgrad_slices(int N);
int ae_expert_kv_dgrad(const void* dy, const float* W, const int* experts, void* dx, int B, int T, int N, int Dc, int E, float* partial,
                       void* stream);
int ae_expert_kv_wgrad(const void* dy, const void* x, const int* experts, float* dW, int B, int T, int N, int Dc, int E, void* stream);

int ae_transpose_last2(const void* in, void* out, int B, int X, int Y, int Xpad, int in_bf16, int out_bf16, void* stream);
int ae_concat_channels_bf16(const void* a, int Ca, const void* b, int Cb, void* y, long rows, void* stream);
int ae_im2col3x3_c8_bf16(const void* x, void* y, int B, int H, int W, void* stream);
int ae_split_channels_bf16(const void* y, int Ca, int Cb, void* a, void* b, long rows, int accumulate_a, int accumulate_b, void* stream);
int ae_timestep_embedding(const long* t_i64, const float* t_f32, void* out_bf16, float* out_f32, int B, int dim, float max_period,
                          void* stream);
int ae_ddim_step_f32(const float* x, const float* eps, const float* noise, float* x_prev, float* pred_x0, float* e_out, long n,
                     int branches, float s0, float s1, float sqrt_one_minus_at, float sqrt_at, float sqrt_a_prev, float dir_coef,
                     float sigma_t, float temperature, void* stream);
int ae_plms_combine_f32(const float* e_t, const float* old1, const float* old2, const float* old3, float* out, long n, int order,
                        void* stream);
int ae_ddim_encode_step_f32(const float* x, const float* eps, float* x_next, long n, int branches, float scale, float cx, float ce,
                            void* stream);
int ae_mask_blend_f32(const float* img, const float* x0, const float* noise, const float* mask, float* out, int B, int C, int HW,
                      float sqrt_ac, float sqrt_one_minus_ac, int ip2p_order, void* stream);
int ae_q_sample_f32(const float* x0, const float* noise, const float* sqrt_ac, const float* sqrt_one_minus_ac, float* out, int B,
                    long per_sample, void* stream);
int ae_silu_to_bf16(const void* x, int in_bf16, void* y, long n, void* stream);
int ae_add_bcast_bf16(const void* x, const void* p, void* y, long n, long period, void* stream);
int ae_resample2x_rows_bf16(const void* x, void* y, int B, int H, int W, int C, int mode, void* stream);
int ae_scale_shift_rows_bf16(const void* x, const float* emb, long ld_emb, void* y, int B, long HW, int C, int silu, void* stream);
int ae_window_partition_bf16(const void* image, void* windows, int B, int H, int W, int C, int ws, int reverse, void* stream);
int ae_layernorm_window_supported(int C);
int ae_layernorm_window_bf16(const void* x, const void* shortcut, const float* gamma, const float* beta, void* y, void* xsum,
                             int B, int H, int W, int C, int ws, int mode, float eps, void* stream);
int ae_sam_relpos_terms(const void* q, long q_sb, long q_sh, long q_sn, const float* Rh, const float* Rw, float* rel_h,
                        float* rel_w, int B, int heads, int qH, int qW, int kH, int kW, int D, void* stream);
int ae_patchify_f32_bf16(const float* x, void* y, int B, int Cin, int H, int W, int P, void* stream);
int ae_mse_f32(const float* a, const float* b, float* out, float* partial, long n, void* stream);
int ae_task_gate(const float* task_emb, const long* edit_code, const float* Wg, const float* bg, int B, int n_tasks, int Dt,
                 int E, float* probs, int* top1, float* top1_prob, void* stream);

int ae_softmax_rows_f32_bf16(const float* S, long lds, void* P, long ldp, int rows, int cols, float scale, void* stream);
int ae_gaussian_moments_f32(const float* moments, const float* noise, float* z, float* mean, float* logvar, float* std_out, int B,
                            long per_half, void* stream);

int ae_ms_deform_attn_fwd_f32(const float* value, const long* spatial_shapes, const long* level_start_index, const float* sampling_loc,
                              const float* attn_weight, float* out, int bs, int S, int heads, int d, int Q, int L, int P, void* stream);
int ae_ms_deform_attn_bwd_f32(const float* value, const long* spatial_shapes, const long* level_start_index, const float* sampling_loc,
                              const float* attn_weight, const float* grad_out, float* grad_value, float* grad_sampling_loc,
                              float* grad_attn_weight, int bs, int S, int heads, int d, int Q, int L, int P, void* stream);
int ae_linear_f32(const float* A, long lda, const float* W, long ldw, const float* bias, float* C, long ldc, int M, int N, int K,
                  void* stream);

int ae_dpm_multistep_f32(const float* x, const float* model_out, const float* m_prev, float* m_cur, float* x_next, long n, int branches,
                         float scale, int v_param, int predict_x0, float sigma_s, float alpha_s, int update, float a, float b, float c,
                         float inv_r0, void* stream);

int ae_lincomb4_f32(float* out, const float* x0, float c0, const float* x1, float c1, const float* x2, float c2, const float* x3, float c3,
                    long n, void* stream);
int ae_dpm_adaptive_err_f32(const float* x_lower, const float* x_higher, const float* x_prev, float atol, float rtol, int B,
                            long n_per_sample, float* out, void* stream);

int ae_layernorm_act_bf16(const void* x, const float* gamma, const float* beta, void* y, long M, int C, float eps, int act, void* stream);
int ae_sam_pe_encode_f32(const float* coords, const int* labels, const float* gauss, const float* table, float* out, int N, int F,
                         float offset, float inv_w, float inv_h, void* stream);
int ae_sam_mask_downscale_bf16(const float* masks, const float* w1, const float* b1, const float* g1, const float* e1, const float* w2,
                               const float* b2, const float* g2, const float* e2, void* out, int B, int h, int w, float eps, void* stream);
int ae_sam_mask_product_f32(const void* up, const float* hyper, float* out, int B, int h, int w, int M, int C, void* stream);
int ae_sam_postprocess_masks(const float* low, float* out_f32, void* out_u8, int N, int Hl, int Wl, int S, int ih, int iw, int oh, int ow,
                             float threshold, int merge, void* stream);
int ae_nms_sorted_f32(const float* boxes, void* keep, int N, float iou_threshold, void* stream);
int ae_sam_preprocess_f32(const void* x, int x_is_u8, float* y, int B, int C, int h, int w, int S, const float* mean, const float* stdv,
                          void* stream);

int ae_attn_causal_short_bf16(const void* q, const void* k, const void* v, void* out, int B, int H, int N, int D,
                              long q_sb, long q_sh, long q_sn, long k_sb, long k_sh, long k_sn, long v_sb, long v_sh, long v_sn,
                              long o_sb, long o_sh, long o_sn, float scale, void* stream);
int ae_clip_embed_bf16(const void* ids, int ids_are_i64, const void* token_table, const void* position_table, void* out, int B, int N,
                       int C, int vocab, int positions, void* stream);
int ae_bias_act_f32_bf16(const float* u, long ldu, const float* bias, void* y, long ldy, long M, int N, int act, void* stream);
int ae_clip_pool_eos_bf16(const void* ids, int ids_are_i64, const void* z, void* out, int B, int N, int C, long eos_token_id, void* stream);

int ae_clip_patch_rows_bf16(const void* x, int x_dtype, void* rows, int B, int Cin, int H, int W, int P, int Kpad, float rescale,
                            const float* mean, const float* stdv, void* stream);
int ae_clip_vision_embed_ln_bf16(const float* patch, long ldp, const float* class_embedding, const float* pos, const float* gamma,
                                 const float* beta, void* out, int B, int G, int C, float eps, void* stream);
int ae_clip_vision_pool_ln_bf16(const void* x, long row_stride, const float* gamma, const float* beta, void* out, int B, int C, float eps,
                                void* stream);

int ae_dino_embed_bf16(const float* patch, long ldp, const float* patch_bias, const float* cls_token, const float* pos, void* out, int B, int G,
                       int C, void* stream);
int ae_swiglu_f32_bf16(const float* u, long ldu, const float* bias, void* y, long ldy, long M, int Hd, void* stream);

int ae_swin_window_attn_bf16(const void* qkv, long ldq, const float* qkv_bias, const float* bias, void* out, long ldo, int B, int H, int W, int C,
                             int nH, int ws, int shift, float scale, void* stream);
int ae_swin_merge_ln_bf16(const void* x, const float* gamma, const float* beta, void* y, int B, int H, int W, int C, float eps, void* stream);

int ae_scale_residual_f32_bf16(const float* u, long ldu, const float* bias, const float* gamma, const void* res, long ldr, void* out, long ldo, long M,
                               int N, void* stream);
int ae_biattn_split_rows(int Nv);
long ae_biattn_workspace_bytes(int B, int heads, int Nv, int Nt, int D);
int ae_biattn_bf16(const void* q, long ldq, const void* k, long ldk, const void* val_v, long ldvv, const void* val_l, long ldvl, const void* mask_v,
                   const void* mask_l, void* out_v, long ldov, void* out_l, long ldol, int B, int heads, int Nv, int Nt, int D, float scale,
                   void* workspace, long workspace_bytes, void* stream);
int ae_attn_masked_short_bf16(const void* q, const void* k, const void* v, const void* mask, void* out, int B, int H, int N, int D, long q_sb, long q_sh,
                              long q_sn, long k_sb, long k_sh, long k_sn, long v_sb, long v_sh, long v_sn, long o_sb, long o_sh, long o_sn, float scale,
                              void* stream);

int ae_contrastive_bf16(const void* x, long ldx, const void* y, const void* token_mask, float* logits, long ldl, float* rowmax, int B, int N, int T, int C,
                        int max_text_len, void* stream);
int ae_topk_rows_max_n(void);
int ae_topk_rows_f32(const float* scores, long ld, int* out, int B, int N, int k, void* stream);
int ae_gdino_proposals_f32(const void* padding_mask, const int* shapes_hw, const int* level_start, int L, float* proposals, void* keep, int B, int N,
                           void* stream);
int ae_gdino_query_sine(const float* ref, const float* valid_ratios, float* ref_input, void* embed, long lde, int B, int nq, int L, void* stream);
int ae_gdino_box_refine_f32(const float* h, long ldh, const float* w3, const float* b3, const float* ref, float* boxes, float* u_out, long M, int ref_is_logit,
                            void* stream);

int ae_gdino_text_spans(const void* ids, int ids_are_i64, int B, int N, int n_special, long s0, long s1, long s2, long s3, long s4, long s5, long s6, long s7,
                        int* spans, long* position_ids, void* dense_mask, void* stream);
int ae_bert_embed_ln_bf16(const long* ids, const long* position_ids, const long* type_ids, const void* word_table, const void* position_table,
                          const void* type_table, const float* gamma, const float* beta, void* out, int B, int N, int C, int vocab, int positions, int types,
                          float eps, void* stream);
int ae_attn_span_short_bf16(const void* q, const void* k, const void* v, const int* spans, void* out, int B, int H, int N, int D, long q_sb, long q_sh,
                            long q_sn, long k_sb, long k_sh, long k_sn, long v_sb, long v_sh, long v_sn, long o_sb, long o_sh, long o_sn, float scale,
                            void* stream);

int ae_gdino_level_geometry(const void* mask, int B, int H, int W, const int* shapes_hw, const int* level_start, int L, float temperatureH,
                            float temperatureW, const float* level_embed, void* mask_flatten, void* pos_flatten, float* valid_ratios, int N, void* stream);
long ae_gdino_neck_groupnorm_workspace_floats(int B, int hw);
int ae_gdino_neck_groupnorm(const float* x, long ldx, const float* gamma, const float* beta, float eps, void* out, long out_batch_stride,
                            long out_row_offset, int B, int hw, float* workspace, void* stream);
int ae_gdino_ground(const float* pred_logits, const float* pred_boxes, float box_threshold, float text_threshold, int* count, int* indices, float* scores,
                    float* boxes, void* token_bits, int B, int nq, int T, void* stream);

int ae_hed_stem_bf16(const void* x, int x_is_f32, long sb, long sc, long sh, long sw, const float* norm, const float* w, const float* bias, void* out,
                     int B, int H, int W, int C1, void* stream);
int ae_relu_bf16(void* x, long n, void* stream);
int ae_hed_tail_bf16(const void* y, const float* wp, const float* bp, float* proj, void* pooled, int B, int H, int W, int C, void* stream);
int ae_hed_fuse(const float* p0, const float* p1, const float* p2, const float* p3, const float* p4, void* out, float* logits, int B, int H, int W,
                int invert, void* stream);

#ifdef __cplusplus
}
#endif
#endif
```

Measured before the change: 6.550 edited-images/sec.

## Share the first UNet stage between the two CFG branches with identical inputs

```diff
diff --git a/anyedit_amd/_lib.py b/anyedit_amd/_lib.py
--- a/anyedit_amd/_lib.py
+++ b/anyedit_amd/_lib.py
@@ -69,6 +69,7 @@
     "ae_expert_kv_dgrad": [c_void_p, c_void_p, c_void_p, c_void_p, c_int, c_int, c_int, c_int, c_int, c_void_p, c_void_p],
     "ae_expert_kv_wgrad": [c_void_p, c_void_p, c_void_p, c_void_p, c_int, c_int, c_int, c_int, c_int, c_void_p],
     "ae_transpose_last2": [c_void_p, c_void_p, c_int, c_int, c_int, c_int, c_int, c_int, c_void_p],
+    "ae_copy_segments": [c_int, ctypes.POINTER(c_void_p), ctypes.POINTER(c_void_p), ctypes.POINTER(c_long), c_void_p],
     "ae_concat_channels_bf16": [c_void_p, c_int, c_void_p, c_int, c_void_p, c_long, c_void_p],
     "ae_im2col3x3_c8_bf16": [c_void_p, c_void_p, c_int, c_int, c_int, c_void_p],
     "ae_split_channels_bf16": [c_void_p, c_int, c_int, c_void_p, c_void_p, c_long, c_int, c_int, c_void_p],
diff --git a/anyedit_amd/anysd/model.py b/anyedit_amd/anysd/model.py
--- a/anyedit_amd/anysd/model.py
+++ b/anyedit_amd/anysd/model.py
@@ -90,9 +90,11 @@
             kv_cache[("adapter", id(attn))] = (kv_ip, gate.float().contiguous())
         return context_rows, kv_cache
 
+    shares_cfg_prefix = True
+
     @torch.no_grad()
-    def denoise(self, x, timesteps, context_rows, kv_cache, emb_pack=None):
-        return self.unet.forward_rows(x, timesteps, context_rows, kv_cache=kv_cache, emb_pack=emb_pack)
+    def denoise(self, x, timesteps, context_rows, kv_cache, emb_pack=None, shared_prefix=None):
+        return self.unet.forward_rows(x, timesteps, context_rows, kv_cache=kv_cache, emb_pack=emb_pack, shared_prefix=shared_prefix)
 
     def forward(self, noisy_latents, timesteps, encoder_hidden_states, image_embeds, edit_code):
         context_rows, kv_cache = self.prepare_conditioning(encoder_hidden_states, image_embeds, edit_code)
diff --git a/anyedit_amd/anysd/pipeline.py b/anyedit_amd/anysd/pipeline.py
--- a/anyedit_amd/anysd/pipeline.py
+++ b/anyedit_amd/anysd/pipeline.py
@@ -18,10 +18,19 @@
         self._emb_pack = None
         self.randn = torch.randn
 
+    def _shared_prefix(self):
+        import os
+        if not getattr(self.moe, "shares_cfg_prefix", False) or os.environ.get("AE_CFG_PREFIX", "1") == "0":
+            return None
+        return self._x_in.shape[0] // 3
+
     def _denoise_static(self):
+        kw = {}
         if self._emb_pack is not None:
-            return self.moe.denoise(self._x_in, self._t, self._ctx_rows, self._kv_cache, emb_pack=self._emb_pack)
-        return self.moe.denoise(self._x_in, self._t, self._ctx_rows, self._kv_cache)
+            kw["emb_pack"] = self._emb_pack
+        if self._shared_prefix() is not None:
+            kw["shared_prefix"] = self._shared_prefix()
+        return self.moe.denoise(self._x_in, self._t, self._ctx_rows, self._kv_cache, **kw)
 
     def _hoist_time_embedding(self, steps_desc, nb, dev):
         import os
@@ -147,7 +156,7 @@
         if temb is not None:
             self._emb_pack.all.copy_(temb[0].unsqueeze(0).expand_as(self._emb_pack.all))
         if self.use_graph:
-            self._ensure_graph((tuple(x_T.shape), steps))
+            self._ensure_graph((tuple(x_T.shape), steps, self._shared_prefix()))
         x_view = self._x_in[:, :C].view(3, B, C, *x_T.shape[2:])
         for i, step in enumerate(np.flip(timesteps)):
             index = total - i - 1
diff --git a/anyedit_amd/csrc/c_api.hip b/anyedit_amd/csrc/c_api.hip
--- a/anyedit_amd/csrc/c_api.hip
+++ b/anyedit_amd/csrc/c_api.hip
@@ -39,6 +39,38 @@
     return AE_OK;
 }
 
+extern "C" int ae_copy_segments(int n, const void* const* src, void* const* dst, const long* bytes, void* stream) {
+    AE_REQUIRE(n >= 1 && n <= AE_COPY_MAX_SEGMENTS, "ae_copy_segments: n = %d segments, expected 1..%d", n, AE_COPY_MAX_SEGMENTS);
+    AE_REQUIRE(src && dst && bytes, "ae_copy_segments: null pointer (segment table)");
+    CopySegments t = {};
+    t.n = n;
+    long units = 0;
+    for (int i = 0; i < n; ++i) {
+        AE_REQUIRE(src[i] && dst[i], "ae_copy_segments: null pointer in segment %d", i);
+        AE_REQUIRE(bytes[i] > 0 && bytes[i] % 4 == 0, "ae_copy_segments: segment %d has %ld bytes, expected a positive multiple of 4", i, bytes[i]);
+        const uintptr_t s = (uintptr_t)src[i], d = (uintptr_t)dst[i];
+        AE_REQUIRE(s % 4 == 0 && d % 4 == 0, "ae_copy_segments: segment %d is not 4-byte aligned", i);
+        t.src[i] = (const char*)src[i];
+        t.dst[i] = (char*)dst[i];
+        t.bytes[i] = bytes[i];
+        t.vec[i] = (s % 16 == 0 && d % 16 == 0) ? 1 : 0;
+        t.first[i] = units;
+        units += (bytes[i] + 15) / 16;
+    }
+    t.first[n] = units;
+    for (int i = 0; i < n; ++i) {
+        const uintptr_t d0 = (uintptr_t)dst[i], d1 = d0 + (uintptr_t)bytes[i];
+        for (int j = 0; j < n; ++j) {
+            const uintptr_t s0 = (uintptr_t)src[j], s1 = s0 + (uintptr_t)bytes[j];
+            AE_REQUIRE(d1 <= s0 || s1 <= d0, "ae_copy_segments: the destination of segment %d overlaps the source of segment %d", i, j);
+            if (j == i) continue;
+            const uintptr_t e0 = (uintptr_t)dst[j], e1 = e0 + (uintptr_t)bytes[j];
+            AE_REQUIRE(d1 <= e0 || e1 <= d0, "ae_copy_segments: the destinations of segments %d and %d overlap", i, j);
+        }
+    }
+    return ae_launch_copy_segments(t, (hipStream_t)stream);
+}
+
 extern "C" int ae_device_info(int* cus, long* hbm_bytes, int* clock_khz) {
     int dev = 0;
     hipDeviceProp_t prop;
diff --git a/anyedit_amd/csrc/common.hpp b/anyedit_amd/csrc/common.hpp
--- a/anyedit_amd/csrc/common.hpp
+++ b/anyedit_amd/csrc/common.hpp
@@ -21,6 +21,17 @@
 int ae_rowpanel_fold_covers(int M, int N, int K, int epilogue, int mode);
 int ae_rowpanel_fold_launch(const void* A, long lda, const void* W, long ldw, void* C, long ldc, int M, int N, int K, const float* bias, const void* residual,
                             long ldr, int epilogue, float* rowstats_out, const float* ln_stats, int ln_parts, const float* ln_colsum, float ln_eps, void* stream);
+
+#define AE_COPY_MAX_SEGMENTS 8
+struct CopySegments {
+    const char* src[AE_COPY_MAX_SEGMENTS];
+    char* dst[AE_COPY_MAX_SEGMENTS];
+    long bytes[AE_COPY_MAX_SEGMENTS];
+    long first[AE_COPY_MAX_SEGMENTS + 1];
+    int vec[AE_COPY_MAX_SEGMENTS];
+    int n;
+};
+int ae_launch_copy_segments(const CopySegments& t, hipStream_t stream);
 
 #define AE_REQUIRE(cond, ...)                 \
     do {                                      \
diff --git a/anyedit_amd/csrc/elementwise.hip b/anyedit_amd/csrc/elementwise.hip
--- a/anyedit_amd/csrc/elementwise.hip
+++ b/anyedit_amd/csrc/elementwise.hip
@@ -510,6 +510,34 @@
 
 }
 
+__global__ __launch_bounds__(256) void copy_segments_kernel(const CopySegments t) {
+    const long total = t.first[t.n];
+    for (long i = (long)blockIdx.x * NT + threadIdx.x; i < total; i += (long)gridDim.x * NT) {
+        const char* src = t.src[0];
+        char* dst = t.dst[0];
+        long bytes = t.bytes[0], first = 0;
+        int vec = t.vec[0];
+#pragma unroll
+        for (int k = 1; k < AE_COPY_MAX_SEGMENTS; ++k)
+            if (k < t.n && i >= t.first[k]) { src = t.src[k]; dst = t.dst[k]; bytes = t.bytes[k]; first = t.first[k]; vec = t.vec[k]; }
+        const long off = (i - first) * 16;
+        src += off;
+        dst += off;
+        const long left = bytes - off;
+        if (vec && left >= 16) {
+            *reinterpret_cast<u32x4*>(dst) = *reinterpret_cast<const u32x4*>(src);
+        } else {
+            const int nd = left >= 16 ? 4 : (int)(left >> 2);
+            for (int d = 0; d < nd; ++d) reinterpret_cast<uint32_t*>(dst)[d] = reinterpret_cast<const uint32_t*>(src)[d];
+        }
+    }
+}
+
+int ae_launch_copy_segments(const CopySegments& t, hipStream_t stream) {
+    hipLaunchKernelGGL(copy_segments_kernel, dim3(grid_for(t.first[t.n], 4)), dim3(NT), 0, stream, t);
+    return ae_check_launch("ae_copy_segments");
+}
+
 __global__ __launch_bounds__(256) void lincomb4_kernel(float* __restrict__ out, const float* x0, float c0, const float* x1, float c1,
                                                         const float* x2, float c2, const float* x3, float c3, long n) {
     const long i = ((long)blockIdx.x * 256 + threadIdx.x) * 4;
diff --git a/anyedit_amd/csrc/gemm_conv.hip b/anyedit_amd/csrc/gemm_conv.hip
--- a/anyedit_amd/csrc/gemm_conv.hip
+++ b/anyedit_amd/csrc/gemm_conv.hip
@@ -1346,7 +1346,9 @@
         const long t128x = (long)((a.M + 127) / 128) * ((a.N + 127) / 128);
         const bool xe_tail = t320_xe && !conv && a.xe == 2 && a.epi != EPI_GEGLU && fill >= 0.74 && fill < 0.85 &&
                              (double)t128x / (double)(((t128x + 511) / 512) * 512) <= 0.72;
-        if (fill >= 0.85 || xe_tail) {
+        static const int t320_round = getenv("AE_CONV_T320_ROUND") ? atoi(getenv("AE_CONV_T320_ROUND")) : 1;
+        const bool one_round = t320_round && conv && a.N == 320 && t <= 256 && fill >= 0.66;
+        if (fill >= 0.85 || xe_tail || one_round) {
             if constexpr (AMODE == A_DENSE) {
                 if (xe_tail || (a.epi == EPI_GEGLU && a.xe == 2)) { rc = run_tile<192, 320, A_DENSE, 4, 2, true, 1, 2, false, 0, 3, 2>(lc, t, lds_aa(192, 320) + 2 * 320 * sizeof(float)); xe_done = true; }
                 else if (a.epi == EPI_GEGLU) rc = run_tile<192, 320, A_DENSE, 4, 2, true, 1, 2, false, 0, 3>(lc, t, lds_aa(192, 320));
diff --git a/anyedit_amd/ldm/modules/attention.py b/anyedit_amd/ldm/modules/attention.py
--- a/anyedit_amd/ldm/modules/attention.py
+++ b/anyedit_amd/ldm/modules/attention.py
@@ -163,7 +163,7 @@
         return ops.gemm(ctx_rows, self._packed()["kv"])
 
     def rows(self, x, B, N, context_rows=None, Nk=None, kv=None, key_mask=None, residual=None, adapter=None, norm=None, rowstats=None,
-             out_rowstats=None):
+             out_rowstats=None, out=None):
         h, d = self.heads, self.dim_head
         inner = h * d
         pk = self._packed()
@@ -202,7 +202,7 @@
                     ks_ip = (T_ip * 2 * inner, d, 2 * inner)
                     ops.attention(q, kv_ip, kv_ip[:, inner:], B, h, N, T_ip, d, self.scale, qs, ks_ip, ks_ip, out=o,
                                   out_scale=gate, accumulate=True)
-        return self.to_out[0].rows(o.reshape(B * N, inner), residual=residual, rowstats=out_rowstats)
+        return self.to_out[0].rows(o.reshape(B * N, inner), residual=residual, rowstats=out_rowstats, out=out)
 
     def forward(self, x, context=None, mask=None):
         B, N, C = x.shape
@@ -244,11 +244,11 @@
         self.norm3 = LayerNorm(dim)
         self.checkpoint = checkpoint
 
-    def rows(self, x, B, N, context_rows=None, kv_cache=None, rowstats=None, tail=None):
+    def rows(self, x, B, N, context_rows=None, kv_cache=None, rowstats=None, tail=None, shared=None):
         tape = ops._TAPE
         if self.checkpoint and tape is not None and tape.active:
             return tape.checkpoint(lambda: self._rows(x, B, N, context_rows, kv_cache))
-        return self._rows(x, B, N, context_rows, kv_cache, rowstats, tail)
+        return self._rows(x, B, N, context_rows, kv_cache, rowstats, tail, shared)
 
     def takes_tail(self, M, C):
         return _FF_TAIL and self.ff.fused_ok(M, C)
@@ -269,14 +269,29 @@
     def wants_rowstats(self, M, C):
         return self._fold_plan(M, C)[0]
 
-    def _rows(self, x, B, N, context_rows=None, kv_cache=None, rowstats=None, tail=None):
+    def _rows(self, x, B, N, context_rows=None, kv_cache=None, rowstats=None, tail=None, shared=None):
         c1 = context_rows if self.disable_self_attn else None
-        M, C = x.shape
+        Mx, C = x.shape
+        M = Mx if shared is None else B * N
         f1, f2, f3 = self._fold_plan(M, C)
+        if shared is not None:
+            inner1, inner2 = self.attn1.heads * self.attn1.dim_head, self.attn2.heads * self.attn2.dim_head
+            f1 = self._fold_plan(Mx, C)[0]
+            f2 = ops.ln_fold_plan(M, inner2, C, ops.EPI_NONE, 2) and ops.ln_fold_plan(Mx, C, inner1, ops.EPI_NONE, 1)
         kv2, adapter = None, None
         st2 = ops.rowstats_buffer(M, C, x.device) if f2 else None
         st3 = ops.rowstats_buffer(M, C, x.device) if f3 else None
-        x = self.attn1.rows(x, B, N, context_rows=c1, residual=x, norm=self.norm1, rowstats=rowstats if f1 else None, out_rowstats=st2)
+        if shared is None:
+            x = self.attn1.rows(x, B, N, context_rows=c1, residual=x, norm=self.norm1, rowstats=rowstats if f1 else None, out_rowstats=st2)
+        else:
+            B0, pairs = shared
+            r0 = B0 * N
+            y = torch.empty(M, C, dtype=BF16, device=x.device)
+            self.attn1.rows(x, B - B0, N, residual=x, norm=self.norm1, rowstats=rowstats if f1 else None, out_rowstats=None if st2 is None else st2[r0:],
+                            out=y[r0:])
+            pairs = list(pairs) + [(y[r0:2 * r0], y[:r0])] + ([] if st2 is None else [(st2[r0:2 * r0], st2[:r0])])
+            ops.copy_segments(pairs)
+            x = y
         if kv_cache is not None and context_rows is not None:
             key = id(self.attn2)
             kv2 = kv_cache.get(key)
@@ -325,13 +340,17 @@
             self.proj_out = zero_module(Linear(in_channels, inner_dim))
         self.use_linear = use_linear
 
-    def rows(self, x, B, H, W, context_rows=None, kv_cache=None, colstats=None, out_colstats=None):
+    def rows(self, x, B, H, W, context_rows=None, kv_cache=None, colstats=None, out_colstats=None, shared=None):
         if isinstance(context_rows, (list, tuple)):
             ctxs = list(context_rows)
         else:
             ctxs = [context_rows] * len(self.transformer_blocks)
         N = H * W
-        h = self.norm.rows(x, B, N, colstats=colstats)
+        B0 = 0
+        if shared is not None:
+            B0, x_full, pairs = shared
+            pairs = list(pairs) + [(x_full[B0 * N:2 * B0 * N], x_full[:B0 * N])]
+        h = self.norm.rows(x, B - B0, N, colstats=colstats)
         pin = self.proj_in._packed()
         M, Ci = h.shape[0], pin["w"].shape[0]
         st = None
@@ -340,10 +359,13 @@
         h = ops.gemm(h, pin["w"], pin["b"], rowstats=st)
         pout = self.proj_out._packed()
         last = len(self.transformer_blocks) - 1
+        if shared is not None:
+            M, x = B * N, x_full
         tail_ok = self.transformer_blocks[last].takes_tail(M, Ci) and pout["w"].shape == (Ci, Ci) and x.shape[1] == Ci
         for i, blk in enumerate(self.transformer_blocks):
             tail = (pout["w"], pout["b"], x, out_colstats) if (tail_ok and i == last) else None
-            h = blk.rows(h, B, N, context_rows=ctxs[i], kv_cache=kv_cache, rowstats=st if i == 0 else None, tail=tail)
+            h = blk.rows(h, B, N, context_rows=ctxs[i], kv_cache=kv_cache, rowstats=st if i == 0 else None, tail=tail,
+                         shared=(B0, pairs) if (shared is not None and i == 0) else None)
         if tail_ok:
             return h
         return ops.gemm(h, pout["w"], pout["b"], residual=x, colstats=out_colstats)
diff --git a/anyedit_amd/ldm/modules/diffusionmodules/openaimodel.py b/anyedit_amd/ldm/modules/diffusionmodules/openaimodel.py
--- a/anyedit_amd/ldm/modules/diffusionmodules/openaimodel.py
+++ b/anyedit_amd/ldm/modules/diffusionmodules/openaimodel.py
@@ -1,5 +1,6 @@
 from abc import abstractmethod
 import math
+import os
 
 import torch
 import torch.nn as nn
@@ -166,13 +167,13 @@
         else:
             self.skip_connection = conv_nd(dims, channels, self.out_channels, 1)
 
-    def rows(self, f, emb_silu):
+    def rows(self, f, emb_silu, out=None):
         tape = ops._TAPE
         if self.use_checkpoint and tape is not None and tape.active:
             return Feat(tape.checkpoint(lambda: self._rows(f, emb_silu).t), f.B, f.H, f.W)
-        return self._rows(f, emb_silu)
-
-    def _rows(self, f, emb_silu):
+        return self._rows(f, emb_silu, out)
+
+    def _rows(self, f, emb_silu, out=None):
         B, H, W = f.B, f.H, f.W
         if isinstance(emb_silu, EmbPack) and id(self) in emb_silu.offsets:
             off = emb_silu.offsets[id(self)]
@@ -208,7 +209,7 @@
         else:
             res, _, _ = self.skip_connection.rows(whole() if xs is None else xs, B, Ho, Wo)
         st = _stats_for(B, Ho, Wo, self.out_channels, dev)
-        y, _, _ = self.out_layers[3].rows(h, B, Ho, Wo, residual=res, colstats=st)
+        y, _, _ = self.out_layers[3].rows(h, B, Ho, Wo, residual=res, colstats=st, out=out)
         return Feat(y, B, Ho, Wo, st=st)
 
     def forward(self, x, emb):
@@ -456,7 +457,35 @@
         emb = self.time_embed[0].rows(t_emb, epilogue=ops.EPI_SILU)
         return self._emb_pack(self.time_embed[2].rows(emb, epilogue=ops.EPI_SILU))
 
-    def forward_rows(self, x, timesteps, context_rows, kv_cache=None, y=None, emb_pack=None):
+    def _shares_prefix(self, B, B0, y):
+        if not B0 or B0 < 0 or B != 3 * B0 or y is not None or (ops._TAPE is not None and ops._TAPE.active) or os.environ.get("AE_CFG_PREFIX", "1") == "0":
+            return False
+        if len(self.input_blocks) < 2 or len(self.input_blocks[0]) != 1 or not hasattr(self.input_blocks[0][0], "out_hw") or len(self.input_blocks[1]) != 2:
+            return False
+        res, st = self.input_blocks[1]
+        return isinstance(res, ResBlock) and not res.updown and isinstance(st, SpatialTransformer) and not st.transformer_blocks[0].disable_self_attn
+
+    def _prefix_rows(self, x, emb_silu, context_rows, kv_cache, B0):
+        B, C, H, W = x.shape
+        Bp, N = B - B0, H * W
+        r0 = B0 * N
+        stem_conv = self.input_blocks[0][0]
+        res, st_mod = self.input_blocks[1]
+        dev = x.device
+        emb_p = EmbPack(None if emb_silu.silu is None else emb_silu.silu[B0:], emb_silu.all[B0:], emb_silu.offsets)
+        stem = torch.empty(B * N, stem_conv.out_channels, dtype=BF16, device=dev)
+        stem_st = _stats_for(B, H, W, stem_conv.out_channels, dev)
+        pairs = [(stem[r0:2 * r0], stem[:r0])]
+        if stem_st is not None:
+            pairs.append((stem_st[r0 // 32:2 * r0 // 32], stem_st[:r0 // 32]))
+        stem_conv.rows(ops.nchw_to_rows(x[B0:], (C + 7) // 8 * 8), Bp, H, W, colstats=None if stem_st is None else stem_st[r0 // 32:], out=stem[r0:])
+        h = torch.empty(B * N, res.out_channels, dtype=BF16, device=dev)
+        fr = res.rows(Feat(stem[r0:], Bp, H, W, st=None if stem_st is None else stem_st[r0 // 32:]), emb_p, out=h[r0:])
+        st = _stats_for(B, H, W, res.out_channels, dev)
+        y = st_mod.rows(fr.t, B, H, W, context_rows=context_rows, kv_cache=kv_cache, colstats=fr.st, out_colstats=st, shared=(B0, h, pairs))
+        return Feat(stem, B, H, W, st=stem_st), Feat(y, B, H, W, st=st)
+
+    def forward_rows(self, x, timesteps, context_rows, kv_cache=None, y=None, emb_pack=None, shared_prefix=None):
         B, C, H, W = x.shape
         assert (y is not None) == (self.num_classes is not None), "must specify y if and only if the model is class-conditional"
         if emb_pack is not None:
@@ -473,9 +502,15 @@
                 lab = self._label_rows(y, e32.device)
                 emb_silu = ops.silu_to_bf16(ops.lincomb([(e32, 1.0), (lab, 1.0)]))
             emb_silu = self._emb_pack(emb_silu)
-        f = Feat(ops.nchw_to_rows(x, (C + 7) // 8 * 8), B, H, W)
         hs = []
-        for module in self.input_blocks:
+        blocks = self.input_blocks
+        if self._shares_prefix(B, shared_prefix, y):
+            hs = list(self._prefix_rows(x, emb_silu, context_rows, kv_cache, shared_prefix))
+            f = hs[-1]
+            blocks = list(self.input_blocks)[2:]
+        else:
+            f = Feat(ops.nchw_to_rows(x, (C + 7) // 8 * 8), B, H, W)
+        for module in blocks:
             if isinstance(module[0], TimestepBlock) or isinstance(module[0], (Downsample, Upsample)) or len(module) > 1:
                 f = module.rows(f, emb_silu, context_rows, kv_cache)
             else:
diff --git a/anyedit_amd/ldm/modules/diffusionmodules/util.py b/anyedit_amd/ldm/modules/diffusionmodules/util.py
--- a/anyedit_amd/ldm/modules/diffusionmodules/util.py
+++ b/anyedit_amd/ldm/modules/diffusionmodules/util.py
@@ -95,11 +95,11 @@
     def _pack(self):
         return {"w": ops.pack_linear(self.weight), "b": None if self.bias is None else self.bias.detach().float().contiguous()}
 
-    def rows(self, x, residual=None, epilogue=ops.EPI_NONE, out_f32=False, a2=None, rowstats=None):
+    def rows(self, x, residual=None, epilogue=ops.EPI_NONE, out_f32=False, a2=None, rowstats=None, out=None):
         pk = self._packed()
         if rowstats is not None:
-            return ops.gemm(x, pk["w"], pk["b"], residual=residual, epilogue=epilogue, out_f32=out_f32, a2=a2, rowstats=rowstats)
-        return ops.gemm(x, pk["w"], pk["b"], residual=residual, epilogue=epilogue, out_f32=out_f32, a2=a2)
+            return ops.gemm(x, pk["w"], pk["b"], residual=residual, epilogue=epilogue, out_f32=out_f32, a2=a2, rowstats=rowstats, out=out)
+        return ops.gemm(x, pk["w"], pk["b"], residual=residual, epilogue=epilogue, out_f32=out_f32, a2=a2, out=out)
 
     def forward(self, x):
         shp = x.shape
@@ -118,19 +118,19 @@
             return {"w": ops.pack_conv3x3(self.weight), "b": b}
         raise NotImplementedError(f"anyedit_amd Conv2d: unsupported configuration k={k} stride={self.stride} padding={self.padding}")
 
-    def rows(self, x, B, H, W, addvec=None, residual=None, upsample2x=False, out_f32=False, a2=None, colstats=None):
+    def rows(self, x, B, H, W, addvec=None, residual=None, upsample2x=False, out_f32=False, a2=None, colstats=None, out=None):
         pk = self._packed()
         if self.kernel_size[0] == 1:
-            return ops.gemm(x, pk["w"], pk["b"], residual=residual, out_f32=out_f32, a2=a2, colstats=colstats), H, W
+            return ops.gemm(x, pk["w"], pk["b"], residual=residual, out_f32=out_f32, a2=a2, colstats=colstats, out=out), H, W
         if addvec is None and residual is None and not out_f32 and a2 is None and ops.stem_im2col_ok(self.in_channels, self.stride[0], upsample2x):
             if "w_taps" not in pk:
                 pk["w_taps"] = ops.pack_conv3x3_taps8(self.weight)
-            return ops.gemm(ops.im2col3x3_c8(x, B, H, W), pk["w_taps"], pk["b"], colstats=colstats), H, W
+            return ops.gemm(ops.im2col3x3_c8(x, B, H, W), pk["w_taps"], pk["b"], colstats=colstats, out=out), H, W
         if upsample2x and addvec is None and residual is None and not out_f32 and a2 is None and \
                 ops.up2_subpixel_ok(self.in_channels, self.out_channels, H, W, colstats is not None) and self.stride[0] == 1:
             if "w_up2" not in pk:
                 pk["w_up2"] = ops.pack_conv3x3_up2(self.weight)
-            return ops.conv3x3_up2(x, pk["w_up2"], pk["b"], B, H, W, colstats=colstats)
+            return ops.conv3x3_up2(x, pk["w_up2"], pk["b"], B, H, W, colstats=colstats, out=out)
         Ho, Wo = self.out_hw(H, W, upsample2x)
         ko = ops.conv_k_order(B * Ho * Wo, self.in_channels, self.out_channels, self.stride[0], upsample2x)
         w = pk["w"]
@@ -139,7 +139,7 @@
                 pk["w_kmajor"] = ops.pack_conv3x3(self.weight, k_order=1)
             w = pk["w_kmajor"]
         return ops.conv3x3(x, w, pk["b"], B, H, W, addvec=addvec, residual=residual, stride=self.stride[0],
-                           upsample2x=upsample2x, out_f32=out_f32, colstats=colstats, k_order=ko)
+                           upsample2x=upsample2x, out_f32=out_f32, colstats=colstats, k_order=ko, out=out)
 
     def out_hw(self, H, W, upsample2x=False):
         if self.kernel_size[0] == 1:
diff --git a/anyedit_amd/ops.py b/anyedit_amd/ops.py
--- a/anyedit_amd/ops.py
+++ b/anyedit_amd/ops.py
@@ -1415,6 +1415,19 @@
     return out
 
 
+def copy_segments(pairs):
+    n = len(pairs)
+    src, dst, nbytes = (ctypes.c_void_p * max(n, 1))(), (ctypes.c_void_p * max(n, 1))(), (ctypes.c_long * max(n, 1))()
+    for i, (s, d) in enumerate(pairs):
+        for t, name in ((s, "src"), (d, "dst")):
+            if not t.is_cuda or not t.is_contiguous():
+                raise ValueError(f"copy_segments: {name} of segment {i} must be a contiguous GPU tensor")
+        if s.numel() * s.element_size() != d.numel() * d.element_size():
+            raise ValueError(f"copy_segments: segment {i} copies {s.numel() * s.element_size()} bytes into {d.numel() * d.element_size()}")
+        src[i], dst[i], nbytes[i] = s.data_ptr(), d.data_ptr(), s.numel() * s.element_size()
+    check(lib.ae_copy_segments(n, src, dst, nbytes, _s()), "ae_copy_segments")
+
+
 def split_channels(dy, ca, a=None, b=None, want_a=True, want_b=True):
     dy = _dense(dy, BF16, "split_channels.dy", 2)
     rows, C = dy.shape
@@ -2188,6 +2201,9 @@
 hed_stem = _wrap_profiled(hed_stem, lambda _r, x, norm, w, bias, out=None: (
     f"hed_stem_kernel<{'u8' if x.dtype == torch.uint8 else 'f32'}>|M={_r[0].shape[0]} C1={_r[0].shape[1]}", 2.0 * 27 * _r[0].numel(),
     float(x.numel() * x.element_size() + 2 * _r[0].numel())))
+copy_segments = _wrap_profiled(copy_segments, lambda _r, pairs: (
+    f"copy_segments_kernel|n={len(pairs)} bytes={sum(s.numel() * s.element_size() for s, _d in pairs)}", 0.0,
+    2.0 * sum(s.numel() * s.element_size() for s, _d in pairs)))
 relu_ = _wrap_profiled(relu_, lambda _r, x: (f"relu_bf16_kernel|n={x.numel()}", 0.0, 4.0 * x.numel()))
 hed_tail = _wrap_profiled(hed_tail, lambda _r, y, wp, bp, B, H, W, pool=True, proj=None, pooled=None: (
     f"hed_tail_kernel<{'pool' if pool else 'last'}>|M={y.shape[0]} C={y.shape[1]}", 2.0 * y.numel(),
diff --git a/include/anyedit_hip.h b/include/anyedit_hip.h
--- a/include/anyedit_hip.h
+++ b/include/anyedit_hip.h
@@ -110,6 +110,7 @@
 int ae_expert_kv_wgrad(const void* dy, const void* x, const int* experts, float* dW, int B, int T, int N, int Dc, int E, void* stream);
 
 int ae_transpose_last2(const void* in, void* out, int B, int X, int Y, int Xpad, int in_bf16, int out_bf16, void* stream);
+int ae_copy_segments(int n, const void* const* src, void* const* dst, const long* bytes, void* stream);
 int ae_concat_channels_bf16(const void* a, int Ca, const void* b, int Cb, void* y, long rows, void* stream);
 int ae_im2col3x3_c8_bf16(const void* x, void* y, int B, int H, int W, void* stream);
 int ae_split_channels_bf16(const void* y, int Ca, int Cb, void* a, void* b, long rows, int accumulate_a, int accumulate_b, void* stream);
```

Measured after the change: 6.594 edited-images/sec (median of 6 runs). Within noise of the previous version (+0.7%).
